# roeiherz/CanonicalSg2Im

Hardware: AMD Instinct MI355X
Metric: 256x256 images/sec/node (G+D step) (higher is better)
Workload: dtype f32; 1 GPU; BASELINE config C3: COCO-shaped AttSPADE 256x256, batch 16/GPU, 1-30 objects/img, ngf=64 ndf=64, --no_vgg_loss --use_img_disc 0; Sg2Layout GCN + SPADE G + 2-scale PatchGAN D + object-crop D, fwd+bwd+Adam; global_batch=16, parallelism=dp1

## Files before the change

canonicalsg2im_amd/_lib.py:

```python
import ctypes
import os

import torch

_HERE = os.path.dirname(os.path.abspath(__file__))
LIB_PATH = os.environ.get("CSG_HIP_LIB") or os.path.join(_HERE, "libcsg_hip.so")

MAX_TAPS = 16
ACT_NONE, ACT_LEAKY, ACT_TANH = 0, 1, 2

c_i32, c_i64, c_f32, c_f64, c_p = ctypes.c_int32, ctypes.c_int64, ctypes.c_float, ctypes.c_double, ctypes.c_void_p


class ConvDesc(ctypes.Structure):
    _fields_ = [
        ("B", c_i32), ("IHp", c_i32), ("IWp", c_i32), ("Cin", c_i32), ("x_cs", c_i32),
        ("IHv", c_i32), ("IWv", c_i32), ("in_up", c_i32),
        ("OHg", c_i32), ("OWg", c_i32), ("OHf", c_i32), ("OWf", c_i32), ("os", c_i32), ("ooy", c_i32), ("oox", c_i32),
        ("Cout", c_i32), ("y_cs", c_i32),
        ("istride", c_i32), ("ntaps", c_i32), ("wtaps", c_i32),
        ("tap_dy", c_i32 * MAX_TAPS), ("tap_dx", c_i32 * MAX_TAPS), ("tap_w", c_i32 * MAX_TAPS),
        ("act", c_i32), ("slope", c_f32), ("accumulate", c_i32), ("res_gate", c_i32),
    ]


class WinoDesc(ctypes.Structure):
    _fields_ = [("B", c_i32), ("H", c_i32), ("W", c_i32), ("Cin", c_i32), ("x_cs", c_i32), ("Cout", c_i32),
                ("y_cs", c_i32), ("act", c_i32), ("slope", c_f32)]


class WinoPackItem(ctypes.Structure):
    _fields_ = [("w", c_p), ("s_o", c_i64), ("s_i", c_i64), ("s_h", c_i64), ("s_w", c_i64), ("Cout", c_i64), ("Cin", c_i64),
                ("backward_data", c_i32), ("variant", c_i32), ("packed", c_p)]


class HingeItem(ctypes.Structure):
    _fields_ = [("x", c_p), ("dx", c_p), ("sb", c_i64), ("sh", c_i64), ("sw", c_i64), ("B", c_i64), ("H", c_i64), ("W", c_i64)]


class FewDesc(ctypes.Structure):
    _fields_ = [("B", c_i32), ("IH", c_i32), ("IW", c_i32), ("Cin", c_i32), ("x_cs", c_i32), ("KH", c_i32), ("KW", c_i32),
                ("pad", c_i32), ("cout_real", c_i32), ("act", c_i32), ("slope", c_f32), ("in_act", c_i32), ("in_slope", c_f32)]


class SnFwdItem(ctypes.Structure):
    _fields_ = [("w", c_p), ("u", c_p), ("v", c_p), ("Cout", c_i64), ("K", c_i64), ("w_eff", c_p), ("cl_Cin", c_i64),
                ("sigma", c_p), ("u_used", c_p), ("v_used", c_p), ("workspace", c_p), ("workspace_bytes", c_i64)]


class SnBwdItem(ctypes.Structure):
    _fields_ = [("dweff", c_p), ("Cout", c_i64), ("Cin", c_i64), ("KH", c_i64), ("KW", c_i64), ("s0", c_i64), ("s1", c_i64),
                ("s2", c_i64), ("s3", c_i64), ("w", c_p), ("u_used", c_p), ("v_used", c_p), ("sigma", c_p), ("dw", c_p),
                ("workspace", c_p), ("workspace_bytes", c_i64)]


class NormEvalItem(ctypes.Structure):
    _fields_ = [("running_mean", c_p), ("running_var", c_p), ("C", c_i64), ("offset", c_i64)]


class EmaItem(ctypes.Structure):
    _fields_ = [("src", c_p), ("dst", c_p), ("numel", c_i64), ("chunk0", c_i64), ("kind", c_i32), ("reserved", c_i32)]


class GemmDesc(ctypes.Structure):
    _fields_ = [("M", ctypes.c_int64), ("N", ctypes.c_int64), ("K", ctypes.c_int64),
                ("lda", ctypes.c_int64), ("ldb", ctypes.c_int64), ("ldy", ctypes.c_int64), ("ldg", ctypes.c_int64),
                ("act", ctypes.c_int32), ("slope", ctypes.c_float), ("gate_slope", ctypes.c_float)]


SIGNATURES = {
    "csg_version": (c_i32, []),
    "csg_last_error": (ctypes.c_char_p, []),
    "csg_prof_enable": (c_i32, [c_i32]),
    "csg_prof_reset": (c_i32, []),
    "csg_prof_num_kernels": (c_i32, []),
    "csg_prof_kernel_name": (ctypes.c_char_p, [c_i32]),
    "csg_prof_read": (c_i32, [c_i32, ctypes.POINTER(c_f64), ctypes.POINTER(c_i64), ctypes.POINTER(c_f64)]),
    "csg_embed_fwd": (c_i32, [c_p, c_i64, c_i64, c_p, c_i64, c_i64, c_p, c_i64, c_i64, c_p]),
    "csg_embed_bwd_workspace": (c_i64, [c_i64, c_i64, c_i64]),
    "csg_embed_bwd": (c_i32, [c_p, c_i64, c_i64, c_p, c_i64, c_i64, c_i64, c_i64, c_p, c_p, c_i64, c_p]),
    "csg_real_object_mask": (c_i32, [c_p, c_i64, c_i64, c_i64, c_i64, c_p, c_p]),
    "csg_graph_csr_build": (c_i32, [c_p, c_i64, c_i64, c_i64, c_p, c_p, c_p]),
    "csg_graph_csr_lds": (c_i64, [c_i64, c_i64]),
    "csg_gather_concat_fwd": (c_i32, [c_p, c_p, c_p, c_i64, c_i64, c_i64, c_i64, c_i64, c_p, c_p]),
    "csg_gather_concat_bwd_workspace": (c_i64, [c_i64, c_i64, c_i64, c_i64]),
    "csg_gather_concat_bwd": (c_i32, [c_p, c_p, c_p, c_i64, c_i64, c_i64, c_i64, c_i64, c_p, c_p, c_p, c_i64, c_p]),
    "csg_segment_avg_fwd_workspace": (c_i64, [c_i64, c_i64, c_i64, c_i64]),
    "csg_segment_avg_fwd": (c_i32, [c_p, c_p, c_p, c_p, c_p, c_i64, c_i64, c_i64, c_i64, c_i64, c_p, c_p, c_p, c_p,
                                    c_i64, c_p]),
    "csg_segment_avg_bwd": (c_i32, [c_p, c_p, c_p, c_p, c_p, c_p, c_p, c_p, c_i64, c_i64, c_i64, c_i64, c_i64, c_i32,
                                    c_p, c_p, c_p, c_p]),
    "csg_layout_fwd": (c_i32, [c_p, c_p, c_p, c_p, c_i64, c_i64, c_i64, c_i64, c_i64, c_i64, c_i64, c_i64, c_p, c_i64,
                               c_i64, c_p]),
    "csg_disc_input_fwd": (c_i32, [c_p, c_p, c_p, c_p, c_i64, c_i64, c_i64, c_i64, c_i64, c_i64, c_p, c_i64, c_i64, c_i64,
                                   c_i64, c_p, c_i64, c_p]),
    "csg_layout_bwd_workspace": (c_i64, [c_i64, c_i64, c_i64, c_i64, c_i64, c_i32, c_i32]),
    "csg_layout_bwd": (c_i32, [c_p, c_i64, c_i64, c_p, c_p, c_p, c_i64, c_i64, c_i64, c_i64, c_i64, c_i64, c_i64,
                               c_i64, c_p, c_i32, c_p, c_p, c_p, c_i64, c_p]),
    "csg_layout_bwd_masks": (c_i32, [c_p, c_i64, c_i64, c_p, c_p, c_i64, c_i64, c_i64, c_i64, c_i64, c_i64, c_i64, c_i64,
                                     c_p, c_p, c_i32, c_p]),
    "csg_layout_mass": (c_i32, [c_p, c_p, c_p, c_p, c_i64, c_i64, c_i64, c_i64, c_i64, c_i64, c_p, c_p]),
    "csg_layout_paint": (c_i32, [c_p, c_p, c_p, c_i64, c_p, c_i64, c_i64, c_i64, c_i64, c_i64, c_i64, c_i64, c_p, c_i64,
                                 c_i64, c_p]),
    "csg_conv_fwd_workspace": (c_i64, [ctypes.POINTER(ConvDesc)]),
    "csg_conv_fwd": (c_i32, [ctypes.POINTER(ConvDesc), c_p, c_p, c_p, c_p, c_p, c_p, c_i64, c_p]),
    "csg_conv_bwd_weight_workspace": (c_i64, [ctypes.POINTER(ConvDesc)]),
    "csg_conv_bwd_weight": (c_i32, [ctypes.POINTER(ConvDesc), c_p, c_p, c_p, c_p, c_p, c_i64, c_p]),
    "csg_wino_pack_bytes": (c_i64, [c_i64, c_i64]),
    "csg_wino_pack_weights": (c_i32, [c_p, c_i64, c_i64, c_i64, c_i64, c_i64, c_i64, c_i32, c_p, c_p, c_p]),
    "csg_conv_fwd_multi_workspace": (c_i64, [ctypes.POINTER(ConvDesc), c_i32]),
    "csg_conv_fwd_multi": (c_i32, [ctypes.POINTER(ConvDesc), c_i32, c_p, c_p, c_p, c_p, c_p, c_p, c_i64, c_p]),
    "csg_gemm_supported": (c_i32, [ctypes.POINTER(GemmDesc)]),
    "csg_gemm_nt": (c_i32, [ctypes.POINTER(GemmDesc), c_p, c_p, c_p, c_p, c_p, c_p]),
    "csg_gemm_tn_workspace": (c_i64, [c_i64, c_i64, c_i64]),
    "csg_gemm_tn": (c_i32, [c_i64, c_i64, c_i64, c_p, c_i64, c_p, c_i64, c_p, c_p, c_p, c_i64, c_p]),
    "csg_conv_few_supported": (c_i32, [ctypes.POINTER(FewDesc)]),
    "csg_conv_few_fwd_workspace": (c_i64, [ctypes.POINTER(FewDesc)]),
    "csg_conv_few_fwd": (c_i32, [ctypes.POINTER(FewDesc), c_p, c_p, c_p, c_p, c_p, c_i64, c_p]),
    "csg_conv_few_bwd_data": (c_i32, [ctypes.POINTER(FewDesc), c_p, c_p, c_p, c_p]),
    "csg_conv_few_bwd_weight_workspace": (c_i64, [ctypes.POINTER(FewDesc)]),
    "csg_conv_few_bwd_weight": (c_i32, [ctypes.POINTER(FewDesc), c_p, c_p, c_p, c_p, c_p, c_i64, c_p]),
    "csg_wino_conv_workspace": (c_i64, [ctypes.POINTER(WinoDesc)]),
    "csg_wino_conv": (c_i32, [ctypes.POINTER(WinoDesc), c_p, c_p, c_p, c_p, c_p, c_f32, c_p, c_p, c_i64, c_p]),
    "csg_wino_bwd_weight_workspace": (c_i64, [ctypes.POINTER(WinoDesc)]),
    "csg_wino_bwd_weight": (c_i32, [ctypes.POINTER(WinoDesc), c_p, c_p, c_p, c_p, c_p, c_i64, c_p]),
    "csg_wino4_bwd_weight_workspace": (c_i64, [ctypes.POINTER(WinoDesc)]),
    "csg_wino4_bwd_weight": (c_i32, [ctypes.POINTER(WinoDesc), c_p, c_p, c_p, c_p, c_p, c_i64, c_p]),
    "csg_wino4_supported": (c_i32, [ctypes.POINTER(WinoDesc)]),
    "csg_wino4_persistent": (c_i32, [c_i32]),
    "csg_wino_pack_weights_multi": (c_i32, [ctypes.POINTER(WinoPackItem), c_i32, c_p]),
    "csg_wino4_pack_bytes": (c_i64, [c_i64, c_i64]),
    "csg_wino4_pack_weights": (c_i32, [c_p, c_i64, c_i64, c_i64, c_i64, c_i64, c_i64, c_i32, c_p, c_p, c_p]),
    "csg_wino4_conv_workspace": (c_i64, [ctypes.POINTER(WinoDesc)]),
    "csg_wino4_conv": (c_i32, [ctypes.POINTER(WinoDesc), c_p, c_p, c_p, c_p, c_p, c_f32, c_p, c_p, c_i64, c_p]),
    "csg_wino4_conv_part": (c_i32, [ctypes.POINTER(WinoDesc), c_p, c_p, c_i64, c_i64, c_p, c_p, c_p, c_i64, c_p, c_p, c_f32,
                                    c_p, c_p]),
    "csg_wino4_conv_spade_supported": (c_i32, [ctypes.POINTER(WinoDesc)]),
    "csg_wino4_conv_spade": (c_i32, [ctypes.POINTER(WinoDesc), c_p, c_p, c_p, c_p, c_p, c_i64, c_p, c_p, c_f32, c_p, c_p]),
    "csg_wino34_supported": (c_i32, [ctypes.POINTER(WinoDesc), c_i32]),
    "csg_wino34_pack_weights": (c_i32, [c_p, c_i64, c_i64, c_i64, c_i64, c_i64, c_i64, c_i32, c_p, c_p, c_p]),
    "csg_wino34_conv_workspace": (c_i64, [ctypes.POINTER(WinoDesc), c_i32]),
    "csg_wino34_conv": (c_i32, [ctypes.POINTER(WinoDesc), c_i32, c_p, c_p, c_p, c_p, c_p, c_f32, c_p, c_p, c_i64, c_p]),
    "csg_act_bwd": (c_i32, [c_p, c_p, c_i64, c_i32, c_f32, c_p, c_p]),
    "csg_colsum": (c_i32, [c_p, c_i64, c_i64, c_i64, c_p, c_p, c_i64, c_p]),
    "csg_norm_stats": (c_i32, [c_p, c_i64, c_i64, c_i64, c_p, c_p, c_i64, c_p]),
    "csg_norm_finalize": (c_i32, [c_p, c_i64, c_i64, c_f64, c_f32, c_i32, c_p, c_p, c_p, c_p, c_f32, c_p]),
    "csg_norm_stats_finalize": (c_i32, [c_p, c_i64, c_i64, c_i64, c_p, c_i64, c_f64, c_f32, c_p, c_p, c_p, c_p, c_p, c_p, c_f32,
                                        c_p]),
    "csg_norm_apply_fwd": (c_i32, [c_p, c_p, c_p, c_p, c_f32, c_i64, c_i64, c_i64, c_p, c_p, c_f32, c_p, c_p]),
    "csg_norm_eval_stats_multi": (c_i32, [ctypes.POINTER(NormEvalItem), c_i32, c_f32, c_p, c_p]),
    "csg_deprocess_u8_workspace": (c_i64, [c_i64]),
    "csg_deprocess_u8": (c_i32, [c_p, c_i64, c_i64, c_i64, c_i64, ctypes.POINTER(c_f32), ctypes.POINTER(c_f32), c_i32, c_p, c_p,
                                 c_i64, c_p]),
    "csg_preprocess_workspace": (c_i64, [c_p, c_i64, c_i64]),
    "csg_preprocess": (c_i32, [c_p, c_i64, c_p, c_p, c_i64, c_i64, c_i64, ctypes.POINTER(c_f32), ctypes.POINTER(c_f32), c_p, c_p,
                               c_p, c_i64, c_p]),
    "csg_preprocess_px_workspace": (c_i64, [c_p, c_i64, c_i64]),
    "csg_preprocess_px": (c_i32, [c_p, c_i64, c_p, c_p, c_i64, c_i64, c_i64, ctypes.POINTER(c_f32), ctypes.POINTER(c_f32), c_p,
                                  c_p, c_p, c_i64, c_p]),
    "csg_clevr_boxes": (c_i32, [c_p, c_p, c_i64, c_p, c_p, c_p, c_p, c_i64, c_i64, c_p, c_p]),
    "csg_vg_rows": (c_i32, [c_p, c_p, c_p, c_p, c_p, c_p, c_i64, c_i64, c_i64, c_p, c_p, c_p]),
    "csg_draw_boxes_u8": (c_i32, [c_p, c_p, c_p, c_i64, c_i64, c_i64, c_i64, c_i64, c_i64, c_p, c_i64, c_i32, c_p, c_p]),
    "csg_draw_labels_u8": (c_i32, [c_p, c_p, c_p, c_i64, c_i64, c_i64, c_i64, c_i64, c_i64, c_p, c_i64, c_p, c_p, c_p, c_p,
                                   c_p]),
    "csg_draw_graph_u8": (c_i32, [c_p, c_i64, c_p, c_p, c_i64, c_p, c_i64, c_i64, c_i64, ctypes.c_uint32, c_p, c_p]),
    "csg_box_iou": (c_i32, [c_p, c_p, c_p, c_i64, c_i64, c_i64, c_i64, c_p, c_p, c_p, c_p, c_p]),
    "csg_relation_agreement_workspace": (c_i64, [c_i64]),
    "csg_relation_agreement": (c_i32, [c_p, c_p, c_p, c_p, c_p, c_p, c_i64, c_i64, c_i64, c_i64, c_p, c_p, c_p, c_p, c_p, c_p,
                                       c_i64, c_p]),
    "csg_layout_consistency": (c_i32, [c_p, c_p, c_p, c_i64, c_i64, c_p, c_p, c_p, c_p, c_p, c_p, c_p]),
    "csg_graph_rows_select": (c_i32, [c_p, c_p, c_i64, c_i64, c_i64, c_i64, c_p, c_p, c_p, c_p]),
    "csg_graph_rewrite": (c_i32, [c_p, c_p, c_p, c_i64, c_i64, c_i64, c_p, c_i32, c_i32, c_f64, ctypes.c_uint64, c_p, c_p]),
    "csg_norm_apply_bwd_reduce": (c_i32, [c_p, c_p, c_p, c_p, c_p, c_p, c_f32, c_i64, c_i64, c_i64, c_p, c_p, c_p, c_i64,
                                          c_i64, c_p]),
    "csg_norm_apply_bwd_dx": (c_i32, [c_p, c_p, c_p, c_p, c_p, c_f32, c_p, c_f64, c_i64, c_i64, c_i64, c_p, c_p, c_p, c_f32,
                                      c_p, c_p, c_i64, c_p]),
    "csg_nearest_resize_fwd": (c_i32, [c_p, c_i64, c_i64, c_i64, c_i64, c_i64, c_i64, c_p, c_p]),
    "csg_nearest_resize_bwd": (c_i32, [c_p, c_i64, c_i64, c_i64, c_i64, c_i64, c_i64, c_p, c_p]),
    "csg_upsample2x_fwd": (c_i32, [c_p, c_i64, c_i64, c_i64, c_i64, c_p, c_p]),
    "csg_upsample2x_bwd": (c_i32, [c_p, c_i64, c_i64, c_i64, c_i64, c_p, c_p]),
    "csg_avgpool3s2_fwd": (c_i32, [c_p, c_i64, c_i64, c_i64, c_i64, c_p, c_p]),
    "csg_avgpool3s2_bwd": (c_i32, [c_p, c_i64, c_i64, c_i64, c_i64, c_p, c_p]),
    "csg_avgpool3s2_bwd_add": (c_i32, [c_p, c_i64, c_i64, c_i64, c_i64, c_p, c_p, c_p]),
    "csg_crop_fwd": (c_i32, [c_p, c_i64, c_i64, c_i64, c_i64, c_i64, c_p, c_p, c_i64, c_i64, c_i64, c_p, c_i64, c_p]),
    "csg_crop_bwd": (c_i32, [c_p, c_i64, c_i64, c_i64, c_i64, c_i64, c_p, c_p, c_i64, c_i64, c_i64, c_i64, c_p, c_p]),
    "csg_crop_bwd_boxes": (c_i32, [c_p, c_p, c_i64, c_i64, c_i64, c_i64, c_i64, c_p, c_p, c_i64, c_i64, c_i64, c_i64, c_p,
                                   c_p]),
    "csg_maxpool2_fwd": (c_i32, [c_p, c_i64, c_i64, c_i64, c_i64, c_p, c_p]),
    "csg_maxpool2_bwd": (c_i32, [c_p, c_p, c_i64, c_i64, c_i64, c_i64, c_p, c_p]),
    "csg_avgpool2_fwd": (c_i32, [c_p, c_i64, c_i64, c_i64, c_i64, c_p, c_p]),
    "csg_avgpool2_bwd": (c_i32, [c_p, c_i64, c_i64, c_i64, c_i64, c_p, c_p]),
    "csg_l1_mean_workspace": (c_i64, [c_i64]),
    "csg_l1_mean_fwd": (c_i32, [c_p, c_p, c_i64, c_p, c_p, c_i64, c_p]),
    "csg_l1_mean_bwd": (c_i32, [c_p, c_p, c_p, c_i64, c_p, c_p]),
    "csg_hinge_mean_fwd": (c_i32, [ctypes.POINTER(HingeItem), c_i32, c_i32, c_p, c_p]),
    "csg_hinge_mean_bwd": (c_i32, [ctypes.POINTER(HingeItem), c_i32, c_i32, c_p, c_p]),
    "csg_spectral_norm_workspace": (c_i64, [c_i64, c_i64]),
    "csg_spectral_norm_fwd_multi": (c_i32, [ctypes.POINTER(SnFwdItem), c_i32, c_i32, c_f32, c_p]),
    "csg_spectral_norm_bwd_multi": (c_i32, [ctypes.POINTER(SnBwdItem), c_i32, c_p]),
    "csg_canon_workspace": (c_i64, [c_i64]),
    "csg_canon_build": (c_i32, [c_p, c_p, c_p, c_p, c_i64, c_i64, ctypes.POINTER(c_i32), c_i64, c_i32, c_i32, c_p, c_i64,
                                c_p, c_p]),
    "csg_canon_emit": (c_i32, [c_p, c_p, c_i64, c_i64, ctypes.POINTER(c_i32), c_i64, c_i32, c_i32, c_p, c_p, c_i64, c_p,
                               c_p, c_p]),
    "csg_canon_converse": (c_i32, [c_p, c_p, c_i64, c_i64, ctypes.POINTER(c_i32), c_i64, c_i32, c_i32, c_p, c_p, c_p, c_p,
                                   c_i64, c_p, c_p, c_p]),
    "csg_canon_general_workspace": (c_i64, [c_i64, c_i64, c_i64]),
    "csg_canon_general_build": (c_i32, [c_p, c_p, c_p, c_p, c_i64, c_i64, c_p, c_p, c_i64, ctypes.POINTER(c_i32), c_i64,
                                        c_i64, c_i32, c_p, c_i64, c_p, c_p]),
    "csg_canon_general_build_dev": (c_i32, [c_p, c_p, c_p, c_p, c_i64, c_i64, c_p, c_p, c_i64, ctypes.POINTER(c_i32), c_i64,
                                            c_i64, c_i32, c_p, c_i64, c_p, c_p]),
    "csg_pair_relations": (c_i32, [c_p, c_p, c_p, c_p, c_p, c_p, c_p, c_p, c_i64, c_i64, ctypes.POINTER(c_i32), c_i32, c_p,
                                   c_p]),
    "csg_coco_masks": (c_i32, [c_p] * 16 + [c_i64] * 6 + [c_p, c_p, c_p]),
    "csg_canon_general_converse": (c_i32, [c_i64, ctypes.POINTER(c_i32), c_i64, c_p, c_i64, c_p, c_p, c_p, c_p, c_p]),
    "csg_canon_general_close": (c_i32, [c_i64, ctypes.POINTER(c_i32), c_i64, c_i32, c_p, c_i64, c_p, c_p]),
    "csg_canon_general_emit": (c_i32, [c_i64, ctypes.POINTER(c_i32), c_i64, c_p, c_i64, c_p, c_i64, c_p, c_p, c_p]),
    "csg_canon_small_workspace": (c_i64, [c_i64, c_i64]),
    "csg_canon_small_build": (c_i32, [c_p, c_p, c_p, c_i64, c_i64, c_p, c_p, c_i64, c_i64, c_i64, c_i64, c_i64, c_i32, c_i32,
                                      c_p, c_p, c_p, c_i64, c_p, c_p, c_i64, c_p, c_p]),
    "csg_canon_small_emit": (c_i32, [c_i64, c_i64, c_i64, c_p, c_i64, c_p, c_i64, c_p, c_p, c_p]),
    "csg_clevr_graph_count": (c_i32, [c_p, c_p, c_i64, c_i64, c_p, c_p, c_i64, c_i64, c_i64, c_i64, c_i32, c_p, c_p]),
    "csg_clevr_graph_emit": (c_i32, [c_p, c_i64, c_i64, c_p, c_i64, c_i64, c_i64, c_i64, c_i32, c_i64, c_p, c_p, c_p]),
    "csg_resize_bilinear": (c_i32, [c_p, c_i32, c_i64, c_i64, c_i64, c_i64, c_i64, c_i64, c_f32, c_f32, c_i32, c_p, c_p]),
    "csg_pool3": (c_i32, [c_p, c_i64, c_i64, c_i64, c_i64, c_i64, c_i32, c_i32, c_i32, c_p, c_i64, c_i64, c_p]),
    "csg_spatial_mean": (c_i32, [c_p, c_i64, c_i64, c_i64, c_i64, c_p, c_p]),
    "csg_bias_act": (c_i32, [c_p, c_i64, c_i64, c_i64, c_i64, c_p, c_i32, c_f32, c_p]),
    "csg_feat_stats": (c_i32, [c_p, c_i64, c_i64, c_p, c_p, c_p]),
    "csg_feat_stats_finalize": (c_i32, [c_p, c_p, c_i64, c_i64, c_p, c_p, c_p]),
    "csg_softmax_rows": (c_i32, [c_p, c_i64, c_i64, c_i64, c_p, c_p]),
    "csg_inception_score_workspace": (c_i64, [c_i64, c_i64, c_i64]),
    "csg_inception_score": (c_i32, [c_p, c_i64, c_i64, c_i64, c_p, c_i64, c_p, c_p]),
    "csg_crop_windows": (c_i32, [c_p, c_i64, c_i64, c_i64, c_p, c_p]),
    "csg_crop_resize_bilinear": (c_i32, [c_p, c_i64, c_i64, c_i64, c_p, c_p, c_i64, c_i64, c_i64, c_f32, c_f32, c_i32, c_p, c_p]),
    "csg_kid_sums_workspace_bytes": (c_i64, [c_i64, c_i64]),
    "csg_kid_sums": (c_i32, [c_p, c_i64, c_p, c_i64, c_i64, c_p, c_p, c_i64, c_i64, c_f64, c_f64, c_i32, c_p, c_i64, c_p, c_p]),
    "csg_feat_class_sums": (c_i32, [c_p, c_p, c_i64, c_i64, c_i64, c_p, c_p, c_p]),
    "csg_manifold_column_chunks": (c_i64, [c_i64, c_i64]),
    "csg_knn_radii_workspace_bytes": (c_i64, [c_i64, c_i64]),
    "csg_knn_radii": (c_i32, [c_p, c_i64, c_i64, c_i64, c_p, c_i64, c_p, c_p]),
    "csg_ball_counts_workspace_bytes": (c_i64, [c_i64, c_i64]),
    "csg_ball_counts": (c_i32, [c_p, c_i64, c_p, c_i64, c_i64, c_p, c_p, c_i64, c_p, c_p, c_p]),
    "csg_ema_table_plan": (c_i64, [ctypes.POINTER(EmaItem), c_i64]),
    "csg_ema_apply": (c_i32, [c_p, c_i64, c_i64, c_i32, c_f32, c_f32, c_p]),
    "csg_augment_table": (c_i32, [ctypes.c_uint64, c_i64, c_i64, c_i64, c_i64, c_i64, c_p, c_p]),
    "csg_augment_table_host": (c_i32, [ctypes.c_uint64, c_i64, c_i64, c_i64, c_i64, c_i64, c_p]),
    "csg_augment_workspace_bytes": (c_i64, [c_i64, c_i64]),
    "csg_augment_fwd": (c_i32, [c_p, c_p, c_p, c_i64, c_i64, c_i64, c_i64, c_i64, c_i32, c_p, c_i64, c_p]),
    "csg_augment_bwd": (c_i32, [c_p, c_p, c_p, c_i64, c_i64, c_i64, c_i64, c_i64, c_i32, c_p, c_i64, c_p]),
    "csg_augment_gate": (c_i32, [ctypes.c_uint64, c_i64, c_i64, c_i64, c_i64, c_p, c_p, c_p]),
    "csg_augment_gate_host": (c_i32, [ctypes.c_uint64, c_i64, c_i64, c_i64, c_i64, c_i64, c_p]),
    "csg_augment_fwd_gated": (c_i32, [c_p, c_p, c_p, c_i64, c_i64, c_i64, c_i64, c_i64, c_i32, c_p, c_i64, c_p, c_p]),
    "csg_augment_bwd_gated": (c_i32, [c_p, c_p, c_p, c_i64, c_i64, c_i64, c_i64, c_i64, c_i32, c_p, c_i64, c_p, c_p]),
    "csg_ada_accumulate": (c_i32, [ctypes.POINTER(HingeItem), c_i32, c_p, c_p]),
    "csg_ada_update": (c_i32, [c_p, c_i64, c_i64, c_p]),
    "csg_ada_update_host": (c_i32, [c_p, c_i64, c_i64]),
}


def _load():
    if not os.path.exists(LIB_PATH):
        raise ImportError(
            "libcsg_hip.so is not built (%s). Run `python -c 'import __graft_entry__ as g; g.build()'` "
            "from the repository root; there is no CPU fallback." % LIB_PATH)
    lib = ctypes.CDLL(LIB_PATH)
    for name, (res, args) in SIGNATURES.items():
        fn = getattr(lib, name)
        fn.restype = res
        fn.argtypes = args
    return lib


lib = _load()


def last_error():
    return lib.csg_last_error().decode("utf-8", "replace")

# ... 41 lines not shown
```

canonicalsg2im_amd/csrc/csg_api.hip:

```cpp
#include <stdarg.h>
#include <string.h>

#include <mutex>
#include <vector>

#include "csg_common.h"

namespace csg {

static thread_local char g_err[512] = "";

void set_error(const char* fmt, ...) {
  va_list ap;
  va_start(ap, fmt);
  vsnprintf(g_err, sizeof(g_err), fmt, ap);
  va_end(ap);
}

int check_launch(const char* what) {
  hipError_t e = hipGetLastError();
  if (e != hipSuccess) {
    set_error("%s: %s", what, hipGetErrorString(e));
    return CSG_E_LAUNCH;
  }
  return CSG_OK;
}

struct Rec {
  int kid;
  double work;
  hipEvent_t e0, e1;
  bool first;
};
static int g_prof = 0;
static std::mutex g_mu;
static std::vector<Rec> g_pending;
static std::vector<hipEvent_t> g_free;
static double g_ms[K_COUNT];
static double g_work[K_COUNT];
static int64_t g_n[K_COUNT];

static bool hbm_kernel(int kid) {
  switch (kid) {
    case K_GATHER_FWD: case K_GATHER_BWD: case K_SEGAVG_FWD: case K_SEGAVG_BWD: case K_LAYOUT_FWD: case K_LAYOUT_BWD:
    case K_ACT_BWD: case K_NORM_STATS: case K_NORM_APPLY_FWD: case K_NORM_BWD_REDUCE: case K_NORM_BWD_DX:
    case K_UPSAMPLE_FWD: case K_UPSAMPLE_BWD: case K_AVGPOOL_FWD: case K_AVGPOOL_BWD:
      return true;
    default:
      return false;
  }
}

bool prof_on(int kid) {
  return g_prof == 1 || (g_prof == 2 && (kid == K_IGEMM_FWD || kid == K_WINO_CONV || kid == K_WINO4_CONV)) ||
         (g_prof == 3 && hbm_kernel(kid));
}

bool prof_serialize() { return g_prof == 1 || g_prof == 3; }

ProfCur& prof_cur() {
  static thread_local ProfCur cur = {0, 0.0, false, false};
  return cur;
}

static hipEvent_t get_event() {
  std::lock_guard<std::mutex> lk(g_mu);
  if (!g_free.empty()) {
    hipEvent_t e = g_free.back();
    g_free.pop_back();
    return e;
  }
  hipEvent_t e;
  hipEventCreate(&e);
  return e;
}

void prof_begin(int kid, double work) {
  ProfCur& c = prof_cur();
  c.kid = kid;
  c.work = work;
  c.armed = true;
  c.used = false;
}

void prof_next(hipEvent_t& e0, hipEvent_t& e1) {
  ProfCur& c = prof_cur();
  e0 = get_event();
  e1 = get_event();
  std::lock_guard<std::mutex> lk(g_mu);
  g_pending.push_back(Rec{c.kid, c.used ? 0.0 : c.work, e0, e1, !c.used});
  c.used = true;
}

void prof_end() {
  ProfCur& c = prof_cur();
  c.armed = c.used = false;
}

static void resolve() {
  std::lock_guard<std::mutex> lk(g_mu);
  for (auto& r : g_pending) {
    hipEventSynchronize(r.e1);
    float ms = 0.f;
    hipEventElapsedTime(&ms, r.e0, r.e1);
    g_ms[r.kid] += ms;
    g_work[r.kid] += r.work;
    g_n[r.kid] += r.first ? 1 : 0;
    g_free.push_back(r.e0);
    g_free.push_back(r.e1);
  }
  g_pending.clear();
}

static const char* kNames[K_COUNT] = {
    "embed_fwd",      "embed_bwd",      "real_object_mask", "graph_csr_build", "gather_concat_fwd", "gather_concat_bwd",
    "segment_avg_fwd", "segment_avg_bwd", "layout_fwd",       "layout_bwd",      "igemm_fwd",         "igemm_fwd64",   "splitk_epilogue", "igemm_wgrad",
    "wgrad_reduce",   "act_bwd",        "colsum",           "norm_stats",      "norm_finalize",     "norm_apply_fwd",
    "norm_bwd_reduce", "norm_bwd_dx",    "upsample2x_fwd",   "upsample2x_bwd",  "avgpool3s2_fwd",    "avgpool3s2_bwd", "crop_fwd", "crop_bwd",
    "maxpool2_fwd",   "maxpool2_bwd",   "l1_mean_fwd",      "l1_mean_bwd",
    "canon_build",    "canon_emit",     "spectral_norm_fwd", "spectral_norm_bwd",
    "wino_conv",      "wino_pack",      "wino_wgrad",
    "few_fwd",        "few_bwd_data",   "few_bwd_weight",
    "wino4_conv",     "wino4_wgrad",
    "gemm_nt",        "gemm_tn",
    "norm_eval_stats", "deprocess_u8", "box_iou", "preprocess", "clevr_boxes", "vg_rows", "draw_boxes_u8",
    "canon_small_build", "canon_small_emit", "clevr_graph_count", "clevr_graph_emit", "coco_masks",
    "resize_bilinear", "pool3", "spatial_mean", "bias_act", "feat_stats", "inception_score",
    "draw_labels_u8", "draw_graph_u8",
    "crop_windows", "crop_resize_bilinear", "kid_sums", "feat_class_sums",
    "knn_radii", "ball_counts",
    "ema", "augment"};

}

extern "C" {

int csg_version(void) { return 122; }
const char* csg_last_error(void) { return csg::g_err; }

int csg_prof_enable(int on) {
  csg::resolve();
  csg::g_prof = on < 0 ? 0 : (on > 3 ? 1 : on);
  return CSG_OK;
}

int csg_prof_reset(void) {
  csg::resolve();
  memset(csg::g_ms, 0, sizeof(csg::g_ms));
  memset(csg::g_work, 0, sizeof(csg::g_work));
  memset(csg::g_n, 0, sizeof(csg::g_n));
  return CSG_OK;
}

int csg_prof_num_kernels(void) { return csg::K_COUNT; }

const char* csg_prof_kernel_name(int kid) {
  if (kid < 0 || kid >= csg::K_COUNT) return "";
  return csg::kNames[kid];
}

int csg_prof_read(int kid, double* ms, int64_t* launches, double* work) {
  CSG_REQUIRE(kid >= 0 && kid < csg::K_COUNT, CSG_E_BADSHAPE, "csg_prof_read: bad kernel id %d", kid);
  csg::resolve();
  if (ms) *ms = csg::g_ms[kid];
  if (launches) *launches = csg::g_n[kid];
  if (work) *work = csg::g_work[kid];
  return CSG_OK;
}

}
```

canonicalsg2im_amd/csrc/csg_pack.h:

```cpp
#pragma once
#include <stdint.h>

#include <hip/hip_runtime.h>

#define CSG_PACK_MULTI 24

struct PackMultiItem {
  const float* w;
  float4* up;
  int s_n, s_k, s_h, s_w;
  int flip, N, K, NT32, Q8;
  int start;
};

struct PackMulti {
  PackMultiItem it[CSG_PACK_MULTI];
  int n;
};

extern "C" __attribute__((visibility("hidden"))) int csg_wino2_pack_multi_launch(const PackMulti* pm, int blocks, double bytes,
                                                                                 hipStream_t s);
extern "C" __attribute__((visibility("hidden"))) int csg_wino4_pack_multi_launch(const PackMulti* pm, int blocks, double bytes,
                                                                                 hipStream_t s);
```

canonicalsg2im_amd/csrc/csg_wino_host.h:

```cpp
#pragma once
#include "csg_common.h"
#include "csg_reduce.h"

namespace csg {

template <typename Pixels>
static inline int wino_desc_check(const csg_wino_desc* d, const char* who, int positions, Pixels pixels) {
  CSG_REQUIRE(d != nullptr, CSG_E_BADSHAPE, "%s: null descriptor", who);
  CSG_REQUIRE(d->B > 0 && d->H > 0 && d->W > 0 && d->Cin > 0 && d->Cout > 0, CSG_E_BADSHAPE, "%s: non-positive dimension", who);
  CSG_REQUIRE(d->Cin % 4 == 0 && d->x_cs % 4 == 0 && d->x_cs >= d->Cin && d->Cout % 4 == 0 && d->y_cs % 4 == 0 &&
                  d->y_cs >= d->Cout,
              CSG_E_UNSUPPORTED, "%s: channel counts and strides must be multiples of 4", who);
  CSG_REQUIRE((int64_t)pixels(*d) * (int64_t)(d->x_cs > d->y_cs ? d->x_cs : d->y_cs) * 4 < CSG_MAX_RECORDS, CSG_E_UNSUPPORTED,
              "%s: tensor too large for 32-bit byte offsets", who);
  CSG_REQUIRE((int64_t)positions * ((d->Cout + 31) / 32) * ((d->Cin + 7) / 8) * 1024 < CSG_MAX_RECORDS, CSG_E_UNSUPPORTED,
              "%s: packed weights too large for 32-bit byte offsets", who);
  return CSG_OK;
}

static inline int wino_conv_dense_x(const csg_wino_desc* d, const char* who) {
  CSG_REQUIRE(d->x_cs == d->Cin, CSG_E_UNSUPPORTED, "%s: x must be dense (x_cs=%d, Cin=%d)", who, d->x_cs, d->Cin);
  return CSG_OK;
}

template <typename P>
static inline void wino_split_plan(P& p, bool plain, int min_stages, int min_range) {
  if (!plain || p.y_cs != p.Cout) return;
  const int64_t blocks = (int64_t)p.B * p.tby * p.tbx * p.nblocks;
  if (blocks >= 384 || p.nstage < min_stages) return;
  int ks = (int)((512 + blocks - 1) / blocks);
  if (ks > p.nstage / min_range) ks = p.nstage / min_range;
  if (ks < 2) return;
  p.sps = (p.nstage + ks - 1) / ks;
  p.ksplit = (p.nstage + p.sps - 1) / p.sps;
}

template <typename P, typename Plan>
static inline int64_t wino_conv_workspace(const csg_wino_desc* d, int min_stages, int min_range, Plan plan) {
  P p;
  size_t shm = 0;
  if (plan(p, shm)) return -1;
  wino_split_plan(p, d->act == CSG_ACT_NONE, min_stages, min_range);
  return p.ksplit > 1 ? (int64_t)p.ksplit * p.slab * 4 : 0;
}

struct WinoConvArgs {
  const float *x, *packed, *bias, *residual, *gate;
  float gate_slope;
  float *y, *workspace;
  int64_t workspace_bytes;
  hipStream_t s;
};

template <typename P, typename Plan, typename Launch>
static inline int wino_conv_entry(const char* who, const char* sum_who, const csg_wino_desc* d, int min_stages, int min_range,
                                  int kid, double taps, const WinoConvArgs& a, Plan plan, Launch launch) {
  P p;
  size_t shm = 0;
  int rc = plan(p, shm);
  if (rc) return rc;
  wino_split_plan(p, d->act == CSG_ACT_NONE && a.bias == nullptr && a.residual == nullptr && a.gate == nullptr, min_stages,
                  min_range);
  p.gate_slope = a.gate_slope;
  if (p.ksplit > 1 && (a.workspace == nullptr || a.workspace_bytes < (int64_t)p.ksplit * p.slab * 4)) {
    p.ksplit = 1;
    p.sps = p.nstage;
  }
  float* const y = p.ksplit > 1 ? a.workspace : a.y;
  CSG_REQUIRE(((uintptr_t)a.x % 16) == 0 && ((uintptr_t)a.packed % 16) == 0 && ((uintptr_t)y % 16) == 0 &&
                  (a.gate == nullptr || ((uintptr_t)a.gate % 16) == 0),
              CSG_E_UNSUPPORTED, "%s: x, packed, y, gate and workspace must be 16-byte aligned", who);
  ProfScope ps(kid, 2.0 * (double)(p.slab / p.y_cs) * taps * p.Cin * p.Cout, a.s);
  rc = launch(p, shm, y);
  if (rc == CSG_OK && p.ksplit > 1) {
    launch_slab_reduce(a.workspace, p.slab, a.y, nullptr, 0, nullptr, p.ksplit, a.s);
    rc = check_launch(sum_who);
  }
  return rc;
}

static inline int64_t wino_pack_bytes(int positions, int64_t N, int64_t K) {
  if (N <= 0 || K <= 0) return -1;
  return (int64_t)positions * cdiv(N, 32) * cdiv(K, 8) * 64 * 16;
}

template <typename Launch>
static inline int wino_pack_entry(const char* who, int positions, int taps, const float* w, int64_t s_o, int64_t s_i,
                                  int64_t s_h, int64_t s_w, int64_t Cout, int64_t Cin, int32_t backward_data,
                                  const float* sigma, float* packed, void* stream, Launch launch) {
  CSG_REQUIRE(w != nullptr && packed != nullptr && Cout > 0 && Cin > 0, CSG_E_BADSHAPE, "%s: bad arguments", who);
  CSG_REQUIRE(((uintptr_t)packed % 16) == 0, CSG_E_UNSUPPORTED, "%s: packed must be 16-byte aligned", who);
  const int64_t N = backward_data ? Cin : Cout, K = backward_data ? Cout : Cin;
  const int64_t s_n = backward_data ? s_i : s_o, s_k = backward_data ? s_o : s_i;
  const int NT32 = (int)cdiv(N, 32), Q8 = (int)cdiv(K, 8);
  hipStream_t s = (hipStream_t)stream;
  ProfScope ps(K_WINO_PACK, (double)Cout * Cin * taps * 4 + (double)wino_pack_bytes(positions, N, K), s);
  launch(dim3((unsigned)cdiv(Q8, 4), (unsigned)NT32), s, w, s_n, s_k, s_h, s_w, backward_data ? 1 : 0, (int)N, (int)K, sigma, NT32,
         Q8, (float4*)packed);
  return check_launch(who);
}

template <typename P>
static inline int wino_wg_slice_plan(P& p, const char* who, int tiles2d, int target_blocks, int min_regions, int max_slices) {
  const int64_t nr = (int64_t)p.B * p.RXn * p.RYn;
  CSG_REQUIRE(nr < (1ll << 30), CSG_E_UNSUPPORTED, "%s: too many regions", who);
  p.nregions = (int)nr;
  int ns = (target_blocks + tiles2d - 1) / tiles2d;
  const int max_ns = (int)((nr + min_regions - 1) / min_regions);
  if (ns > max_ns) ns = max_ns;
  if (ns > max_slices) ns = max_slices;
  if (ns < 1) ns = 1;
  p.rps = (int)((nr + ns - 1) / ns);
  p.nsplit = (int)((nr + p.rps - 1) / p.rps);
  return CSG_OK;
}

static inline int64_t wino_wg_workspace(const csg_wino_desc* d, int nslab) {
  return (int64_t)nslab * d->Cout * (9 * (int64_t)d->Cin + 1) * 4;
}

template <typename Launch>
static inline int wino_wg_run(const char* who, const char* sum_who, const csg_wino_desc* d, int nslab, bool direct, float* dw,
                              float* db, float* workspace, int64_t workspace_bytes, hipStream_t s, Launch launch) {
  const int64_t wsize = (int64_t)d->Cout * 9 * d->Cin, need = wino_wg_workspace(d, nslab);
  CSG_REQUIRE(workspace != nullptr && workspace_bytes >= need, CSG_E_WORKSPACE, "%s: workspace %ld < %ld bytes", who,
              (long)workspace_bytes, (long)need);
  float* const dbslabs = db != nullptr ? workspace + (int64_t)nslab * wsize : nullptr;
  const int rc = direct ? launch(dw, db) : launch(workspace, dbslabs);
  if (rc || direct) return rc;
  ProfScope ps(K_WGRAD_REDUCE, (double)(nslab + 1) * wsize * 4, s);
  launch_slab_reduce(workspace, wsize, dw, dbslabs, db != nullptr ? d->Cout : 0, db, nslab, s);
  return check_launch(sum_who);
}

}
```

canonicalsg2im_amd/csrc/wino.hip:

```cpp
#include <stddef.h>
#include <stdlib.h>

#include <type_traits>

#include "csg_buffer.h"
#include "csg_common.h"
#include "csg_pack.h"
#include "csg_reduce.h"
#include "csg_wino_host.h"

using namespace csg;

typedef __attribute__((ext_vector_type(16))) float f32x16;

#define WN_BK 16
#define WN_PS 18
#define WN_RSE 36
#define WN_MAXLD 7

struct WinoParams {
  int B, H, W, Cin, x_cs, Cout, y_cs;
  int TW, TH;
  int tbx, tby;
  int nblocks;
  int RS;
  int NT32, Q8;
  int act;
  float slope;
  float gate_slope;
  int nstage;
  int ntb;
  int ksplit, sps;
  long long slab;
};

__device__ __forceinline__ int wn_xcd_remap(int bid, int nblk) {
  const int q = nblk >> 3, r = nblk & 7;
  const int xcd = bid & 7, idx = bid >> 3;
  return (xcd < r ? xcd * (q + 1) : r * (q + 1) + (xcd - r) * q) + idx;
}

#define WP_LD 33
__device__ __forceinline__ void wn_pack_tile(const float* __restrict__ w, int64_t s_n, int64_t s_k, int64_t s_h,
                                             int64_t s_w, int flip, int N, int K, const float* __restrict__ sigma,
                                             int NT32, int Q8, float4* __restrict__ up, int qb, int nt) {
  __shared__ float g[9][32][WP_LD];
  const int tid = threadIdx.x;
  const bool k_fast = s_k <= s_n;
  const float sg = sigma != nullptr ? sigma[0] : 1.0f;
  float stage[36];
#pragma unroll
  for (int it = 0; it < 36; ++it) {
    const int t = it >> 2, r = tid + 256 * (it & 3);
    const int nl = k_fast ? (r >> 5) : (r & 31), kl = k_fast ? (r & 31) : (r >> 5);
    const int n = nt * 32 + nl, k = qb * 32 + kl;
    const int a = t / 3, b = t - 3 * a;
    const int aa = flip ? 2 - a : a, bb = flip ? 2 - b : b;
    stage[it] = (n < N && k < K) ? w[(int64_t)n * s_n + (int64_t)k * s_k + aa * s_h + bb * s_w] : 0.f;
  }
#pragma unroll
  for (int it = 0; it < 36; ++it) {
    const int t = it >> 2, r = tid + 256 * (it & 3);
    const int nl = k_fast ? (r >> 5) : (r & 31), kl = k_fast ? (r & 31) : (r >> 5);
    g[t][nl][kl] = sigma != nullptr ? stage[it] / sg : stage[it];
  }
  __syncthreads();
  const int lane = tid & 63, ql = tid >> 6;
  const int q = qb * 4 + ql;
  if (q >= Q8) return;
  const int nl = lane & 31, h = lane >> 5;
  float u[16][4];
#pragma unroll
  for (int e = 0; e < 4; ++e) {
    const int kl = 8 * ql + (e >> 1) * 4 + 2 * h + (e & 1);
    float t[4][3];
#pragma unroll
    for (int b = 0; b < 3; ++b) {
      const float g0 = g[b][nl][kl], g1 = g[3 + b][nl][kl], g2 = g[6 + b][nl][kl];
      t[0][b] = g0;
      t[1][b] = 0.5f * g0 + 0.5f * g1 + 0.5f * g2;
      t[2][b] = 0.5f * g0 - 0.5f * g1 + 0.5f * g2;
      t[3][b] = g2;
    }
#pragma unroll
    for (int xi = 0; xi < 4; ++xi) {
      u[xi * 4 + 0][e] = t[xi][0];
      u[xi * 4 + 1][e] = 0.5f * t[xi][0] + 0.5f * t[xi][1] + 0.5f * t[xi][2];
      u[xi * 4 + 2][e] = 0.5f * t[xi][0] - 0.5f * t[xi][1] + 0.5f * t[xi][2];
      u[xi * 4 + 3][e] = t[xi][2];
    }
  }
#pragma unroll
  for (int p = 0; p < 16; ++p)
    up[(((int64_t)p * NT32 + nt) * Q8 + q) * 64 + lane] = make_float4(u[p][0], u[p][1], u[p][2], u[p][3]);
}

__global__ __launch_bounds__(256) void k_wino_pack(const float* __restrict__ w, int64_t s_n, int64_t s_k, int64_t s_h,
                                                    int64_t s_w, int flip, int N, int K, const float* __restrict__ sigma,
                                                    int NT32, int Q8, float4* __restrict__ up) {
  wn_pack_tile(w, s_n, s_k, s_h, s_w, flip, N, K, sigma, NT32, Q8, up, blockIdx.x, blockIdx.y);
}

__global__ __launch_bounds__(256) void k_wino_pack_multi(PackMulti pm) {
  int i = 0;
  while (i + 1 < pm.n && (int)blockIdx.x >= pm.it[i + 1].start) ++i;
  const PackMultiItem& d = pm.it[i];
  const int local = blockIdx.x - d.start, nqb = (d.Q8 + 3) >> 2;
  wn_pack_tile(d.w, d.s_n, d.s_k, d.s_h, d.s_w, d.flip, d.N, d.K, nullptr, d.NT32, d.Q8, d.up, local % nqb, local / nqb);
}

constexpr int wn_row_stride(int TW) {
  const int C = 2 * TW + 2;
  for (int pad = 0; pad < 256; pad += 2) {
    const int RS = C * WN_PS + pad;
    unsigned long long used = 0;
    bool ok = true;
    for (int j = 0; j < 32 && ok; ++j) {
      const int wa = (WN_PS * (j % TW) + 2 * RS * (j / TW)) & 63;
      const unsigned long long m = (1ull << wa) | (1ull << ((wa + 1) & 63));
      if (used & m) ok = false;
      used |= m;
    }
    if (ok) return RS;
  }
  return C * WN_PS;
}

template <int TW, int NTB = 2>
__global__ __launch_bounds__(256, 2) void k_wino_conv2(WinoParams p, const float* __restrict__ x,
                                                        const float4* __restrict__ up, const float* __restrict__ bias,
                                                        const float* __restrict__ res, const float* __restrict__ gate,
                                                        float* __restrict__ y) {
  constexpr int TH = 32 / TW;
  constexpr int R = 2 * TH + 2, C = 2 * TW + 2;
  constexpr int RS = wn_row_stride(TW);
  constexpr int BUFW = R * RS + 16;
  constexpr int HALF = (C / 2) * WN_PS;
  constexpr int NLD = (R * C * 4 + 255) / 256;
  extern __shared__ __attribute__((aligned(16))) float smem[];
  const int tid = threadIdx.x, lane = tid & 63, wave = tid >> 6;

  int bid = wn_xcd_remap(blockIdx.x, gridDim.x);
  const int split = bid % p.ksplit;
  bid /= p.ksplit;
  const int nb = bid % p.nblocks;
  bid /= p.nblocks;
  const int bx = bid % p.tbx;
  bid /= p.tbx;
  const int by = bid % p.tby;
  const int img = bid / p.tby;
  const int X0 = bx * 2 * TW, Y0 = by * 2 * TH;

  const csg_i32x4 rsX = csg_make_srd(x, (long long)p.B * p.H * p.W * p.x_cs * 4);
  const csg_i32x4 rsU = csg_make_srd(up, (long long)16 * p.NT32 * p.Q8 * 64 * 16);
  unsigned goff[NLD];
  int loff[NLD];
#pragma unroll
  for (int i = 0; i < NLD; ++i) {
    const int e = tid + 256 * i;
    goff[i] = CSG_OOB_OFF;
    loff[i] = BUFW - 16 + (tid & 3) * 4;
    if (e < R * C * 4) {
      const int pix = e >> 2, c4 = e & 3;
      const int row = pix / C, col = pix - row * C;
      const int iy = Y0 + row - 1, ix = X0 + col - 1;
      loff[i] = row * RS + ((col & 1) * (C >> 1) + (col >> 1)) * WN_PS + c4 * 4;
      if (iy >= 0 && iy < p.H && ix >= 0 && ix < p.W)
        goff[i] = (unsigned)(((img * p.H + iy) * p.W + ix) * p.x_cs + c4 * 4) * 4u;
    }
  }
  csg_f32x4 st[NLD];
  auto load_stage = [&](int s) {
#pragma unroll
    for (int i = 0; i < NLD; ++i) st[i] = csg_buf_load_x4(rsX, (int)goff[i], s * (WN_BK * 4), 0);
  };
  auto store_stage = [&](float* base) {
#pragma unroll
    for (int i = 0; i < NLD; ++i) {
      float* dst = base + loff[i];
      *(float2*)(dst) = make_float2(st[i].x, st[i].y);
      *(float2*)(dst + 2) = make_float2(st[i].z, st[i].w);
    }
  };

  const int j = lane & 31, h = lane >> 5;
  const int tx = j % TW, tyl = j / TW;
  const int ia = wave == 0 ? 0 : (wave == 2 ? 2 : 1);
  const int ib = wave == 0 ? 2 : (wave == 1 ? 2 : (wave == 2 ? 1 : 3));
  const float sgn = wave == 1 ? 1.0f : -1.0f;
  const float* pa0 = smem + (2 * tyl + ia) * RS + tx * WN_PS + 2 * h;
  const float* pb0 = smem + (2 * tyl + ib) * RS + tx * WN_PS + 2 * h;

  unsigned uoff[4][NTB];
#pragma unroll
  for (int nt = 0; nt < NTB; ++nt) {
    const int nt32 = nb * NTB + nt;
#pragma unroll
    for (int nu = 0; nu < 4; ++nu)
      uoff[nu][nt] = nt32 < p.NT32 ? (unsigned)((((wave * 4 + nu) * p.NT32 + nt32) * p.Q8) * 64 + lane) * 16u : CSG_OOB_OFF;
  }
  csg_f32x4 u[4][NTB];
  auto load_u_half = [&](int nt, int q) {
    const int qq = min(q, p.Q8 - 1);
#pragma unroll
    for (int nu = 0; nu < 4; ++nu) u[nu][nt] = csg_buf_load_x4(rsU, (int)uoff[nu][nt], qq * 1024, 0);
  };

  f32x16 acc[4][NTB];
#pragma unroll
  for (int nu = 0; nu < 4; ++nu)
#pragma unroll
    for (int nt = 0; nt < NTB; ++nt)
#pragma unroll
      for (int e = 0; e < 16; ++e) acc[nu][nt][e] = 0.f;

  float2 v[4][2];
  auto prepare = [&](int bufsel, int o) {
    const float* pa = pa0 + bufsel * BUFW + 8 * o;
    const float* pb = pb0 + bufsel * BUFW + 8 * o;
#pragma unroll
    for (int cp = 0; cp < 2; ++cp) {
      float2 q[4];
#pragma unroll
      for (int c = 0; c < 4; ++c) {
        const int co = (c & 1) * HALF + (c >> 1) * WN_PS + 4 * cp;
        const float2 da = *(const float2*)(pa + co), db = *(const float2*)(pb + co);
        q[c] = make_float2(da.x + sgn * db.x, da.y + sgn * db.y);
      }
      v[0][cp] = make_float2(q[0].x - q[2].x, q[0].y - q[2].y);
      v[1][cp] = make_float2(q[1].x + q[2].x, q[1].y + q[2].y);
      v[2][cp] = make_float2(q[2].x - q[1].x, q[2].y - q[1].y);
      v[3][cp] = make_float2(q[1].x - q[3].x, q[1].y - q[3].y);
    }
  };
  auto mfma_half = [&](int nt) {
#pragma unroll
    for (int nu = 0; nu < 4; ++nu) acc[nu][nt] = __builtin_amdgcn_mfma_f32_32x32x2f32(u[nu][nt].x, v[nu][0].x, acc[nu][nt], 0, 0, 0);
#pragma unroll
    for (int nu = 0; nu < 4; ++nu) acc[nu][nt] = __builtin_amdgcn_mfma_f32_32x32x2f32(u[nu][nt].y, v[nu][0].y, acc[nu][nt], 0, 0, 0);
#pragma unroll
    for (int nu = 0; nu < 4; ++nu) acc[nu][nt] = __builtin_amdgcn_mfma_f32_32x32x2f32(u[nu][nt].z, v[nu][1].x, acc[nu][nt], 0, 0, 0);
#pragma unroll
    for (int nu = 0; nu < 4; ++nu) acc[nu][nt] = __builtin_amdgcn_mfma_f32_32x32x2f32(u[nu][nt].w, v[nu][1].y, acc[nu][nt], 0, 0, 0);
  };
  auto stage = [&](int s, auto bufsel_tag) {
    constexpr int bufsel = decltype(bufsel_tag)::value;
    load_stage(s + 1);
#pragma unroll
    for (int o = 0; o < 2; ++o) {
      prepare(bufsel, o);
      mfma_half(0);
      __builtin_amdgcn_sched_barrier(0);
      load_u_half(0, 2 * s + o + 1);
      if (NTB > 1) {
        mfma_half(NTB - 1);
        __builtin_amdgcn_sched_barrier(0);
        load_u_half(NTB - 1, 2 * s + o + 1);
      }
    }
    store_stage(smem + (bufsel ^ 1) * BUFW);
    __syncthreads();
  };

  const int s_begin = split * p.sps, s_end = min(p.nstage, s_begin + p.sps);
  y += (long long)split * p.slab;
  load_stage(s_begin);
  load_u_half(0, 2 * s_begin);
  if (NTB > 1) load_u_half(NTB - 1, 2 * s_begin);
  store_stage(smem);
  __syncthreads();
  int s = s_begin;
  for (; s + 1 < s_end; s += 2) {
    stage(s, std::integral_constant<int, 0>());
    stage(s + 1, std::integral_constant<int, 1>());
  }
  if (s < s_end) stage(s, std::integral_constant<int, 0>());

  float* rbuf = smem;
#pragma unroll
  for (int nt = 0; nt < NTB; ++nt) {
#pragma unroll
    for (int g = 0; g < 4; ++g) {
      float r0[4], r1[4];
#pragma unroll
      for (int e = 0; e < 4; ++e) {
        const float m0 = acc[0][nt][4 * g + e], m1 = acc[1][nt][4 * g + e], m2 = acc[2][nt][4 * g + e], m3 = acc[3][nt][4 * g + e];
        r0[e] = m0 + m1 + m2;
        r1[e] = m1 - m2 - m3;
      }
      const int ch = 8 * g + 4 * h;
      *(float4*)(rbuf + ((wave * 2 + 0) * 32 + j) * WN_RSE + ch) = make_float4(r0[0], r0[1], r0[2], r0[3]);
      *(float4*)(rbuf + ((wave * 2 + 1) * 32 + j) * WN_RSE + ch) = make_float4(r1[0], r1[1], r1[2], r1[3]);
    }
    __syncthreads();
    {
      const int tile = tid >> 3, cq = tid & 7;
      const int n = nb * (32 * NTB) + nt * 32 + cq * 4;
      const int ttx = tile % TW, tty = tile / TW;
      const int oy = Y0 + 2 * tty, ox = X0 + 2 * ttx;
      if (n < p.Cout && oy < p.H && ox < p.W) {
        float4 rr[4][2];
#pragma unroll
        for (int xi = 0; xi < 4; ++xi)
#pragma unroll
          for (int b = 0; b < 2; ++b) rr[xi][b] = *(const float4*)(rbuf + ((xi * 2 + b) * 32 + tile) * WN_RSE + cq * 4);
        float4 bv = make_float4(0.f, 0.f, 0.f, 0.f);
        if (bias != nullptr) bv = *(const float4*)(bias + n);
#pragma unroll
        for (int a = 0; a < 2; ++a)
#pragma unroll
          for (int b = 0; b < 2; ++b) {
            float vv[4];
            const float4 q0 = rr[0][b], q1 = rr[1][b], q2 = rr[2][b], q3 = rr[3][b];
            if (a == 0) {
              vv[0] = q0.x + q1.x + q2.x; vv[1] = q0.y + q1.y + q2.y; vv[2] = q0.z + q1.z + q2.z; vv[3] = q0.w + q1.w + q2.w;
            } else {
              vv[0] = q1.x - q2.x - q3.x; vv[1] = q1.y - q2.y - q3.y; vv[2] = q1.z - q2.z - q3.z; vv[3] = q1.w - q2.w - q3.w;
            }
            vv[0] += bv.x; vv[1] += bv.y; vv[2] += bv.z; vv[3] += bv.w;
#pragma unroll
            for (int e = 0; e < 4; ++e) {
              if (p.act == CSG_ACT_LEAKY)
                vv[e] = vv[e] > 0.f ? vv[e] : vv[e] * p.slope;
              else if (p.act == CSG_ACT_TANH)
                vv[e] = tanhf(vv[e]);
            }
            const int64_t pix = ((int64_t)img * p.H + (oy + a)) * p.W + (ox + b);
            if (res != nullptr) {
              const float4 rv = *(const float4*)(res + pix * p.y_cs + n);
              vv[0] += rv.x; vv[1] += rv.y; vv[2] += rv.z; vv[3] += rv.w;
            }
            if (gate != nullptr) {
              const float4 gv = *(const float4*)(gate + pix * p.y_cs + n);
              vv[0] *= gv.x > 0.f ? 1.f : p.gate_slope; vv[1] *= gv.y > 0.f ? 1.f : p.gate_slope;
              vv[2] *= gv.z > 0.f ? 1.f : p.gate_slope; vv[3] *= gv.w > 0.f ? 1.f : p.gate_slope;
            }
            *(float4*)(y + pix * p.y_cs + n) = make_float4(vv[0], vv[1], vv[2], vv[3]);
          }
      }
    }
    __syncthreads();
  }
}

constexpr size_t wn_conv_lds(int TW) {
  const size_t in_bytes = (size_t)2 * ((2 * (32 / TW) + 2) * wn_row_stride(TW) + 16) * 4;
  const size_t ep_bytes = (size_t)4 * 2 * 32 * WN_RSE * 4;
  return in_bytes > ep_bytes ? in_bytes : ep_bytes;
}

static int wn_plan(const csg_wino_desc* d, WinoParams& p, size_t& shm, const char* who) {
  int rc = wino_desc_check(d, who, 16, [](const csg_wino_desc& d) { return (int64_t)d.B * d.H * d.W; });
  if (rc == CSG_OK) rc = wino_conv_dense_x(d, who);
  if (rc) return rc;
  CSG_REQUIRE(d->H % 2 == 0 && d->W % 2 == 0 && d->W >= 8, CSG_E_UNSUPPORTED, "%s: H=%d, W=%d must be even, W >= 8", who,
              d->H, d->W);
  CSG_REQUIRE(d->Cin % 16 == 0, CSG_E_UNSUPPORTED, "%s: Cin must be a multiple of 16 (one LDS stage)", who);
  p.B = d->B; p.H = d->H; p.W = d->W; p.Cin = d->Cin; p.x_cs = d->x_cs; p.Cout = d->Cout; p.y_cs = d->y_cs;
  p.TW = d->W >= 32 ? 16 : (d->W >= 16 ? 8 : 4);
  p.TH = 32 / p.TW;
  p.tbx = (d->W / 2 + p.TW - 1) / p.TW;
  p.tby = (d->H / 2 + p.TH - 1) / p.TH;
  p.ntb = d->Cout <= 32 ? 1 : 2;
  p.nblocks = (d->Cout + 32 * p.ntb - 1) / (32 * p.ntb);
  p.RS = wn_row_stride(p.TW);
  p.NT32 = (d->Cout + 31) / 32;
  p.Q8 = (d->Cin + 7) / 8;
  p.act = d->act; p.slope = d->slope;
  p.nstage = (d->Cin + WN_BK - 1) / WN_BK;
  p.ksplit = 1;
  p.sps = p.nstage;
  p.slab = (long long)d->B * d->H * d->W * d->y_cs;
  shm = wn_conv_lds(p.TW);
  return CSG_OK;
}

template <int TW, int NTB>
static int wn_conv_launch(const WinoParams& p, int64_t grid, const float* x, const float4* up, const float* bias,
                          const float* residual, const float* gate, float* y, hipStream_t s) {
  constexpr size_t shm = wn_conv_lds(TW);
  static_assert(shm <= 96 * 1024, "k_wino_conv2: two blocks per CU");
  const int rc = lds_limit<k_wino_conv2<TW, NTB>, shm>(shm, "csg_wino_conv");
  if (rc) return rc;
  CSG_LAUNCH((k_wino_conv2<TW, NTB>), dim3((unsigned)grid), dim3(256), shm, s, p, x, up, bias, residual, gate, y);
  return check_launch("csg_wino_conv");
}

static int wn_conv_dispatch(const WinoParams& p, const WinoConvArgs& a, float* y) {
  const int64_t grid = (int64_t)p.B * p.tby * p.tbx * p.nblocks * p.ksplit;
  CSG_REQUIRE(grid < (1ll << 31), CSG_E_UNSUPPORTED, "csg_wino_conv: grid too large");
  const float4* up = (const float4*)a.packed;
  if (p.ntb == 1) {
    if (p.TW == 16) return wn_conv_launch<16, 1>(p, grid, a.x, up, a.bias, a.residual, a.gate, y, a.s);
    if (p.TW == 8) return wn_conv_launch<8, 1>(p, grid, a.x, up, a.bias, a.residual, a.gate, y, a.s);
    return wn_conv_launch<4, 1>(p, grid, a.x, up, a.bias, a.residual, a.gate, y, a.s);
  }
  if (p.TW == 16) return wn_conv_launch<16, 2>(p, grid, a.x, up, a.bias, a.residual, a.gate, y, a.s);
  if (p.TW == 8) return wn_conv_launch<8, 2>(p, grid, a.x, up, a.bias, a.residual, a.gate, y, a.s);
  return wn_conv_launch<4, 2>(p, grid, a.x, up, a.bias, a.residual, a.gate, y, a.s);
}

#define WN_SPLIT 16, 8

extern "C" {

int64_t csg_wino_pack_bytes(int64_t N, int64_t K) { return wino_pack_bytes(16, N, K); }

int csg_wino_pack_weights(const float* w, int64_t s_o, int64_t s_i, int64_t s_h, int64_t s_w, int64_t Cout, int64_t Cin,
                          int32_t backward_data, const float* sigma, float* packed, void* stream) {
  return wino_pack_entry("csg_wino_pack_weights", 16, 9, w, s_o, s_i, s_h, s_w, Cout, Cin, backward_data, sigma, packed, stream,
                         [](dim3 grid, hipStream_t s, auto... a) { CSG_LAUNCH(k_wino_pack, grid, dim3(256), 0, s, a...); });
}

int csg_wino2_pack_multi_launch(const PackMulti* pm, int blocks, double bytes, hipStream_t s) {
  ProfScope ps(K_WINO_PACK, bytes, s);
  CSG_LAUNCH(k_wino_pack_multi, dim3((unsigned)blocks), dim3(256), 0, s, *pm);
  return check_launch("csg_wino_pack_weights_multi(F(2x2,3x3))");
}

int64_t csg_wino_conv_workspace(const csg_wino_desc* d) {
  return wino_conv_workspace<WinoParams>(
      d, WN_SPLIT, [&](WinoParams& p, size_t& shm) { return wn_plan(d, p, shm, "csg_wino_conv_workspace"); });
}

int csg_wino_conv(const csg_wino_desc* d, const float* x, const float* packed, const float* bias, const float* residual,
                  const float* gate, float gate_slope, float* y, float* workspace, int64_t workspace_bytes, void* stream) {
  const WinoConvArgs a{x, packed, bias, residual, gate, gate_slope, y, workspace, workspace_bytes, (hipStream_t)stream};
  return wino_conv_entry<WinoParams>(
      "csg_wino_conv", "csg_wino_conv(slab sum)", d, WN_SPLIT, K_WINO_CONV, 9.0, a,
      [&](WinoParams& p, size_t& shm) { return wn_plan(d, p, shm, "csg_wino_conv"); },
      [&](const WinoParams& p, size_t, float* out) { return wn_conv_dispatch(p, a, out); });
}

}

struct WinoWgParams {
  int B, H, W, Cin, x_cs, Cout, y_cs;
  int RXn, RYn, nregions;
  int cblocks, kblocks;
  int nsplit, rps;
};

#define WG_EPS 33

template <int TSX, int NT>
__global__ __launch_bounds__(256, 2) void k_wino_wgrad(WinoWgParams p, const float* __restrict__ x,
                                                        const float* __restrict__ dy, float* __restrict__ slabs,
                                                        float* __restrict__ dbslabs) {
  static_assert(NT == 1, "one 32-channel input group per block");
  constexpr int TSY = 16 / TSX;
  constexpr int XR = 2 * TSY + 2, XC = 2 * TSX + 2, YR = 2 * TSY, YC = 2 * TSX;
  constexpr int XCH = 32 * NT, XF4 = XCH / 4;
  constexpr int NLX = (XR * XC * XF4 + 255) / 256, NLY = (YR * YC * 16) / 256;
  static_assert((YR * YC * 16) % 256 == 0, "dY staging divides evenly");
  constexpr int XW = NLX * 256 * 4, YW = YR * YC * 64, BUFW = XW + YW;
  extern __shared__ __attribute__((aligned(16))) float smem[];
  const int tid = threadIdx.x, lane = tid & 63, wave = tid >> 6;
  const int c = lane & 31, h = lane >> 5;
  int bid = wn_xcd_remap(blockIdx.x, gridDim.x);
  const int kb = bid % p.kblocks;
  bid /= p.kblocks;
  const int cb = bid % p.cblocks;
  const int sp = bid / p.cblocks;
  const int r0 = sp * p.rps, r1 = min(p.nregions, r0 + p.rps);

  const int ia = wave == 0 ? 0 : (wave == 1 ? 1 : (wave == 2 ? 2 : 3));
  const int ib = wave == 0 ? 2 : (wave == 1 ? 2 : 1);
  const float sgn = wave == 1 ? 1.0f : -1.0f;
  const float ea = wave == 3 ? 0.f : 1.f;
  const float eb = wave == 0 ? 0.f : (wave == 2 ? -1.f : 1.f);

  const __amdgpu_buffer_rsrc_t rsX = __builtin_amdgcn_make_buffer_rsrc(
      (void*)(x - (int64_t)(p.W + 1) * p.x_cs), 0, (int)(((long long)p.B * p.H * p.W + p.W + 1) * p.x_cs * 4), 0x00020000);
  const __amdgpu_buffer_rsrc_t rsY =
      __builtin_amdgcn_make_buffer_rsrc((void*)dy, 0, (int)((long long)p.B * p.H * p.W * p.y_cs * 4), 0x00020000);
  unsigned xoff[NLX], yoff[NLY];
  int xflag[NLX];
#pragma unroll
  for (int i = 0; i < NLX; ++i) {
    const int e = tid + 256 * i;
    const int pix = e / XF4, c4 = e - pix * XF4;
    const int row = pix / XC, col = pix - row * XC;
    const int ch = kb * XCH + c4 * 4;
    const bool ok = (e < XR * XC * XF4) & (ch < p.Cin);
    xoff[i] = ok ? (unsigned)((row * p.W + col) * p.x_cs + ch) * 4u : CSG_OOB_OFF;
    xflag[i] = (row == 0 ? 1 : 0) | (row == XR - 1 ? 2 : 0) | (col == 0 ? 4 : 0) | (col == XC - 1 ? 8 : 0);
  }
#pragma unroll
  for (int i = 0; i < NLY; ++i) {
    const int e = tid + 256 * i;
    const int pix = e >> 4, c4 = e & 15;
    const int row = pix / YC, col = pix - row * YC;
    const int ch = cb * 64 + c4 * 4;
    yoff[i] = ch < p.Cout ? (unsigned)((row * p.W + col) * p.y_cs + ch) * 4u : CSG_OOB_OFF;
  }
  typedef __attribute__((address_space(3))) void* lds_ptr;
  auto dma_stage = [&](int r, int bufsel) {
    const int rr = min(r, p.nregions - 1);
    const int rx = rr % p.RXn, t = rr / p.RXn;
    const int ry = t % p.RYn, img = t / p.RYn;
    const int y0 = ry * 2 * TSY, x0 = rx * 2 * TSX;
    const int edge = (y0 == 0 ? 1 : 0) | (y0 + 2 * TSY == p.H ? 2 : 0) | (x0 == 0 ? 4 : 0) | (x0 + 2 * TSX == p.W ? 8 : 0);
    const int pix0 = (img * p.H + y0) * p.W + x0;
    float* base = smem + bufsel * BUFW + wave * 256;
#pragma unroll
    for (int i = 0; i < NLX; ++i)
      __builtin_amdgcn_raw_ptr_buffer_load_lds(rsX, (lds_ptr)(base + i * 1024), 16,
                                               (int)((xflag[i] & edge) ? CSG_OOB_OFF : xoff[i]), pix0 * p.x_cs * 4, 0, 0);
#pragma unroll
    for (int i = 0; i < NLY; ++i)
      __builtin_amdgcn_raw_ptr_buffer_load_lds(rsY, (lds_ptr)(base + XW + i * 1024), 16, (int)yoff[i], pix0 * p.y_cs * 4, 0, 0);
  };

  const bool do_db = dbslabs != nullptr && kb == 0 && wave == 1;
  float dbacc[2] = {0.f, 0.f};

  f32x16 acc[4][2][NT];
#pragma unroll
  for (int nu = 0; nu < 4; ++nu)
#pragma unroll
    for (int mt = 0; mt < 2; ++mt)
#pragma unroll
      for (int nt = 0; nt < NT; ++nt)
#pragma unroll
        for (int e = 0; e < 16; ++e) acc[nu][mt][nt][e] = 0.f;

  struct Raw {
    float dy[2][2][2];
    float xr[NT][2][4];
  };
  const float* lxx = smem + h * (2 * XCH) + c;
  const float* lxy = smem + XW + h * (2 * 64) + c;
  auto read_pair = [&](int bufsel, int kp, Raw& r) {
    const int t = 2 * kp, tsx = t % TSX, tsy = t / TSX;
    const float* bx = lxx + bufsel * BUFW;
    const float* by = lxy + bufsel * BUFW;
#pragma unroll
    for (int m = 0; m < 2; ++m)
#pragma unroll
      for (int i = 0; i < 2; ++i)
#pragma unroll
        for (int jx = 0; jx < 2; ++jx) r.dy[m][i][jx] = by[((2 * tsy + i) * YC + 2 * tsx + jx) * 64 + m * 32];
#pragma unroll
    for (int m = 0; m < NT; ++m)
#pragma unroll
      for (int jx = 0; jx < 4; ++jx) {
        r.xr[m][0][jx] = bx[((2 * tsy + ia) * XC + 2 * tsx + jx) * XCH + m * 32];
        r.xr[m][1][jx] = bx[((2 * tsy + ib) * XC + 2 * tsx + jx) * XCH + m * 32];
      }
  };
  auto compute_pair = [&](const Raw& r) {
    float E[4][2], V[4][NT];
#pragma unroll
    for (int m = 0; m < 2; ++m) {
      const float e0 = ea * r.dy[m][0][0] + eb * r.dy[m][1][0];
      const float e1 = ea * r.dy[m][0][1] + eb * r.dy[m][1][1];
      E[0][m] = e0;
      E[1][m] = e0 + e1;
      E[2][m] = e0 - e1;
      E[3][m] = e1;
      if (do_db) dbacc[m] += (r.dy[m][0][0] + r.dy[m][0][1]) + (r.dy[m][1][0] + r.dy[m][1][1]);
    }
#pragma unroll
    for (int m = 0; m < NT; ++m) {
      float q[4];
#pragma unroll
      for (int jx = 0; jx < 4; ++jx) q[jx] = r.xr[m][0][jx] + sgn * r.xr[m][1][jx];
      V[0][m] = q[0] - q[2];
      V[1][m] = q[1] + q[2];
      V[2][m] = q[2] - q[1];
      V[3][m] = q[3] - q[1];
    }
#pragma unroll
    for (int nu = 0; nu < 4; ++nu)
#pragma unroll
      for (int mt = 0; mt < 2; ++mt)
#pragma unroll
        for (int nt = 0; nt < NT; ++nt)
          acc[nu][mt][nt] = __builtin_amdgcn_mfma_f32_32x32x2f32(E[nu][mt], V[nu][nt], acc[nu][mt][nt], 0, 0, 0);
  };

  Raw ra, rb;
  auto stage = [&](int r, auto bufsel_tag) {
    constexpr int bufsel = decltype(bufsel_tag)::value;
    dma_stage(r + 1, bufsel ^ 1);
    __builtin_amdgcn_sched_barrier(0);
#pragma unroll
    for (int kp = 0; kp < 8; kp += 2) {
      read_pair(bufsel, kp + 1, rb);
      compute_pair(ra);
      __builtin_amdgcn_sched_barrier(0);
      if (kp + 2 < 8) {
        read_pair(bufsel, kp + 2, ra);
        compute_pair(rb);
        __builtin_amdgcn_sched_barrier(0);
      }
    }
    __syncthreads();
    read_pair(bufsel ^ 1, 0, ra);
    compute_pair(rb);
    __builtin_amdgcn_sched_barrier(0);
  };

  if (r0 < r1) {
    dma_stage(r0, 0);
    __syncthreads();
    read_pair(0, 0, ra);
    int r = r0;
    for (; r + 1 < r1; r += 2) {
      stage(r, std::integral_constant<int, 0>());
      stage(r + 1, std::integral_constant<int, 1>());
    }
    if (r < r1) stage(r, std::integral_constant<int, 0>());
  }
  __syncthreads();

  const float gx = (wave == 1 || wave == 2) ? 0.5f : 1.0f;
  float* slab = slabs + (int64_t)sp * p.Cout * 9 * p.Cin;
#pragma unroll
  for (int mt = 0; mt < 2; ++mt)
#pragma unroll
    for (int nt = 0; nt < NT; ++nt) {
#pragma unroll
      for (int e = 0; e < 16; ++e) {
        const float a0 = acc[0][mt][nt][e], a1 = 0.5f * acc[1][mt][nt][e], a2 = 0.5f * acc[2][mt][nt][e], a3 = acc[3][mt][nt][e];
        const int i = (e & 3) + 8 * (e >> 2) + 4 * h;
        smem[((wave * 3 + 0) * 32 + i) * WG_EPS + c] = gx * (a0 + a1 + a2);
        smem[((wave * 3 + 1) * 32 + i) * WG_EPS + c] = gx * (a1 - a2);
        smem[((wave * 3 + 2) * 32 + i) * WG_EPS + c] = gx * (a1 + a2 + a3);
      }
      __syncthreads();
      const int kcol = tid & 31;
      const int cin_g = kb * XCH + nt * 32 + kcol;
#pragma unroll
      for (int rep = 0; rep < 4; ++rep) {
        const int i = (tid >> 5) + 8 * rep;
        const int cout_g = cb * 64 + mt * 32 + i;
        if (cout_g < p.Cout && cin_g < p.Cin) {
          float R[4][3];
#pragma unroll
          for (int xi = 0; xi < 4; ++xi)
#pragma unroll
            for (int b = 0; b < 3; ++b) R[xi][b] = smem[((xi * 3 + b) * 32 + i) * WG_EPS + kcol];
          float* dst = slab + (int64_t)cout_g * 9 * p.Cin + cin_g;
#pragma unroll
          for (int b = 0; b < 3; ++b) {
            dst[(0 * 3 + b) * p.Cin] = R[0][b] + R[1][b] + R[2][b];
            dst[(1 * 3 + b) * p.Cin] = R[1][b] - R[2][b];
            dst[(2 * 3 + b) * p.Cin] = R[1][b] + R[2][b] + R[3][b];
          }
        }
      }
      __syncthreads();
    }
  if (do_db) {
#pragma unroll
    for (int m = 0; m < 2; ++m) {
      const float tot = dbacc[m] + __shfl_xor(dbacc[m], 32, 64);
      const int co = cb * 64 + m * 32 + c;
      if (h == 0 && co < p.Cout) dbslabs[(int64_t)sp * p.Cout + co] = tot;
    }
  }
}

static int wn_wg_tsx(int W) { return W >= 32 ? 16 : (W >= 16 ? 8 : 4); }

static int wn_wg_plan(const csg_wino_desc* d, WinoWgParams& p, const char* who) {
  const int rc = wino_desc_check(d, who, 0, [](const csg_wino_desc& d) { return (int64_t)d.B * d.H * d.W + d.W + 1; });
  if (rc) return rc;
  const int tsx = wn_wg_tsx(d->W), tsy = 16 / tsx;
  CSG_REQUIRE(d->W >= 8 && d->W % (2 * tsx) == 0 && d->H % (2 * tsy) == 0, CSG_E_UNSUPPORTED,
              "%s: H=%d, W=%d must be multiples of the %dx%d-tile stage", who, d->H, d->W, tsx, tsy);
  p.B = d->B; p.H = d->H; p.W = d->W; p.Cin = d->Cin; p.x_cs = d->x_cs; p.Cout = d->Cout; p.y_cs = d->y_cs;
  p.RXn = d->W / (2 * tsx);
  p.RYn = d->H / (2 * tsy);
  p.cblocks = (d->Cout + 63) / 64;
  p.kblocks = (d->Cin + 31) / 32;
  return wino_wg_slice_plan(p, who, p.cblocks * p.kblocks, 1024, 8, 512);
}

template <int TSX>
static int wn_wg_launch(const WinoWgParams& p, const float* x, const float* dy, float* slabs, float* dbslabs, hipStream_t s) {
  constexpr int tsx = TSX, tsy = 16 / TSX;
  constexpr size_t x_f4 = (size_t)(((2 * tsy + 2) * (2 * tsx + 2) * 8 + 255) / 256) * 256;
  constexpr size_t stage_bytes = 2 * (x_f4 * 16 + (size_t)(2 * tsy) * (2 * tsx) * 64 * 4);
  constexpr size_t ep_bytes = (size_t)4 * 3 * 32 * WG_EPS * 4;
  constexpr size_t shm = stage_bytes > ep_bytes ? stage_bytes : ep_bytes;
  const int rc = lds_limit<k_wino_wgrad<TSX, 1>, shm>(shm, "csg_wino_bwd_weight");
  if (rc) return rc;
  ProfScope ps(K_WINO_WGRAD, 2.0 * p.B * p.H * p.W * 9.0 * p.Cin * p.Cout, s);
  CSG_LAUNCH((k_wino_wgrad<TSX, 1>), dim3((unsigned)(p.cblocks * p.kblocks * p.nsplit)), dim3(256), shm, s, p, x, dy, slabs,
             dbslabs);
  return check_launch("csg_wino_bwd_weight");
}

extern "C" {

int64_t csg_wino_bwd_weight_workspace(const csg_wino_desc* d) {
  WinoWgParams p;
  if (wn_wg_plan(d, p, "csg_wino_bwd_weight_workspace")) return -1;
  return wino_wg_workspace(d, p.nsplit);
}

int csg_wino_bwd_weight(const csg_wino_desc* d, const float* x, const float* dy, float* dw, float* db, float* workspace,
                        int64_t workspace_bytes, void* stream) {
  WinoWgParams p;
  const int rc = wn_wg_plan(d, p, "csg_wino_bwd_weight");
  if (rc) return rc;
  hipStream_t s = (hipStream_t)stream;
  return wino_wg_run("csg_wino_bwd_weight", "csg_wino_bwd_weight(reduce)", d, p.nsplit, p.nsplit == 1, dw, db, workspace,
                     workspace_bytes, s, [&](float* slabs, float* dbslabs) {
                       const int tsx = wn_wg_tsx(d->W);
                       if (tsx == 16) return wn_wg_launch<16>(p, x, dy, slabs, dbslabs, s);
                       if (tsx == 8) return wn_wg_launch<8>(p, x, dy, slabs, dbslabs, s);
                       return wn_wg_launch<4>(p, x, dy, slabs, dbslabs, s);
                     });
}

}
```

canonicalsg2im_amd/csrc/wino4.hip:

```cpp
#include <stddef.h>
#include <stdlib.h>

#include <type_traits>

#include "csg_buffer.h"
#include "csg_common.h"
#include "csg_pack.h"
#include "csg_reduce.h"
#include "csg_wino_host.h"

using namespace csg;

typedef __attribute__((ext_vector_type(16))) float f32x16;
typedef const volatile __attribute__((address_space(3))) csg_f32x2* w4_lds_cv2;

#define W4_TW 8
#define W4_TH 4
#define W4_CQ 9
#define W4_PS 8
#define W4_RSE 36
#define W4_NLD 2
#define W4_THREADS 768
#define W4_RBUF (6 * 2 * 32 * W4_RSE)

struct Wino4Params {
  int B, H, W, Cin, x_cs, Cout, y_cs;
  int Ho, Wo, pad;
  int tbx, tby;
  int nblocks;
  int NT32, Q8;
  int act;
  float slope;
  float gate_slope;
  int nt_off;
  int mod, g_cs;
  int gb_off;
  float mod_slope;
  const float* mod_mean;
  const float* mod_invstd;
  int nstage;
  int ksplit, sps;
  long long slab;
  int nitems;
};

__device__ __forceinline__ int w4_xcd_remap(int bid, int nblk) {
  const int q = nblk >> 3, r = nblk & 7;
  const int xcd = bid & 7, idx = bid >> 3;
  return (xcd < r ? xcd * (q + 1) : r * (q + 1) + (xcd - r) * q) + idx;
}


#define WP4_LD 33
template <int RT>
__device__ __forceinline__ void w4_pack_tile(const float* __restrict__ w, int64_t s_n, int64_t s_k, int64_t s_h,
                                             int64_t s_w, int flip, int N, int K, const float* __restrict__ sigma,
                                             int NT32, int Q8, float4* __restrict__ up, int qb, int nt) {
  __shared__ float g[RT][32][WP4_LD];
  const int tid = threadIdx.x;
  const bool k_fast = s_k <= s_n;
  const float sg = sigma != nullptr ? sigma[0] : 1.0f;
  const int lane = tid & 63, ql = tid >> 6;
  const int q = qb * 4 + ql;
  const int nl = lane & 31, h = lane >> 5;
  const float Gp[5] = {0.0f, 1.0f, -1.0f, 0.5f, -2.0f};
  const float Gc[5] = {1.0f, (float)(1.0 / 3.0), (float)(-1.0 / 3.0), (float)(-16.0 / 15.0), (float)(1.0 / 15.0)};
  float G[6][RT];
#pragma unroll
  for (int k = 0; k < 5; ++k) {
    float pw = 1.0f;
#pragma unroll
    for (int a = 0; a < RT; ++a) {
      G[k][a] = (float)((double)Gc[k] * (double)pw);
      pw *= Gp[k];
    }
  }
#pragma unroll
  for (int a = 0; a < RT; ++a) G[5][a] = a == RT - 1 ? 1.0f : 0.0f;
  float stage[RT * RT * 4];
#pragma unroll
  for (int it = 0; it < RT * RT * 4; ++it) {
    const int tap = it >> 2, r = tid + 256 * (it & 3);
    const int nl2 = k_fast ? (r >> 5) : (r & 31), kl = k_fast ? (r & 31) : (r >> 5);
    const int n = nt * 32 + nl2, k = qb * 32 + kl;
    const int a = tap / RT, b = tap - RT * a;
    const int aa = flip ? RT - 1 - a : a, bb = flip ? RT - 1 - b : b;
    stage[it] = (n < N && k < K) ? w[(int64_t)n * s_n + (int64_t)k * s_k + aa * s_h + bb * s_w] : 0.f;
  }
  float t[4][6][RT];
#pragma unroll
  for (int b = 0; b < RT; ++b) {
    if (b) __syncthreads();
#pragma unroll
    for (int it = 0; it < RT * 4; ++it) {
      const int a = it >> 2, r = tid + 256 * (it & 3);
      const int nl2 = k_fast ? (r >> 5) : (r & 31), kl = k_fast ? (r & 31) : (r >> 5);
      const float v = stage[(a * RT + b) * 4 + (it & 3)];
      g[a][nl2][kl] = sigma != nullptr ? v / sg : v;
    }
    __syncthreads();
#pragma unroll
    for (int e = 0; e < 4; ++e) {
      const int kl = 8 * ql + (e >> 1) * 4 + 2 * h + (e & 1);
#pragma unroll
      for (int xi = 0; xi < 6; ++xi) {
        float acc = G[xi][0] * g[0][nl][kl];
#pragma unroll
        for (int a = 1; a < RT; ++a) acc += G[xi][a] * g[a][nl][kl];
        t[e][xi][b] = acc;
      }
    }
  }
  if (q >= Q8) return;
#pragma unroll
  for (int xi = 0; xi < 6; ++xi)
#pragma unroll
    for (int nu = 0; nu < 6; ++nu) {
      float u[4];
#pragma unroll
      for (int e = 0; e < 4; ++e) {
        float acc = t[e][xi][0] * G[nu][0];
#pragma unroll
        for (int b = 1; b < RT; ++b) acc += t[e][xi][b] * G[nu][b];
        u[e] = acc;
      }
      up[(((int64_t)(xi * 6 + nu) * NT32 + nt) * Q8 + q) * 64 + lane] = make_float4(u[0], u[1], u[2], u[3]);
    }
}

template <int RT>
__global__ __launch_bounds__(256) void k_wino4_pack(const float* __restrict__ w, int64_t s_n, int64_t s_k, int64_t s_h,
                                                     int64_t s_w, int flip, int N, int K, const float* __restrict__ sigma,
                                                     int NT32, int Q8, float4* __restrict__ up) {
  w4_pack_tile<RT>(w, s_n, s_k, s_h, s_w, flip, N, K, sigma, NT32, Q8, up, blockIdx.x, blockIdx.y);
}

__global__ __launch_bounds__(256) void k_wino4_pack_multi(PackMulti pm) {
  int i = 0;
  while (i + 1 < pm.n && (int)blockIdx.x >= pm.it[i + 1].start) ++i;
  const PackMultiItem& d = pm.it[i];
  const int local = blockIdx.x - d.start, nqb = (d.Q8 + 3) >> 2;
  w4_pack_tile<3>(d.w, d.s_n, d.s_k, d.s_h, d.s_w, d.flip, d.N, d.K, nullptr, d.NT32, d.Q8, d.up, local % nqb, local / nqb);
}

__device__ __forceinline__ csg_f32x2 w4_pfma(float c, csg_f32x2 a, csg_f32x2 b) {
  return __builtin_elementwise_fma(csg_f32x2{c, c}, a, b);
}

template <int MODE, int NB>
__device__ __forceinline__ void w4_store_columns(const Wino4Params& p, const float* rbuf, int tig, int round, int nt32,
                                                 int img, int X0, int Y0, const float* __restrict__ bias,
                                                 const float* __restrict__ res, const float* __restrict__ gate,
                                                 float* __restrict__ y) {
  for (int item = tig; item < 256 * NB; item += W4_THREADS / 2) {
    const int cq = item & 7, tile = (item >> 3) & 31, bb = item >> 8;
    const int n = nt32 * 32 + cq * 4;
    const int ttx = tile & (W4_TW - 1), tty = tile >> 3;
    const int oy = Y0 + 4 * tty, ox = X0 + 4 * ttx + NB * round + bb;
    if (n < p.Cout && oy < p.Ho && ox < p.Wo) {
      csg_f32x2 lo[6], hi[6];
#pragma unroll
      for (int xi = 0; xi < 6; ++xi) {
        const csg_f32x4 r = *(const csg_f32x4*)(rbuf + ((xi * NB + bb) * 32 + tile) * W4_RSE + cq * 4);
        lo[xi] = __builtin_shufflevector(r, r, 0, 1);
        hi[xi] = __builtin_shufflevector(r, r, 2, 3);
      }
      csg_f32x2 blo = {0.f, 0.f}, bhi = {0.f, 0.f};
      if (bias != nullptr) {
        const csg_f32x4 bv = *(const csg_f32x4*)(bias + n);
        blo = __builtin_shufflevector(bv, bv, 0, 1);
        bhi = __builtin_shufflevector(bv, bv, 2, 3);
      }
      const int64_t rowstride = (int64_t)p.Wo * p.y_cs;
      const int64_t pix0 = ((int64_t)img * p.Ho + oy) * p.Wo + ox;
      int64_t off = pix0 * p.y_cs + n;
      float4 mx[4], mg[4], mm, mr;
      if (MODE == 2) {
        mm = *(const float4*)(p.mod_mean + n);
        mr = *(const float4*)(p.mod_invstd + n);
#pragma unroll
        for (int a = 0; a < 4; ++a) {
          mx[a] = *(const float4*)(res + off + a * rowstride);
          mg[a] = *(const float4*)(gate + (pix0 + (int64_t)a * p.Wo) * p.g_cs + n);
        }
      }
#pragma unroll
      for (int a = 0; a < 4; ++a, off += rowstride) {
        csg_f32x2 vl, vh;
        if (a == 0) {
          vl = ((lo[0] + lo[1]) + (lo[2] + lo[3])) + lo[4];
          vh = ((hi[0] + hi[1]) + (hi[2] + hi[3])) + hi[4];
        } else if (a == 1) {
          vl = w4_pfma(-2.0f, lo[4], w4_pfma(0.5f, lo[3], lo[1] - lo[2]));
          vh = w4_pfma(-2.0f, hi[4], w4_pfma(0.5f, hi[3], hi[1] - hi[2]));
        } else if (a == 2) {
          vl = w4_pfma(4.0f, lo[4], w4_pfma(0.25f, lo[3], lo[1] + lo[2]));
          vh = w4_pfma(4.0f, hi[4], w4_pfma(0.25f, hi[3], hi[1] + hi[2]));
        } else {
          vl = w4_pfma(-8.0f, lo[4], w4_pfma(0.125f, lo[3], lo[1] - lo[2])) + lo[5];
          vh = w4_pfma(-8.0f, hi[4], w4_pfma(0.125f, hi[3], hi[1] - hi[2])) + hi[5];
        }
        vl += blo;
        vh += bhi;
        float vv[4] = {vl.x, vl.y, vh.x, vh.y};
        if (MODE == 2) {
          const float xs[4] = {mx[a].x, mx[a].y, mx[a].z, mx[a].w}, gs[4] = {mg[a].x, mg[a].y, mg[a].z, mg[a].w};
          const float ms[4] = {mm.x, mm.y, mm.z, mm.w}, rs[4] = {mr.x, mr.y, mr.z, mr.w};
#pragma unroll
          for (int e = 0; e < 4; ++e) {
            const float xh = (xs[e] - ms[e]) * rs[e];
            float o = xh * (1.f + gs[e]) + vv[e];
            if (p.mod_slope != 1.0f) o = o > 0.f ? o : o * p.mod_slope;
            vv[e] = o;
          }
        }
        if (MODE == 1) {
#pragma unroll
          for (int e = 0; e < 4; ++e) {
            if (p.act == CSG_ACT_LEAKY)
              vv[e] = vv[e] > 0.f ? vv[e] : vv[e] * p.slope;
            else if (p.act == CSG_ACT_TANH)
              vv[e] = tanhf(vv[e]);
          }
          if (res != nullptr) {
            const float4 rv = *(const float4*)(res + off);
            vv[0] += rv.x; vv[1] += rv.y; vv[2] += rv.z; vv[3] += rv.w;
          }
          if (gate != nullptr) {
            const float4 gv = *(const float4*)(gate + off);
            vv[0] *= gv.x > 0.f ? 1.f : p.gate_slope; vv[1] *= gv.y > 0.f ? 1.f : p.gate_slope;
            vv[2] *= gv.z > 0.f ? 1.f : p.gate_slope; vv[3] *= gv.w > 0.f ? 1.f : p.gate_slope;
          }
        }
        *(float4*)(y + off) = make_float4(vv[0], vv[1], vv[2], vv[3]);
      }
    }
  }
}

__device__ __forceinline__ csg_f32x2 w4_out_row(int a, const csg_f32x2 (&m)[6]) {
  if (a == 0) return ((m[0] + m[1]) + (m[2] + m[3])) + m[4];
  if (a == 1) return w4_pfma(-2.0f, m[4], w4_pfma(0.5f, m[3], m[1] - m[2]));
  if (a == 2) return w4_pfma(4.0f, m[4], w4_pfma(0.25f, m[3], m[1] + m[2]));
  return w4_pfma(-8.0f, m[4], w4_pfma(0.125f, m[3], m[1] - m[2])) + m[5];
}
template <int NB>
__device__ __forceinline__ void w4_store_joint(const Wino4Params& p, const float* rbuf0, int tid, int round, int nb, int img,
                                               int X0, int Y0, const float* __restrict__ bias, const float* __restrict__ xin,
                                               float* __restrict__ gout, float* __restrict__ y) {
  const float* rbuf1 = rbuf0 + W4_RBUF / 2 * NB;
  for (int item = tid; item < 512 * NB; item += W4_THREADS) {
    const int cq = item & 7, tile = (item >> 3) & 31, half = (item >> 8) & 1, bb = item >> 9;
    const int n = nb * 32 + cq * 4;
    const int ttx = tile & (W4_TW - 1), tty = tile >> 3;
    const int oy = Y0 + 4 * tty, ox = X0 + 4 * ttx + NB * round + bb;
    if (oy < p.Ho && ox < p.Wo) {
      csg_f32x2 gl2[2], gh2[2], bl2[2], bh2[2];
      {
        csg_f32x2 lo[6], hi[6];
#pragma unroll
        for (int xi = 0; xi < 6; ++xi) {
          const csg_f32x4 g = *(const csg_f32x4*)(rbuf0 + ((xi * NB + bb) * 32 + tile) * W4_RSE + cq * 4);
          lo[xi] = __builtin_shufflevector(g, g, 0, 1);
          hi[xi] = __builtin_shufflevector(g, g, 2, 3);
        }
        const csg_f32x4 bg = *(const csg_f32x4*)(bias + n);
#pragma unroll
        for (int r = 0; r < 2; ++r) {
          gl2[r] = w4_out_row(2 * half + r, lo) + csg_f32x2{bg.x, bg.y};
          gh2[r] = w4_out_row(2 * half + r, hi) + csg_f32x2{bg.z, bg.w};
        }
      }
      {
        csg_f32x2 lo[6], hi[6];
#pragma unroll
        for (int xi = 0; xi < 6; ++xi) {
          const csg_f32x4 b = *(const csg_f32x4*)(rbuf1 + ((xi * NB + bb) * 32 + tile) * W4_RSE + cq * 4);
          lo[xi] = __builtin_shufflevector(b, b, 0, 1);
          hi[xi] = __builtin_shufflevector(b, b, 2, 3);
        }
        const csg_f32x4 bbv = *(const csg_f32x4*)(bias + p.Cout + n);
#pragma unroll
        for (int r = 0; r < 2; ++r) {
          bl2[r] = w4_out_row(2 * half + r, lo) + csg_f32x2{bbv.x, bbv.y};
          bh2[r] = w4_out_row(2 * half + r, hi) + csg_f32x2{bbv.z, bbv.w};
        }
      }
      const float4 mm = *(const float4*)(p.mod_mean + n), mr = *(const float4*)(p.mod_invstd + n);
      const int64_t rowstride = (int64_t)p.Wo * p.y_cs;
      const int64_t pix0 = ((int64_t)img * p.Ho + oy + 2 * half) * p.Wo + ox;
      const int64_t off = pix0 * p.y_cs + n;
      float4 mx[2];
#pragma unroll
      for (int r = 0; r < 2; ++r) mx[r] = *(const float4*)(xin + off + r * rowstride);
#pragma unroll
// ... 450 lines not shown
      w4_epilogue<1>(acc, pe, smem + W4V_V0, tid_o, wave, grp, tid_o & 31, (tid_o >> 5) & 1, nt32, img, X0, Y0, ka->bias,
                     ka->res, ka->gate, ka->y);
    } else if (T == 4) {
      w4_epilogue<2>(acc, p, smem, tid, wave, grp, j, h, nt32, img, X0, Y0, bias, res, gate, y);
    } else {
      w3_epilogue(acc, p, smem, tid, wave, grp, j, h, nt32, img, X0, Y0, bias, res, gate, y);
    }
    if (!P || !more) break;
    v = item_n;
    nb = nb_n; img = img_n; X0 = X0_n; Y0 = Y0_n;
    nt32 = p.gb_off ? nb + grp * p.gb_off : nb * 2 + grp;
    ubase = ubase_nxt;
    tsel ^= 1;
    __syncthreads();
    produce(0, 0);
    __syncthreads();
  }
#undef W4_TAB
}

template <int T>
constexpr size_t w4_lds = (size_t)(W4Geo<T>::OFFTAB + W4_THREADS * 4) * 4;

static int w4_plan(const csg_wino_desc* d, int T, int pad, Wino4Params& p, size_t& shm, const char* who) {
  int rc = wino_desc_check(d, who, 36, [](const csg_wino_desc& d) { return (int64_t)d.B * (d.H + 1) * (d.W + 1); });
  if (rc == CSG_OK) rc = wino_conv_dense_x(d, who);
  if (rc) return rc;
  if (T == 4)
    CSG_REQUIRE(d->H % 4 == 0 && d->W % 4 == 0 && d->W >= 32 && d->H >= 16, CSG_E_UNSUPPORTED,
                "%s: F(4x4,3x3) needs H=%d, W=%d multiples of 4, W >= 32, H >= 16", who, d->H, d->W);
  else
    CSG_REQUIRE((pad == 1 || pad == 2) && d->H + 2 * pad >= 4 && d->W + 2 * pad >= 4, CSG_E_UNSUPPORTED,
                "%s: F(3x3,4x4) serves pad 1 or 2 (got %d) on maps of at least 4 - 2 pad pixels", who, pad);
  const int Ho = T == 4 ? d->H : d->H + 2 * pad - 3, Wo = T == 4 ? d->W : d->W + 2 * pad - 3;
  CSG_REQUIRE(d->Cin % 8 == 0, CSG_E_UNSUPPORTED, "%s: Cin must be a multiple of 8 (one LDS stage)", who);
  p.B = d->B; p.H = d->H; p.W = d->W; p.Cin = d->Cin; p.x_cs = d->x_cs; p.Cout = d->Cout; p.y_cs = d->y_cs;
  p.Ho = Ho; p.Wo = Wo; p.pad = pad;
  p.tbx = (Wo + T * W4_TW - 1) / (T * W4_TW);
  p.tby = (Ho + T * W4_TH - 1) / (T * W4_TH);
  p.nblocks = (d->Cout + 63) / 64;
  p.NT32 = (d->Cout + 31) / 32;
  p.Q8 = (d->Cin + 7) / 8;
  p.act = d->act; p.slope = d->slope; p.gate_slope = 0.f;
  p.nt_off = 0; p.mod = 0; p.g_cs = 0; p.gb_off = 0; p.mod_slope = 1.f; p.mod_mean = nullptr; p.mod_invstd = nullptr;
  p.nstage = d->Cin / W4_PS;
  p.ksplit = 1;
  p.sps = p.nstage;
  p.slab = (long long)d->B * Ho * Wo * d->y_cs;
  p.nitems = 0;
  shm = T == 4 ? w4_lds<4> : w4_lds<3>;
  return CSG_OK;
}

static std::atomic<int> w4_persist_on{-1};
static int w4_persistent_blocks(const Wino4Params& p, int64_t items) {
  static std::atomic<int> cus[32];
  int on = w4_persist_on.load(std::memory_order_relaxed);
  if (on < 0) {
    on = getenv("CSG_WINO4_PERSIST") ? atoi(getenv("CSG_WINO4_PERSIST")) : 1;
    int expect = -1;
    w4_persist_on.compare_exchange_strong(expect, on);
    on = w4_persist_on.load(std::memory_order_relaxed);
  }
  int dev = 0;
  (void)hipGetDevice(&dev);
  if (!on || dev < 0) return 0;
  int ncu = dev < 32 ? cus[dev].load(std::memory_order_relaxed) : 0;
  if (ncu == 0) {
    if (hipDeviceGetAttribute(&ncu, hipDeviceAttributeMultiprocessorCount, dev) != hipSuccess || ncu < 8) ncu = -1;
    if (dev < 32) cus[dev].store(ncu, std::memory_order_relaxed);
  }
  const int g = ncu > 0 ? (ncu & ~7) : 0;
  if (g == 0 || p.ksplit != 1 || (p.nstage & 1) || p.nstage < 4 || (p.gb_off == 0 && (p.Cout & 63)) || items < 2 * (int64_t)g) return 0;
  return g;
}

template <int T>
static int w4_launch(Wino4Params& p, size_t shm, const float* x, const float* packed, const float* bias,
                     const float* residual, const float* gate, float* y, hipStream_t s, const char* who) {
  const int64_t grid = (int64_t)p.B * p.tby * p.tbx * p.nblocks * p.ksplit;
  CSG_REQUIRE(grid < (1ll << 31), CSG_E_UNSUPPORTED, "%s: grid too large", who);
  p.nitems = (int)grid;
  const int pblocks = T == 4 ? w4_persistent_blocks(p, grid) : 0;
  static_assert(w4_lds<T> <= 128 * 1024, "k_wino4_conv_v: one block per CU with room for the persistent form's table");
  int rc = pblocks ? lds_limit<k_wino4_conv_v<4, true>, w4_lds<4> + W4_THREADS * 16>(shm + W4_THREADS * 16, who)
                   : lds_limit<k_wino4_conv_v<T, false>, w4_lds<T>>(shm, who);
  if (rc) return rc;
  if (pblocks)
    CSG_LAUNCH((k_wino4_conv_v<4, true>), dim3((unsigned)pblocks), dim3(W4_THREADS), shm + W4_THREADS * 16, s, p, x,
               (const float4*)packed, bias, residual, gate, y);
  else
    CSG_LAUNCH((k_wino4_conv_v<T, false>), dim3((unsigned)grid), dim3(W4_THREADS), shm, s, p, x, (const float4*)packed, bias,
               residual, gate, y);
  return check_launch(who);
}

#define W4_SPLIT 32, 16

template <int T>
static int w4_conv(const char* who, const csg_wino_desc* d, int pad, const WinoConvArgs& a) {
  return wino_conv_entry<Wino4Params>(
      who, "csg_wino4_conv(slab sum)", d, W4_SPLIT, K_WINO4_CONV, T == 4 ? 9.0 : 16.0, a,
      [&](Wino4Params& p, size_t& shm) { return w4_plan(d, T, pad, p, shm, who); },
      [&](Wino4Params& p, size_t shm, float* y) {
        return w4_launch<T>(p, shm, a.x, a.packed, a.bias, a.residual, a.gate, y, a.s, who);
      });
}

extern "C" {

int32_t csg_wino4_supported(const csg_wino_desc* d) {
  static const int on = getenv("CSG_WINO4") ? atoi(getenv("CSG_WINO4")) : 1;
  if (!on || d == nullptr) return 0;
  return (d->H % 4 == 0 && d->W % 4 == 0 && d->W >= 32 && d->H >= 16 && d->Cin % 8 == 0 && d->Cout % 4 == 0) ? 1 : 0;
}

int csg_wino4_pack_multi_launch(const PackMulti* pm, int blocks, double bytes, hipStream_t s) {
  ProfScope ps(K_WINO_PACK, bytes, s);
  CSG_LAUNCH(k_wino4_pack_multi, dim3((unsigned)blocks), dim3(256), 0, s, *pm);
  return check_launch("csg_wino_pack_weights_multi(F(4x4,3x3))");
}

int csg_wino_pack_weights_multi(const csg_wino_pack_item* items, int32_t n, void* stream) {
  CSG_REQUIRE(n >= 0 && (items != nullptr || n == 0), CSG_E_BADSHAPE, "csg_wino_pack_weights_multi: bad arguments");
  hipStream_t s = (hipStream_t)stream;
  for (int variant = 2; variant <= 4; variant += 2) {
    PackMulti pm;
    int cnt = 0, blocks = 0;
    double bytes = 0.0;
    auto flush = [&]() -> int {
      if (cnt == 0) return CSG_OK;
      pm.n = cnt;
      const int rc = variant == 4 ? csg_wino4_pack_multi_launch(&pm, blocks, bytes, s)
                                  : csg_wino2_pack_multi_launch(&pm, blocks, bytes, s);
      cnt = 0;
      blocks = 0;
      bytes = 0.0;
      return rc;
    };
    for (int i = 0; i < n; ++i) {
      const csg_wino_pack_item& it = items[i];
      CSG_REQUIRE(it.variant == 2 || it.variant == 4, CSG_E_UNSUPPORTED,
                  "csg_wino_pack_weights_multi: item %d: variant %d (2 = F(2x2,3x3), 4 = F(4x4,3x3))", i, it.variant);
      if (it.variant != variant) continue;
      CSG_REQUIRE(it.w != nullptr && it.packed != nullptr && it.Cout > 0 && it.Cin > 0 && ((uintptr_t)it.packed % 16) == 0,
                  CSG_E_BADSHAPE, "csg_wino_pack_weights_multi: item %d: bad arguments", i);
      const int64_t N = it.backward_data ? it.Cin : it.Cout, K = it.backward_data ? it.Cout : it.Cin;
      const int64_t s_n = it.backward_data ? it.s_i : it.s_o, s_k = it.backward_data ? it.s_o : it.s_i;
      const int64_t span = (it.Cout - 1) * it.s_o + (it.Cin - 1) * it.s_i + 2 * it.s_h + 2 * it.s_w;
      CSG_REQUIRE(span < (1ll << 31) && s_n >= 0 && s_k >= 0 && it.s_h >= 0 && it.s_w >= 0, CSG_E_UNSUPPORTED,
                  "csg_wino_pack_weights_multi: item %d: weight too large for 32-bit element offsets", i);
      const int NT32 = (int)cdiv(N, 32), Q8 = (int)cdiv(K, 8);
      const int nb = (int)cdiv(Q8, 4) * NT32;
      if (cnt == CSG_PACK_MULTI || blocks + nb > (1 << 20)) {
        const int rc = flush();
        if (rc) return rc;
      }
      PackMultiItem& d = pm.it[cnt++];
      d.w = it.w; d.up = (float4*)it.packed;
      d.s_n = (int)s_n; d.s_k = (int)s_k; d.s_h = (int)it.s_h; d.s_w = (int)it.s_w;
      d.flip = it.backward_data ? 1 : 0; d.N = (int)N; d.K = (int)K; d.NT32 = NT32; d.Q8 = Q8;
      d.start = blocks;
      blocks += nb;
      bytes += (double)it.Cout * it.Cin * 9 * 4 + (double)(variant == 4 ? 36 : 16) * NT32 * Q8 * 64 * 16;
    }
    const int rc = flush();
    if (rc) return rc;
  }
  return CSG_OK;
}

int32_t csg_wino4_persistent(int32_t on) {
  const int prev = w4_persist_on;
  if (on >= 0) w4_persist_on = on != 0;
  return prev;
}

int64_t csg_wino4_pack_bytes(int64_t N, int64_t K) { return wino_pack_bytes(36, N, K); }

int csg_wino4_pack_weights(const float* w, int64_t s_o, int64_t s_i, int64_t s_h, int64_t s_w, int64_t Cout, int64_t Cin,
                           int32_t backward_data, const float* sigma, float* packed, void* stream) {
  return wino_pack_entry("csg_wino4_pack_weights", 36, 9, w, s_o, s_i, s_h, s_w, Cout, Cin, backward_data, sigma, packed, stream,
                         [](dim3 grid, hipStream_t s, auto... a) { CSG_LAUNCH(k_wino4_pack<3>, grid, dim3(256), 0, s, a...); });
}

int csg_wino34_pack_weights(const float* w, int64_t s_o, int64_t s_i, int64_t s_h, int64_t s_w, int64_t Cout, int64_t Cin,
                            int32_t backward_data, const float* sigma, float* packed, void* stream) {
  return wino_pack_entry("csg_wino34_pack_weights", 36, 16, w, s_o, s_i, s_h, s_w, Cout, Cin, backward_data, sigma, packed, stream,
                         [](dim3 grid, hipStream_t s, auto... a) { CSG_LAUNCH(k_wino4_pack<4>, grid, dim3(256), 0, s, a...); });
}

int32_t csg_wino34_supported(const csg_wino_desc* d, int32_t pad) {
  static const int on = getenv("CSG_WINO34") ? atoi(getenv("CSG_WINO34")) : 1;
  if (!on || d == nullptr) return 0;
  return ((pad == 1 || pad == 2) && d->H >= 15 && d->W >= 15 && d->Cin % 8 == 0 && d->Cout % 4 == 0 && d->Cin >= 64 &&
          d->Cout >= 32) ? 1 : 0;
}

int64_t csg_wino34_conv_workspace(const csg_wino_desc* d, int32_t pad) {
  return wino_conv_workspace<Wino4Params>(
      d, W4_SPLIT, [&](Wino4Params& p, size_t& shm) { return w4_plan(d, 3, pad, p, shm, "csg_wino34_conv_workspace"); });
}

int csg_wino34_conv(const csg_wino_desc* d, int32_t pad, const float* x, const float* packed, const float* bias,
                    const float* residual, const float* gate, float gate_slope, float* y, float* workspace,
                    int64_t workspace_bytes, void* stream) {
  return w4_conv<3>("csg_wino34_conv", d, pad,
                    {x, packed, bias, residual, gate, gate_slope, y, workspace, workspace_bytes, (hipStream_t)stream});
}

int64_t csg_wino4_conv_workspace(const csg_wino_desc* d) {
  return wino_conv_workspace<Wino4Params>(
      d, W4_SPLIT, [&](Wino4Params& p, size_t& shm) { return w4_plan(d, 4, 1, p, shm, "csg_wino4_conv_workspace"); });
}

int csg_wino4_conv(const csg_wino_desc* d, const float* x, const float* packed, const float* bias, const float* residual,
                   const float* gate, float gate_slope, float* y, float* workspace, int64_t workspace_bytes, void* stream) {
  return w4_conv<4>("csg_wino4_conv", d, 1,
                    {x, packed, bias, residual, gate, gate_slope, y, workspace, workspace_bytes, (hipStream_t)stream});
}

int csg_wino4_conv_part(const csg_wino_desc* d, const float* x, const float* packed, int64_t tile_off, int64_t tiles_total,
                        const float* bias, const float* mod_x, const float* mod_gamma, int64_t gamma_cs,
                        const float* mod_mean, const float* mod_invstd, float mod_slope, float* y, void* stream) {
  Wino4Params p;
  size_t shm = 0;
  int rc = w4_plan(d, 4, 1, p, shm, "csg_wino4_conv_part");
  if (rc) return rc;
  CSG_REQUIRE(d->act == CSG_ACT_NONE, CSG_E_UNSUPPORTED, "csg_wino4_conv_part: no activation (the modulation has its own)");
  CSG_REQUIRE(tile_off >= 0 && tiles_total >= tile_off + p.NT32 && d->Cout % 32 == 0, CSG_E_BADSHAPE,
              "csg_wino4_conv_part: tiles [%ld, %ld) of %ld with Cout=%d", (long)tile_off, (long)(tile_off + p.NT32),
              (long)tiles_total, d->Cout);
  CSG_REQUIRE((int64_t)36 * tiles_total * p.Q8 * 1024 < CSG_MAX_RECORDS, CSG_E_UNSUPPORTED,
              "csg_wino4_conv_part: packed weights too large for 32-bit byte offsets");
  p.nt_off = (int)tile_off;
  p.NT32 = (int)tiles_total;
  if (mod_x != nullptr) {
    CSG_REQUIRE(mod_gamma != nullptr && mod_mean != nullptr && mod_invstd != nullptr && gamma_cs >= d->Cout &&
                    gamma_cs % 4 == 0,
                CSG_E_BADSHAPE, "csg_wino4_conv_part: the modulation needs gamma, mean, invstd");
    CSG_REQUIRE(((uintptr_t)mod_x % 16) == 0 && ((uintptr_t)mod_gamma % 16) == 0 && ((uintptr_t)mod_mean % 16) == 0 &&
                    ((uintptr_t)mod_invstd % 16) == 0,
                CSG_E_UNSUPPORTED, "csg_wino4_conv_part: pointers must be 16-byte aligned");
    p.mod = 1; p.g_cs = (int)gamma_cs; p.mod_slope = mod_slope; p.mod_mean = mod_mean; p.mod_invstd = mod_invstd;
  }
  CSG_REQUIRE(((uintptr_t)x % 16) == 0 && ((uintptr_t)packed % 16) == 0 && ((uintptr_t)y % 16) == 0 &&
                  (bias == nullptr || ((uintptr_t)bias % 16) == 0),
              CSG_E_UNSUPPORTED, "csg_wino4_conv_part: pointers must be 16-byte aligned");
  hipStream_t s = (hipStream_t)stream;
  ProfScope ps(K_WINO4_CONV, 2.0 * p.B * p.H * p.W * 9.0 * p.Cin * p.Cout, s);
  return w4_launch<4>(p, shm, x, packed, bias, mod_x, mod_gamma, y, s, "csg_wino4_conv_part");
}

static int w4_spade_plan(const csg_wino_desc* d, Wino4Params& p, size_t& shm, const char* who) {
  CSG_REQUIRE(d != nullptr && d->Cout % 32 == 0, CSG_E_UNSUPPORTED, "%s: C must be a multiple of 32", who);
  int rc = w4_plan(d, 4, 1, p, shm, who);
  if (rc) return rc;
  const int tiles = d->Cout / 32;
  p.NT32 = 2 * tiles;
  p.nblocks = tiles;
  p.gb_off = tiles;
  p.mod = 2;
  const int64_t items = (int64_t)p.B * p.tby * p.tbx * p.nblocks;
  CSG_REQUIRE(items < (1ll << 31) && w4_persistent_blocks(p, items) > 0, CSG_E_UNSUPPORTED,
              "%s: the launch does not qualify for the persistent form (%ld items, %d stages)", who, (long)items, p.nstage);
  return CSG_OK;
}

int32_t csg_wino4_conv_spade_supported(const csg_wino_desc* d) {
  if (!csg_wino4_supported(d)) return 0;
  Wino4Params p;
  size_t shm = 0;
  const int rc = w4_spade_plan(d, p, shm, "csg_wino4_conv_spade_supported");
  return rc == CSG_OK ? 1 : 0;
}

int csg_wino4_conv_spade(const csg_wino_desc* d, const float* x, const float* packed, const float* bias, const float* mod_x,
                         float* gamma_out, int64_t gamma_cs, const float* mod_mean, const float* mod_invstd, float mod_slope,
                         float* y, void* stream) {
  Wino4Params p;
  size_t shm = 0;
  int rc = w4_spade_plan(d, p, shm, "csg_wino4_conv_spade");
  if (rc) return rc;
  CSG_REQUIRE(d->act == CSG_ACT_NONE, CSG_E_UNSUPPORTED, "csg_wino4_conv_spade: no activation (the modulation has its own)");
  CSG_REQUIRE(bias != nullptr && mod_x != nullptr && mod_mean != nullptr && mod_invstd != nullptr,
              CSG_E_BADSHAPE, "csg_wino4_conv_spade: needs the 2C biases, x, mean, invstd");
  CSG_REQUIRE(gamma_out == nullptr || (gamma_cs >= d->Cout && gamma_cs % 4 == 0 && ((uintptr_t)gamma_out % 16) == 0),
              CSG_E_BADSHAPE, "csg_wino4_conv_spade: bad gamma buffer");
  const int tiles = d->Cout / 32;
  CSG_REQUIRE((int64_t)36 * 2 * tiles * p.Q8 * 1024 < CSG_MAX_RECORDS, CSG_E_UNSUPPORTED,
              "csg_wino4_conv_spade: packed weights too large for 32-bit byte offsets");
  CSG_REQUIRE(((uintptr_t)x % 16) == 0 && ((uintptr_t)packed % 16) == 0 && ((uintptr_t)y % 16) == 0 && ((uintptr_t)bias % 16) == 0 &&
                  ((uintptr_t)mod_x % 16) == 0 && ((uintptr_t)mod_mean % 16) == 0 && ((uintptr_t)mod_invstd % 16) == 0,
              CSG_E_UNSUPPORTED, "csg_wino4_conv_spade: pointers must be 16-byte aligned");
  p.g_cs = (int)gamma_cs; p.mod_slope = mod_slope; p.mod_mean = mod_mean; p.mod_invstd = mod_invstd;
  hipStream_t s = (hipStream_t)stream;
  ProfScope ps(K_WINO4_CONV, 2.0 * p.B * p.H * p.W * 9.0 * p.Cin * 2.0 * p.Cout, s);
  return w4_launch<4>(p, shm, x, packed, bias, mod_x, gamma_out, y, s, "csg_wino4_conv_spade");
}

}
```

canonicalsg2im_amd/ops.py:

```python
import collections
import ctypes
import os

import torch
import torch.distributed as dist
import torch.nn.functional as F
from torch.optim.optimizer import register_optimizer_step_post_hook as _register_optimizer_step_post_hook

from . import _lib
from . import dist as csg_dist
from ._lib import ACT_LEAKY, ACT_NONE, ACT_TANH, ConvDesc, FewDesc, GemmDesc, HingeItem, WinoDesc, WinoPackItem, check, lib, ptr, stream

__all__ = [
    "nhwc", "empty_nhwc", "conv2d", "linear", "norm_act", "upsample2x", "nearest_resize", "avgpool3s2", "embed", "real_object_mask",
    "norm_act_pair", "graph_csr", "gather_concat", "segment_avg", "layout_pyramid", "layout_paint", "disc_input", "crop_objects", "maxpool2", "avgpool2", "l1_mean",
    "invalidate_weight_caches", "pack_conv_weight", "wino_pack", "prepack_weights", "wino_eligible", "wino_variant", "plan_conv", "spectral_weight", "spectral_weights", "spade_infer", "norm_eval_stats", "deprocess_u8", "preprocess_images", "pack_frozen_forward", "ACT_NONE", "ACT_LEAKY", "ACT_TANH",
    "conv2d_forward", "pool3", "spatial_mean", "resize_bilinear", "feat_stats", "feat_stats_finalize", "softmax_rows", "inception_score", "POOL_MAX", "POOL_AVG9", "POOL_AVG_INSIDE",
    "crop_windows", "crop_resize_bilinear", "kid_sums", "feat_class_sums", "knn_radii", "ball_counts",
    "augment_table", "augment_table_host", "d_augment",
    "augment_gate", "augment_gate_host", "ada_accumulate", "ada_update", "ada_update_host",
]


def nhwc(t):
    if t.permute(0, 2, 3, 1).is_contiguous():
        return t
    return t.permute(0, 2, 3, 1).contiguous().permute(0, 3, 1, 2)


def empty_nhwc(B, C, H, W, device, zero=False):
    f = torch.zeros if zero else torch.empty
    return f((B, H, W, C), device=device, dtype=torch.float32).permute(0, 3, 1, 2)


def _f32(t):
    if t.dtype != torch.float32:
        raise RuntimeError("canonicalsg2im_amd kernels compute in fp32; got %s" % t.dtype)
    return t


_NORM_BLOCKS = int(os.environ.get("CSG_NORM_BLOCKS", "1024"))


def _chunks(P, G=1):
    c = max(1, min(P // 32, max(1, _NORM_BLOCKS // max(G, 1))))
    return int(c)


def _desc_forward(B, IH, IW, Cin, Cout, KH, KW, stride, pad, act=ACT_NONE, slope=0.0, x_cs=None, y_cs=None):
    d = ConvDesc()
    d.B, d.IHp, d.IWp, d.Cin, d.x_cs = B, IH, IW, Cin, (Cin if x_cs is None else x_cs)
    d.IHv, d.IWv, d.in_up = IH, IW, 0
    OH = (IH + 2 * pad - KH) // stride + 1
    OW = (IW + 2 * pad - KW) // stride + 1
    d.OHg, d.OWg, d.OHf, d.OWf, d.os, d.ooy, d.oox = OH, OW, OH, OW, 1, 0, 0
    d.Cout, d.y_cs = Cout, (Cout if y_cs is None else y_cs)
    d.istride, d.ntaps, d.wtaps = stride, KH * KW, KH * KW
    for ky in range(KH):
        for kx in range(KW):
            s = ky * KW + kx
            d.tap_dy[s], d.tap_dx[s], d.tap_w[s] = ky - pad, kx - pad, s
    d.act, d.slope, d.accumulate = act, slope, 0
    return d, OH, OW


def _descs_backward_data(B, IH, IW, Cin, Cout, KH, KW, stride, pad, OH, OW):
    out = []
    for py in range(stride):
        for px in range(stride):
            gh = (IH - py + stride - 1) // stride
            gw = (IW - px + stride - 1) // stride
            if gh <= 0 or gw <= 0:
                continue
            d = ConvDesc()
            d.B, d.IHp, d.IWp, d.Cin, d.x_cs = B, OH, OW, Cout, Cout
            d.IHv, d.IWv, d.in_up = OH, OW, 0
            d.OHg, d.OWg, d.OHf, d.OWf, d.os, d.ooy, d.oox = gh, gw, IH, IW, stride, py, px
            d.Cout, d.y_cs = Cin, Cin
            d.istride, d.wtaps = 1, KH * KW
            n = 0
            for ky in range(KH):
                if (py + pad - ky) % stride:
                    continue
                for kx in range(KW):
                    if (px + pad - kx) % stride:
                        continue
                    d.tap_dy[n], d.tap_dx[n], d.tap_w[n] = (py + pad - ky) // stride, (px + pad - kx) // stride, ky * KW + kx
                    n += 1
            d.ntaps = n
            d.act, d.slope, d.accumulate = ACT_NONE, 0.0, 0
            out.append(d)
    return out


def _conv_launch(d, x, w, bias, res, y, what):
    nbytes = lib.csg_conv_fwd_workspace(d)
    if nbytes < 0:
        raise RuntimeError("conv_fwd_workspace: " + _lib.last_error())
    ws = torch.empty(nbytes // 4, device=x.device, dtype=torch.float32) if nbytes > 0 else None
    y_ptr = y if isinstance(y, ctypes.c_void_p) else ptr(y)
    check(lib.csg_conv_fwd(d, ptr(x), ptr(w), ptr(bias), ptr(res), y_ptr, ptr(ws), nbytes, stream()), what)


def _conv_launch_classes(descs, x, w, y_ptr, what):
    if len(descs) == 1:
        return _conv_launch(descs[0], x, w, None, None, y_ptr, what)
    arr = (ConvDesc * len(descs))(*descs)
    nbytes = lib.csg_conv_fwd_multi_workspace(arr, len(descs))
    if nbytes < 0:
        raise RuntimeError("conv_fwd_multi_workspace: " + _lib.last_error())
    ws = torch.empty(nbytes // 4, device=x.device, dtype=torch.float32) if nbytes > 0 else None
    check(lib.csg_conv_fwd_multi(arr, len(descs), ptr(x), ptr(w), None, None, y_ptr, ptr(ws), nbytes, stream()), what)


FEW_ENABLED = os.environ.get("CSG_FEW_OUTPUT_KERNELS", "1") != "0"
WINO_MIN_PIXELS = int(os.environ.get("CSG_WINO_MIN_PIXELS", "1024"))
WINO_ENABLED = os.environ.get("CSG_WINOGRAD", "1") != "0"
WINO_WGRAD = os.environ.get("CSG_WINOGRAD_WGRAD", "1") != "0"
WINO4_WGRAD = os.environ.get("CSG_WINO4_WGRAD", "1") != "0"
WINO4_WGRAD_MIN_PIXELS = int(os.environ.get("CSG_WINO4_WGRAD_MIN_PIXELS", "64"))

GEMM_MODE = os.environ.get("CSG_GEMM", "auto")
GEMM_MIN_TILES = int(os.environ.get("CSG_GEMM_MIN_TILES", "256"))
_GEMM_CALLS = [0]


def gemm_calls():
    return _GEMM_CALLS[0]


def gemm_eligible(M, N, K):
    if GEMM_MODE in ("off", "0") or K % 4 or N % 4 or K < 32:
        return False
    if ((M + 127) // 128) * ((N + 127) // 128) < GEMM_MIN_TILES:
        return False
    return GEMM_MODE == "all" or (N <= 256 <= K)


def _gemm_nt(a, M, K, w2, N, bias, act, slope, gate, gate_slope, y):
    d = GemmDesc()
    d.M, d.N, d.K, d.lda, d.ldb, d.ldy, d.ldg = M, N, K, K, K, N, N
    d.act, d.slope, d.gate_slope = act, slope, gate_slope
    check(lib.csg_gemm_nt(d, ptr(a), ptr(w2), ptr(bias), ptr(gate), ptr(y), stream()), "gemm_nt")
    _GEMM_CALLS[0] += 1



def wino_eligible(B, H, W, Cin, Cout, KH, KW, stride, pad):
    enough = B * H * W >= WINO_MIN_PIXELS
    return (WINO_ENABLED and KH == 3 and KW == 3 and stride == 1 and pad == 1 and H % 2 == 0 and W % 2 == 0 and W >= 8
            and Cin % 16 == 0 and Cout % 4 == 0 and Cout >= 32 and enough)


def _wino_desc(B, H, W, Cin, Cout, act=ACT_NONE, slope=0.0):
    d = WinoDesc()
    d.B, d.H, d.W, d.Cin, d.x_cs, d.Cout, d.y_cs, d.act, d.slope = B, H, W, Cin, Cin, Cout, Cout, act, slope
    return d


WINO4_MIN_ITEMS = int(os.environ.get("CSG_WINO4_MIN_ITEMS", "160"))


def wino_variant(B, H, W, Cin, Cout, plain=False):
    d = _wino_desc(B, H, W, Cin, Cout)
    if lib.csg_wino4_supported(d) != 1:
        return 2
    items = B * ((H + 15) // 16) * ((W + 31) // 32) * ((Cout + 63) // 64)
    if items < WINO4_MIN_ITEMS and not (plain and lib.csg_wino4_conv_workspace(d) > 0):
        return 2
# ... 391 lines not shown
                     "wino34_conv_bwd_data", gate=gate, gate_slope=gate_slope, variant=34, pad=3 - pad, may_split=in_act is None)
        gated = True
    elif fam == "gemm":
        wt = w.detach().reshape(Cout, Cin).t().contiguous()
        dx = empty_nhwc(B, Cin, IH, IW, dev)
        _gemm_nt(dpre, B * IH * IW, Cout, wt, Cin, None, ACT_NONE, 0.0, gate, gate_slope, dx)
        gated = True
    elif fam == "direct":
        wt = packs.bwd if packs is not None else w.detach().permute(1, 2, 3, 0).contiguous()
        dx = empty_nhwc(B, Cin, IH, IW, dev)
        descs = _descs_backward_data(B, IH, IW, Cin, Cout, KH, KW, stride, pad, OH, OW)
        if in_act is not None and len(descs) == 1:
            d = descs[0]
            d.res_gate, d.slope = 1, gate_slope
            _conv_launch(d, dpre, wt, None, x, dx, "conv_bwd_data")
            gated = True
        else:
            _conv_launch_classes(descs, dpre, wt, ptr(dx), "conv_bwd_data")
    if dx is not None and not gated:
        check(lib.csg_act_bwd(ptr(dx), ptr(x), dx.numel(), in_act[0], in_act[1], ptr(dx), stream()), "act_bwd")
    want_db = plan.has_bias and need[2]
    wg = plan.wgrad
    if not need[1] and wg != "few":
        wg = "colsum" if want_db else None
    if wg == "few":
        nbytes = lib.csg_conv_few_bwd_weight_workspace(plan.few)
        ws = torch.empty(nbytes // 4, device=dev, dtype=torch.float32)
        dwp = torch.empty((Cout, KH, KW, Cin), device=dev, dtype=torch.float32)
        db = torch.empty(Cout, device=dev, dtype=torch.float32) if plan.has_bias else None
        check(lib.csg_conv_few_bwd_weight(plan.few, ptr(x), ptr(dpre), ptr(dwp), ptr(db), ptr(ws), nbytes, stream()),
              "conv_few_bwd_weight")
        dw = dwp[:w.shape[0]].permute(0, 3, 1, 2)
        db = db[:w.shape[0]] if db is not None else None
    elif wg == "gemm_tn":
        M = B * IH * IW
        nbytes = lib.csg_gemm_tn_workspace(M, Cout, Cin)
        if nbytes < 0:
            raise RuntimeError("gemm_tn_workspace: (%d, %d, %d) not served" % (M, Cout, Cin))
        ws = torch.empty(max(nbytes // 4, 4), device=dev, dtype=torch.float32)
        dwp, db = _weight_grad_dest(w, Cout, KH, KW, Cin, want_db, dev)
        check(lib.csg_gemm_tn(M, Cout, Cin, ptr(dpre), Cout, ptr(x), Cin, ptr(dwp), ptr(db), ptr(ws), nbytes, stream()),
              "gemm_tn")
        _GEMM_CALLS[0] += 1
        dw = dwp.permute(0, 3, 1, 2)
    elif wg in ("wino4w", "wino"):
        ws = torch.empty(plan.wgrad_ws // 4, device=dev, dtype=torch.float32)
        dwp, db = _weight_grad_dest(w, Cout, KH, KW, Cin, want_db, dev)
        fn, what = (lib.csg_wino4_bwd_weight, "wino4_bwd_weight") if wg == "wino4w" else (lib.csg_wino_bwd_weight, "wino_bwd_weight")
        check(fn(_wino_desc(B, IH, IW, Cin, Cout), ptr(x), ptr(dpre), ptr(dwp), ptr(db), ptr(ws), plan.wgrad_ws, stream()), what)
        dw = dwp.permute(0, 3, 1, 2)
    elif wg == "direct":
        d, _, _ = _desc_forward(B, IH, IW, Cin, Cout, KH, KW, stride, pad)
        nbytes = lib.csg_conv_bwd_weight_workspace(d)
        if nbytes < 0:
            raise RuntimeError("conv_bwd_weight_workspace: " + _lib.last_error())
        ws = torch.empty(max(nbytes // 4, 4), device=dev, dtype=torch.float32)
        dwp, db = _weight_grad_dest(w, Cout, KH, KW, Cin, want_db, dev)
        check(lib.csg_conv_bwd_weight(d, ptr(x), ptr(dpre), ptr(dwp), ptr(db), ptr(ws), nbytes, stream()), "conv_bwd_weight")
        dw = dwp.permute(0, 3, 1, 2)
    elif wg == "colsum":
        rows = B * OH * OW
        nch = _chunks(rows)
        part = torch.empty(nch * 2 * Cout, device=dev, dtype=torch.float64)
        db = torch.empty(Cout, device=dev, dtype=torch.float32)
        check(lib.csg_colsum(ptr(dpre), rows, Cout, Cout, ptr(db), ptr(part), nch, stream()), "colsum")
    return dx, dw, db


class _Conv2d(torch.autograd.Function):

    @staticmethod
    def forward(ctx, x, weight, bias, residual, stride, pad, act, slope, packs=None, dx_range=None, in_act=None,
                grad_is_pre=False, cout_real=None, pre_slope=None):
        x = nhwc(_f32(x))
        B, Cin, IH, IW = x.shape
        Cout, _, KH, KW = weight.shape
        res = nhwc(residual) if residual is not None else None
        ctx.plan = plan_conv(B, IH, IW, Cin, Cout, KH, KW, stride, pad, act, slope, bias is not None, res is not None, packs,
                             dx_range, in_act, cout_real, pre_slope, ctx.needs_input_grad[:3])
        y, ctx.ut_pre = _conv_fwd(ctx.plan, x, weight, bias, res, packs)
        ctx.packs, ctx.grad_is_pre, ctx.has_res = packs, grad_is_pre, res is not None
        ctx.save_for_backward(x, weight, y if act != ACT_NONE else None)
        return y

    @staticmethod
    def backward(ctx, dy):
        x, weight, y = ctx.saved_tensors
        dy = nhwc(dy)
        dx, dw, db = _conv_bwd(ctx.plan, dy, x, weight, None if ctx.grad_is_pre else y, ctx.needs_input_grad[:3], ctx.packs,
                               ctx.ut_pre)
        dres = dy if (ctx.has_res and ctx.needs_input_grad[3]) else None
        return dx, dw, db, dres, None, None, None, None, None, None, None, None, None, None


FrozenPacks = collections.namedtuple("FrozenPacks", "fwd bwd wino_fwd wino_bwd cache", defaults=(None, None, None))


def pack_conv_weight(weight):
    pc = (-weight.shape[1]) % 4
    w = F.pad(weight.detach(), (0, 0, 0, 0, 0, pc)) if pc else weight.detach()
    fwd, bwd = w.permute(0, 2, 3, 1).contiguous(), w.permute(1, 2, 3, 0).contiguous()
    if WINO_ENABLED and w.shape[2] == 3 and w.shape[3] == 3 and w.shape[0] % 4 == 0:
        return FrozenPacks(fwd, bwd, wino_pack(w, False), wino_pack(w, True), {"w": w})
    return FrozenPacks(fwd, bwd)


def _frozen_pack(packs, backward_data, variant):
    if variant == 2:
        return packs.wino_bwd if backward_data else packs.wino_fwd
    key = ("bwd" if backward_data else "fwd", variant)
    if key not in packs.cache:
        packs.cache[key] = wino_pack(packs.cache["w"], backward_data, None, variant)
    return packs.cache[key]


def conv2d(x, weight, bias=None, stride=1, padding=0, act=ACT_NONE, slope=0.0, residual=None, packs=None,
           dx_range=None, in_act=None, grad_is_pre=False, pre_slope=None):
    Cout, Cin = weight.shape[0], weight.shape[1]
    pc, po = (-Cin) % 4, (-Cout) % 4
    if residual is not None and act != ACT_NONE:
        raise NotImplementedError("conv2d: a fused residual needs act == ACT_NONE")
    if packs is not None and po:
        raise RuntimeError("conv2d: packed weights need an output-channel count that is a multiple of 4")
    if packs is not None and pc and weight.requires_grad and torch.is_grad_enabled():
        raise RuntimeError("conv2d: packs= needs a frozen weight when the input channels (%d) are padded" % Cin)
    if pc:
        if x.shape[1] == Cin:
            x = F.pad(x, (0, 0, 0, 0, 0, pc))
        if packs is None:
            weight = F.pad(weight, (0, 0, 0, 0, 0, pc))
    few_raw = False
    if (po and Cout + po == 4 and not pc and residual is None and packs is None and dx_range is None and in_act is None
            and x.dim() == 4 and x.is_cuda):
        few_raw = plan_conv(x.shape[0], x.shape[2], x.shape[3], Cin, 4, weight.shape[2], weight.shape[3], int(stride),
                            int(padding), int(act), float(slope), cout_real=Cout).fwd == "few"
    if pre_slope is not None and not (few_raw and x.shape[1] < 256):
        x, pre_slope = F.leaky_relu(x, float(pre_slope)), None
    if po and not few_raw:
        weight = F.pad(weight, (0, 0, 0, 0, 0, 0, 0, po))
        bias = F.pad(bias, (0, po)) if bias is not None else None
        residual = F.pad(residual, (0, 0, 0, 0, 0, po)) if residual is not None else None
    if dx_range is not None and (dx_range[0] % 4 or dx_range[1] % 4 or pc):
        raise RuntimeError("conv2d: dx_range must be 4-aligned channel bounds of an unpadded input")
    if in_act is not None and (pc or dx_range is not None or in_act[0] != ACT_LEAKY):
        raise RuntimeError("conv2d: in_act needs an unpadded input, no dx_range and a (Leaky)ReLU producer")
    if grad_is_pre and po:
        raise RuntimeError("conv2d: grad_is_pre needs an unpadded output")
    y = _Conv2d.apply(x, weight, bias, residual, int(stride), int(padding), int(act), float(slope), packs, dx_range,
                      in_act, bool(grad_is_pre), Cout if Cout + po == 4 else None,
                      None if pre_slope is None else float(pre_slope))
    return y[:, :Cout] if po else y


def linear(x, weight, bias=None, act=ACT_NONE, slope=0.0, in_act=None, grad_is_pre=False):
    lead = x.shape[:-1]
    K = x.shape[-1]
    N = weight.shape[0]
    x2 = x.reshape(-1, K)
    if not x2.is_contiguous():
        x2 = x2.contiguous()
    y = conv2d(x2.view(-1, K, 1, 1), weight.view(N, K, 1, 1), bias, 1, 0, act, slope, in_act=in_act, grad_is_pre=grad_is_pre)
    return y.reshape(*lead, N)


class _SpectralWeight(torch.autograd.Function):

    @staticmethod
    def forward(ctx, iterate, eps, *wuv):
        n = len(wuv) // 3
        ws = [_f32(wuv[3 * i]).contiguous() for i in range(n)]
        items = (_lib.SnFwdItem * n)()
        outs, smalls, keep = [], [], []
        for i, w in enumerate(ws):
            u, v = wuv[3 * i + 1], wuv[3 * i + 2]
            Cout = w.shape[0]
            K = w.numel() // Cout
            nbytes = lib.csg_spectral_norm_workspace(Cout, K)
            if nbytes < 0:
                raise RuntimeError("spectral_weight: weight (%d x %d) needs K %% 4 == 0" % (Cout, K))
            wsb = torch.empty(nbytes // 4, device=w.device, dtype=torch.float32)
            cl = w.shape[1] if (w.dim() == 4 and w.shape[1] % 4 == 0 and w.shape[2] * w.shape[3] > 1
                               and w.shape[2] * w.shape[3] * (w.shape[1] + 4) * 4 <= 65536) else 0
            w_eff = torch.empty_like(w, memory_format=torch.channels_last) if cl else torch.empty_like(w)
            small = torch.empty(1 + Cout + K, device=w.device, dtype=torch.float32)
            it = items[i]
            it.w, it.u, it.v, it.Cout, it.K = w.data_ptr(), u.data_ptr(), v.data_ptr(), Cout, K
            it.w_eff, it.cl_Cin = w_eff.data_ptr(), cl
            it.sigma, it.u_used, it.v_used = small.data_ptr(), small.data_ptr() + 4, small.data_ptr() + 4 * (1 + Cout)
            it.workspace, it.workspace_bytes = wsb.data_ptr(), nbytes
            outs.append(w_eff)
            smalls.append(small)
            keep.append(wsb)
        check(lib.csg_spectral_norm_fwd_multi(items, n, 1 if iterate else 0, eps, stream()), "spectral_norm_fwd_multi")
        ctx.n = n
        ctx.set_materialize_grads(False)
        ctx.save_for_backward(*ws, *smalls)
        return tuple(outs)

    @staticmethod
    def backward(ctx, *dweffs):
        n = ctx.n
        ws, smalls = ctx.saved_tensors[:n], ctx.saved_tensors[n:]
        idx = [i for i in range(n) if dweffs[i] is not None and ctx.needs_input_grad[2 + 3 * i]]
        grads = [None] * (2 + 3 * n)
        if not idx:
            return tuple(grads)
        items = (_lib.SnBwdItem * len(idx))()
        keep = []
        for j, i in enumerate(idx):
            w, small = ws[i], smalls[i]
            Cout = w.shape[0]
            K = w.numel() // Cout
            Cin, KH, KW = (w.shape[1], w.shape[2], w.shape[3]) if w.dim() == 4 else (K, 1, 1)
            dweff = _f32(dweffs[i])
            if dweff.dim() != 4:
                dweff = dweff.contiguous()
            st = dweff.stride() if dweff.dim() == 4 else (K, 1, 1, 1)
            if not _rows_dense(st, (Cin, KH, KW), K):
                dweff = dweff.contiguous()
                st = dweff.stride() if dweff.dim() == 4 else (K, 1, 1, 1)
            nbytes = lib.csg_spectral_norm_workspace(Cout, K)
            wsb = torch.empty(nbytes // 4, device=w.device, dtype=torch.float32)
            dw = _grad_dest(w, tuple(w.shape))
            if dw is None:
                dw = torch.empty_like(w)
            it = items[j]
            it.dweff, it.Cout, it.Cin, it.KH, it.KW = dweff.data_ptr(), Cout, Cin, KH, KW
            it.s0, it.s1, it.s2, it.s3 = st[0], st[1], st[2], st[3]
            it.w, it.sigma = w.data_ptr(), small.data_ptr()
            it.u_used, it.v_used = small.data_ptr() + 4, small.data_ptr() + 4 * (1 + Cout)
            it.dw, it.workspace, it.workspace_bytes = dw.data_ptr(), wsb.data_ptr(), nbytes
            keep += [dweff, wsb]
            grads[2 + 3 * i] = dw
        check(lib.csg_spectral_norm_bwd_multi(items, len(idx), stream()), "spectral_norm_bwd_multi")
        return tuple(grads)


def spectral_weights(wuv, iterate, eps=1e-12):
    flat = [t for triple in wuv for t in triple]
    for t in flat:
        if not t.is_cuda:
            raise RuntimeError("canonicalsg2im_amd ops need HIP (cuda) tensors; there is no CPU path")
    return list(_SpectralWeight.apply(bool(iterate), float(eps), *flat))


def _rows_dense(st, dims, K):
    run = 1
    for i in sorted(range(3), key=lambda i: st[1 + i]):
        if dims[i] > 1 and st[1 + i] != run:
            return False
        run *= dims[i]
    return st[0] == K


def spectral_weight(w, u, v, iterate, eps=1e-12):
    return spectral_weights([(w, u, v)], iterate, eps)[0]


def _sync_world():
    return dist.get_world_size() if (dist.is_available() and dist.is_initialized()) else 1


def _multi(world, syncs):
    return bool(syncs) and (world > 1 or csg_dist.active())


def _drop_clamped_invstd_term(dsums, invstd, eps, C):
    live = invstd < (float(eps) ** -0.5) * (1.0 - 1e-6)
    dsums.view(-1, 2 * C)[:, C:].mul_(live.to(dsums.dtype))
    return dsums


def _nothing():
    return None


class _Norm:

    __slots__ = ("G", "P", "C", "count", "eps", "multi", "nch")

    def __init__(self, x, G, eps, syncs):
        B, C, H, W = x.shape
        world = _sync_world() if syncs else 1
        self.G, self.P, self.C, self.eps = G, (B * H * W) // G, C, eps
        self.multi = _multi(world, syncs)
        self.count = float(self.P * world)
        self.nch = _chunks(self.P, G)

    @staticmethod
    def _exchange(sums, overlap):
        if overlap:
            return csg_dist.all_reduce_stats_async(sums)
        csg_dist.all_reduce_stats(sums)
        return None

    def stats(self, x, momentum, running, overlap=False):
        G, P, C, dev = self.G, self.P, self.C, x.device
        mean = torch.empty(G * C, device=dev, dtype=torch.float32)
        invstd = torch.empty(G * C, device=dev, dtype=torch.float32)
        part = torch.empty(G * self.nch * 2 * C, device=dev, dtype=torch.float64)
        running = [(rm, rv if rm is not None else None) for rm, rv in running]
        if not self.multi:
            (rm0, rv0), (rm1, rv1) = (running + [(None, None)])[:2]
            check(lib.csg_norm_stats_finalize(ptr(x), G, P, C, ptr(part), self.nch, self.count, self.eps, ptr(mean), ptr(invstd),
                                              ptr(rm0), ptr(rv0), ptr(rm1), ptr(rv1), momentum, stream()), "norm_stats_finalize")
            return mean, invstd, _nothing
# ... 1962 lines not shown
```

canonicalsg2im_amd/spade/models/networks/generator.py:

```python
import torch.nn as nn

from .... import ops
from .... import spectral_norm as csg_spectral_norm
from ....sg2im.attribute_embed import AttributeEmbeddings
from ....sg2im.layers import Conv2d, GlobalAvgPool, build_cnn, build_mlp
from ....sg2im.utils import real_object_mask
from .architecture import SPADEResnetBlock
from .base_network import BaseNetwork
from .normalization import SegPyramid


class AppearanceEncoder(nn.Module):

    def __init__(self, vocab, arch, normalization='none', activation='relu', padding='same', vecs_size=1024,
                 pooling='avg'):
        super().__init__()
        self.vocab = vocab
        cnn, channels = build_cnn(arch=arch, normalization=normalization, activation=activation, pooling=pooling,
                                  padding=padding)
        self.cnn = nn.Sequential(cnn, GlobalAvgPool(), nn.Linear(channels, vecs_size))

    def forward(self, crops):
        return self.cnn(crops)


_BLOCKS = (("head_0", 16, 16), ("G_middle_0", 16, 16), ("G_middle_1", 16, 16),
           ("up_0", 16, 8), ("up_1", 8, 4), ("up_2", 4, 2), ("up_3", 2, 1))
_LATENT_HALVINGS = {'normal': 5, 'more': 6, 'most': 7}


class SPADEGenerator(BaseNetwork):

    def __init__(self, opt):
        super().__init__()
        if opt.use_vae:
            raise NotImplementedError("--use_vae is never wired in the reference trainer (SURVEY.md §2 row 22)")
        self.attribute_embedding = AttributeEmbeddings(opt.vocab['attributes'], opt.embedding_dim)
        self.opt = opt
        nf = opt.ngf
        self.sw, self.sh = self.compute_latent_vector_size(opt)
        self.fc = Conv2d(opt.semantic_nc, 16 * nf, 3, padding=1)
        blocks = list(_BLOCKS)
        if opt.num_upsampling_layers == 'most':
            blocks.append(("up_4", 1, 0.5))
        for name, win, wout in blocks:
            setattr(self, name, SPADEResnetBlock(int(win * nf), int(wout * nf), opt))
        self._block_names = [b[0] for b in blocks]
        self.conv_img = Conv2d(int(blocks[-1][2] * nf), 3, 3, padding=1, act=ops.ACT_TANH)
        self.up = nn.Upsample(scale_factor=2)
        self.repr_input = opt.g_mask_dim
        self.repr_net = build_mlp([self.repr_input, 64, opt.rep_size], batch_norm=opt.mlp_normalization)
        self.image_encoder = AppearanceEncoder(vocab=opt.vocab, arch='C4-64-2,C4-128-2,C4-256-2', padding='valid',
                                               normalization=opt.appearance_normalization,
                                               activation=opt.a_activation, vecs_size=opt.g_mask_dim)

    def compute_latent_vector_size(self, opt):
        if opt.num_upsampling_layers not in _LATENT_HALVINGS:
            raise ValueError('opt.num_upsampling_layers [%s] not recognized' % opt.num_upsampling_layers)
        sw = opt.image_size[0] >> _LATENT_HALVINGS[opt.num_upsampling_layers]
        return sw, round(sw / opt.aspect_ratio)

    def forward(self, objs, layout_boxes, layout_masks, test_mode=False):
        if self.sw != self.sh:
            raise NotImplementedError("aspect_ratio != 1 is not on the hot path")
        csg_spectral_norm.prepare(self)
        ops.prepack_weights(self)
        H = self.opt.image_size[0]
        levels = [self.sw << k for k in range(H.bit_length()) if (self.sw << k) <= H]
        valid = real_object_mask(objs, self.opt.vocab)
        if layout_masks is not None and test_mode:
            maps = ops.layout_paint(self.attribute_embedding(objs), layout_boxes, valid, layout_masks, H, levels)
        else:
            maps = ops.layout_pyramid(self.attribute_embedding(objs), layout_boxes, valid, H, levels, masks=layout_masks)
        seg = SegPyramid(zip(levels, maps))
        x = self.fc(seg.at(self.sw))
        no_upsample = {"head_0"} | (set() if self.opt.num_upsampling_layers in ('more', 'most') else {"G_middle_1"})
        for name in self._block_names:
            if name not in no_upsample:
                x = ops.upsample2x(x)
            x = getattr(self, name)(x, seg)
        return self.conv_img(x, pre_slope=2e-1)
```

canonicalsg2im_amd/spade/models/networks/normalization.py:

```python
import re

import torch
import torch.nn as nn

from .... import ops
from ....spectral_norm import spectral_norm
from ....sg2im.layers import Conv2d, _FusedActivation
from .sync_batchnorm import LocalBatchNorm2d, SynchronizedBatchNorm2d


class SegPyramid:

    def __init__(self, levels):
        self.levels = dict(levels)

    def at(self, h):
        return self.levels[int(h)]


class InstanceNormAct(nn.InstanceNorm2d):

    def __init__(self, num_features, fused_slope=1.0):
        super().__init__(num_features, affine=False)
        self.fused_slope = fused_slope

    def forward(self, x, gb=None, fused_slope=None):
        slope = self.fused_slope if fused_slope is None else fused_slope
        return ops.norm_act(x, gb, None, None, instance=True, training=self.training, slope=slope, eps=self.eps)


class SyncBatchNormAct(SynchronizedBatchNorm2d):

    def __init__(self, num_features, fused_slope=1.0):
        super().__init__(num_features, affine=True)
        self.fused_slope = fused_slope

    def forward(self, x):
        return super().forward(x, None, self.fused_slope)


def get_nonspade_norm_layer(opt, norm_type='instance'):
    use_sn = norm_type.startswith('spectral')
    after = norm_type[len('spectral'):] if use_sn else norm_type

    def wrap(conv):
        if use_sn:
            conv = spectral_norm(conv)
        if after in ('', 'none'):
            return conv
        if after not in ('instance', 'batch', 'sync_batch'):
            raise ValueError('normalization layer %s is not recognized' % after)
        if getattr(conv, 'bias', None) is not None:
            del conv.bias
            conv.register_parameter('bias', None)
        width = getattr(conv, 'out_channels', None) or conv.weight.size(0)
        if after == 'batch':
            from ....sg2im.layers import BatchNormAct
            return nn.Sequential(conv, BatchNormAct(width))
        if after == 'sync_batch':
            return nn.Sequential(conv, SyncBatchNormAct(width))
        return nn.Sequential(conv, InstanceNormAct(width))

    return wrap


class _JoinedPair(torch.autograd.Function):

    @staticmethod
    def forward(ctx, a, b, joined):
        ctx.n = a.shape[0]
        return joined.view_as(joined)

    @staticmethod
    def backward(ctx, g):
        return g[:ctx.n], g[ctx.n:], None


def _join_storage(pa, pb):
    cl = pa.dim() == 4
    joined = torch.empty((2 * pa.shape[0],) + tuple(pa.shape[1:]), device=pa.device, dtype=pa.dtype)
    if cl:
        joined = joined.contiguous(memory_format=torch.channels_last)
    n = pa.shape[0]
    with torch.no_grad():
        joined[:n].copy_(pa)
        joined[n:].copy_(pb)
    pa.data = joined[:n]
    pb.data = joined[n:]
    return joined


def _joined(mod, name, pa, pb):
    j = getattr(mod, name, None)
    n = pa.shape[0]
    if (j is None or j.device != pa.device or pa.data_ptr() != j.data_ptr() or
            pb.data_ptr() != j.data_ptr() + n * j.stride(0) * j.element_size() or pa.stride() != j.stride()
            or pb.stride() != j.stride()):
        j = _join_storage(pa, pb)
        object.__setattr__(mod, name, j)
    return _JoinedPair.apply(pa, pb, j)


def _training_batchnorm(pn):
    return isinstance(pn, (SynchronizedBatchNorm2d, LocalBatchNorm2d)) and not pn.affine and pn.training


class SPADE(nn.Module):
    def __init__(self, config_text, norm_nc, label_nc):
        super().__init__()
        assert config_text.startswith('spade')
        parsed = re.search(r'spade(\D+)(\d)x\d', config_text)
        kind, ks = str(parsed.group(1)), int(parsed.group(2))
        if kind == 'instance':
            self.param_free_norm = InstanceNormAct(norm_nc)
        elif kind == 'syncbatch':
            self.param_free_norm = SynchronizedBatchNorm2d(norm_nc, affine=False)
        elif kind == 'batch':
            self.param_free_norm = LocalBatchNorm2d(norm_nc, affine=False)
        else:
            raise ValueError('%s is not a recognized param-free norm type in SPADE' % kind)
        nhidden = 128
        self.pw = ks // 2
        self.mlp_shared = nn.Sequential(Conv2d(label_nc, nhidden, kernel_size=ks, padding=self.pw,
                                               act=ops.ACT_LEAKY, slope=0.0), _FusedActivation())
        self.mlp_gamma = Conv2d(nhidden, norm_nc, kernel_size=ks, padding=self.pw)
        self.mlp_beta = Conv2d(nhidden, norm_nc, kernel_size=ks, padding=self.pw)

    def forward(self, x, segmap, fused_slope=1.0):
        if self.fusable(x):
            return ops.spade_fused(x, [self.fused_operands(x, segmap, fused_slope)], self.param_free_norm.eps,
                                   self.param_free_norm.momentum, getattr(self.param_free_norm, "sync", True))[0]
        pn = self.param_free_norm
        if self.joinable(x):
            actv, w, b, rm, rv, slope, in_slope = self.fused_operands(x, segmap, fused_slope)
            return ops.spade_joined(x, actv, w, b, rm, rv, self.pw, slope, in_slope, pn.eps, pn.momentum,
                                    getattr(pn, "sync", True))
        return pn(x, gb=self.modulation(x, segmap), fused_slope=fused_slope)

    def joinable(self, x):
        return (ops.SPADE_JOINED and _training_batchnorm(self.param_free_norm) and x.dim() == 4 and x.is_cuda
                and self.mlp_gamma.weight.shape[0] % 4 == 0)

    def fusable(self, x):
        return (_training_batchnorm(self.param_free_norm)
                and ops.spade_fused_eligible(x, self.mlp_gamma.weight.shape[1], self.mlp_gamma.weight.shape[0],
                                             self.mlp_gamma.weight.shape[2]))

    def joined_weight(self):
        _joined(self, "_joined_w", self.mlp_gamma.weight, self.mlp_beta.weight)
        return self.__dict__.get("_joined_w")

    def _conv_operands(self, x, segmap):
        if isinstance(segmap, SegPyramid):
            seg = segmap.at(x.size(2))
        else:
            seg = segmap if segmap.shape[2:] == x.shape[2:] else ops.nearest_resize(segmap, x.shape[2:])
        sh = self.mlp_shared[0]
        actv = ops.conv2d(seg, sh.weight, sh.bias, 1, sh.padding[0], sh.act, sh.slope, grad_is_pre=True)
        w = _joined(self, "_joined_w", self.mlp_gamma.weight, self.mlp_beta.weight)
        b = _joined(self, "_joined_b", self.mlp_gamma.bias, self.mlp_beta.bias)
        return actv, w, b

    def fused_operands(self, x, segmap, slope):
        pn = self.param_free_norm
        return self._conv_operands(x, segmap) + (pn.running_mean, pn.running_var, slope, self.mlp_shared[0].slope)

    def modulation(self, x, segmap):
        actv, w, b = self._conv_operands(x, segmap)
        sh = self.mlp_shared[0]
        return ops.conv2d(actv, w, b, 1, self.pw, in_act=(sh.act, sh.slope))


def spade_pair(norm_a, norm_b, x, segmap, slope_a, slope_b):
    pa, pb = norm_a.param_free_norm, norm_b.param_free_norm
    same = (type(pa) is type(pb) and _training_batchnorm(pa) and _training_batchnorm(pb) and pa.eps == pb.eps
            and pa.momentum == pb.momentum and getattr(pa, "sync", True) == getattr(pb, "sync", True) and x.dim() == 4)
    if not same:
        return norm_a(x, segmap, fused_slope=slope_a), norm_b(x, segmap, fused_slope=slope_b)
    if norm_a.fusable(x) and norm_b.fusable(x):
        ya, yb = ops.spade_fused(x, [norm_a.fused_operands(x, segmap, slope_a), norm_b.fused_operands(x, segmap, slope_b)],
                                 pa.eps, pa.momentum, getattr(pa, "sync", True))
        return ya, yb
    return ops.norm_act_pair(x, norm_a.modulation(x, segmap), norm_b.modulation(x, segmap), pa.running_mean, pa.running_var,
                             pb.running_mean, pb.running_var, slope_a, slope_b, pa.eps, pa.momentum,
                             getattr(pa, "sync", True))
```

include/csg_hip.h:

```cpp
#ifndef CSG_HIP_H
#define CSG_HIP_H

#include <stdint.h>

#ifdef __cplusplus
extern "C" {
#endif

#define CSG_OK 0
#define CSG_E_BADSHAPE (-1)
#define CSG_E_UNSUPPORTED (-2)
#define CSG_E_LAUNCH (-3)
#define CSG_E_WORKSPACE (-4)

#define CSG_ACT_NONE 0
#define CSG_ACT_LEAKY 1
#define CSG_ACT_TANH 2

#define CSG_MAX_TAPS 16

int csg_version(void);
const char* csg_last_error(void);

int csg_prof_enable(int mode);
int csg_prof_reset(void);
int csg_prof_num_kernels(void);
const char* csg_prof_kernel_name(int kernel_id);
int csg_prof_read(int kernel_id, double* ms, int64_t* launches, double* work);

int csg_embed_fwd(const int64_t* idx, int64_t rows, int64_t idx_stride, const float* table, int64_t num_emb,
                  int64_t dim, float* out, int64_t out_stride, int64_t out_off, void* stream);
int64_t csg_embed_bwd_workspace(int64_t rows, int64_t num_emb, int64_t dim);
int csg_embed_bwd(const int64_t* idx, int64_t rows, int64_t idx_stride, const float* dout, int64_t out_stride,
                  int64_t out_off, int64_t num_emb, int64_t dim, float* dtable, float* workspace, int64_t workspace_bytes,
                  void* stream);

int csg_real_object_mask(const int64_t* objs, int64_t B, int64_t O, int64_t A, int64_t image_id, uint8_t* mask,
                         void* stream);

int csg_graph_csr_build(const int64_t* triplets, int64_t B, int64_t T, int64_t O, int32_t* row_ptr, int32_t* col,
                        void* stream);
int64_t csg_graph_csr_lds(int64_t T, int64_t O);

int csg_gather_concat_fwd(const float* obj, const float* pred, const int64_t* triplets, int64_t B, int64_t O,
                          int64_t T, int64_t Din, int64_t Dp, float* out, void* stream);
int64_t csg_gather_concat_bwd_workspace(int64_t B, int64_t O, int64_t T, int64_t Din);
int csg_gather_concat_bwd(const float* dcat, const int32_t* row_ptr, const int32_t* col, int64_t B, int64_t O,
                          int64_t T, int64_t Din, int64_t Dp, float* dobj, float* dpred, void* workspace,
                          int64_t workspace_bytes, void* stream);

int64_t csg_segment_avg_fwd_workspace(int64_t B, int64_t O, int64_t T, int64_t H);
int csg_segment_avg_fwd(const float* h, const float* conf, const uint8_t* valid, const int32_t* row_ptr,
                        const int32_t* col, int64_t B, int64_t O, int64_t T, int64_t H, int64_t Dp, float* pooled,
                        float* cnt, float* new_p, void* workspace, int64_t workspace_bytes, void* stream);
int csg_segment_avg_bwd(const float* dpooled, const float* dnew_p, const float* h, const float* conf,
                        const uint8_t* valid, const int64_t* triplets, const float* pooled, const float* cnt,
                        int64_t B, int64_t O, int64_t T, int64_t H, int64_t Dp, int32_t gate_relu, float* dh,
                        float* dconf, float* dcnt_scratch, void* stream);

int csg_layout_fwd(const float* vecs, const float* boxes, const uint8_t* valid, const float* masks, int64_t M,
                   int64_t B, int64_t O, int64_t S, int64_t H, int64_t W, int64_t OH, int64_t OW, float* out,
                   int64_t out_cs, int64_t out_off, void* stream);
int csg_disc_input_fwd(const float* vecs, const float* boxes, const uint8_t* valid, const float* masks, int64_t M, int64_t B,
                       int64_t O, int64_t S, int64_t H, int64_t W, const float* img, int64_t img_sb, int64_t img_sc,
                       int64_t img_sh, int64_t img_sw, float* out, int64_t out_cs, void* stream);
int64_t csg_layout_bwd_workspace(int64_t B, int64_t O, int64_t S, int64_t OH, int64_t OW, int32_t has_masks,
                                 int32_t box_gradients);
int csg_layout_bwd(const float* dout, int64_t out_cs, int64_t out_off, const float* boxes, const uint8_t* valid,
                   const float* masks, int64_t M, int64_t B, int64_t O, int64_t S, int64_t H, int64_t W, int64_t OH,
                   int64_t OW, float* dvecs, int accumulate, const float* vecs, float* dboxes, void* workspace,
                   int64_t workspace_bytes, void* stream);
int csg_layout_bwd_masks(const float* dout, int64_t out_cs, int64_t out_off, const float* boxes, const uint8_t* valid,
                         int64_t M, int64_t B, int64_t O, int64_t S, int64_t H, int64_t W, int64_t OH, int64_t OW,
                         const float* vecs, float* dmasks, int accumulate, void* stream);
int csg_layout_mass(const float* vecs, const float* boxes, const uint8_t* valid, const float* masks, int64_t M,
                    int64_t B, int64_t O, int64_t S, int64_t H, int64_t W, float* mass, void* stream);
int csg_layout_paint(const float* vecs, const float* boxes, const float* masks, int64_t M, const int32_t* order,
                     int64_t B, int64_t O, int64_t S, int64_t H, int64_t W, int64_t OH, int64_t OW, float* out,
                     int64_t out_cs, int64_t out_off, void* stream);

typedef struct csg_conv_desc {
  int32_t B, IHp, IWp, Cin, x_cs;
  int32_t IHv, IWv, in_up;
  int32_t OHg, OWg, OHf, OWf, os, ooy, oox;
  int32_t Cout, y_cs;
  int32_t istride, ntaps, wtaps;
  int32_t tap_dy[CSG_MAX_TAPS], tap_dx[CSG_MAX_TAPS], tap_w[CSG_MAX_TAPS];
  int32_t act;
  float slope;
  int32_t accumulate;
  int32_t res_gate;
} csg_conv_desc;

int64_t csg_conv_fwd_workspace(const csg_conv_desc* d);
int csg_conv_fwd(const csg_conv_desc* d, const float* x, const float* w, const float* bias, const float* residual,
                 float* y, float* workspace, int64_t workspace_bytes, void* stream);
int64_t csg_conv_fwd_multi_workspace(const csg_conv_desc* descs, int32_t n);
int csg_conv_fwd_multi(const csg_conv_desc* descs, int32_t n, const float* x, const float* w, const float* bias,
                       const float* residual, float* y, float* workspace, int64_t workspace_bytes, void* stream);
int64_t csg_conv_bwd_weight_workspace(const csg_conv_desc* d);
int csg_conv_bwd_weight(const csg_conv_desc* d, const float* x, const float* dy, float* dw, float* db,
                        float* workspace, int64_t workspace_bytes, void* stream);

typedef struct csg_wino_desc {
  int32_t B, H, W;
  int32_t Cin, x_cs;
  int32_t Cout, y_cs;
  int32_t act;
  float slope;
} csg_wino_desc;
int64_t csg_wino_pack_bytes(int64_t N, int64_t K);
int csg_wino_pack_weights(const float* w, int64_t s_o, int64_t s_i, int64_t s_h, int64_t s_w, int64_t Cout, int64_t Cin,
                          int32_t backward_data, const float* sigma, float* packed, void* stream);
int64_t csg_wino_conv_workspace(const csg_wino_desc* d);
int csg_wino_conv(const csg_wino_desc* d, const float* x, const float* packed, const float* bias,
                  const float* residual, const float* gate, float gate_slope, float* y, float* workspace,
                  int64_t workspace_bytes, void* stream);
int64_t csg_wino_bwd_weight_workspace(const csg_wino_desc* d);
int csg_wino_bwd_weight(const csg_wino_desc* d, const float* x, const float* dy, float* dw, float* db, float* workspace,
                        int64_t workspace_bytes, void* stream);

int64_t csg_wino4_bwd_weight_workspace(const csg_wino_desc* d);
int csg_wino4_bwd_weight(const csg_wino_desc* d, const float* x, const float* dy, float* dw, float* db, float* workspace,
                         int64_t workspace_bytes, void* stream);

int32_t csg_wino4_supported(const csg_wino_desc* d);
typedef struct csg_wino_pack_item {
  const float* w;
  int64_t s_o, s_i, s_h, s_w;
  int64_t Cout, Cin;
  int32_t backward_data;
  int32_t variant;
  float* packed;
} csg_wino_pack_item;
int csg_wino_pack_weights_multi(const csg_wino_pack_item* items, int32_t n, void* stream);
int32_t csg_wino4_persistent(int32_t on);
int64_t csg_wino4_pack_bytes(int64_t N, int64_t K);
int csg_wino4_pack_weights(const float* w, int64_t s_o, int64_t s_i, int64_t s_h, int64_t s_w, int64_t Cout, int64_t Cin,
                           int32_t backward_data, const float* sigma, float* packed, void* stream);
int64_t csg_wino4_conv_workspace(const csg_wino_desc* d);
int csg_wino4_conv(const csg_wino_desc* d, const float* x, const float* packed, const float* bias,
                   const float* residual, const float* gate, float gate_slope, float* y, float* workspace,
                   int64_t workspace_bytes, void* stream);

int csg_wino4_conv_part(const csg_wino_desc* d, const float* x, const float* packed, int64_t tile_off, int64_t tiles_total,
                        const float* bias, const float* mod_x, const float* mod_gamma, int64_t gamma_cs,
                        const float* mod_mean, const float* mod_invstd, float mod_slope, float* y, void* stream);

int32_t csg_wino4_conv_spade_supported(const csg_wino_desc* d);
int csg_wino4_conv_spade(const csg_wino_desc* d, const float* x, const float* packed, const float* bias, const float* mod_x,
                         float* gamma_out, int64_t gamma_cs, const float* mod_mean, const float* mod_invstd, float mod_slope,
                         float* y, void* stream);

int32_t csg_wino34_supported(const csg_wino_desc* d, int32_t pad);
int csg_wino34_pack_weights(const float* w, int64_t s_o, int64_t s_i, int64_t s_h, int64_t s_w, int64_t Cout, int64_t Cin,
                            int32_t backward_data, const float* sigma, float* packed, void* stream);
int64_t csg_wino34_conv_workspace(const csg_wino_desc* d, int32_t pad);
int csg_wino34_conv(const csg_wino_desc* d, int32_t pad, const float* x, const float* packed, const float* bias,
                    const float* residual, const float* gate, float gate_slope, float* y, float* workspace,
                    int64_t workspace_bytes, void* stream);

typedef struct csg_few_desc {
  int32_t B, IH, IW;
  int32_t Cin, x_cs;
  int32_t KH, KW, pad;
  int32_t cout_real;
  int32_t act;
  float slope;
  int32_t in_act;
  float in_slope;
} csg_few_desc;
int csg_conv_few_supported(const csg_few_desc* d);
int64_t csg_conv_few_fwd_workspace(const csg_few_desc* d);
int csg_conv_few_fwd(const csg_few_desc* d, const float* x, const float* w, const float* bias, float* y, float* workspace,
                     int64_t workspace_bytes, void* stream);
int csg_conv_few_bwd_data(const csg_few_desc* d, const float* dy, const float* w, float* dx, void* stream);
int64_t csg_conv_few_bwd_weight_workspace(const csg_few_desc* d);
int csg_conv_few_bwd_weight(const csg_few_desc* d, const float* x, const float* dy, float* dw, float* db,
                            float* workspace, int64_t workspace_bytes, void* stream);

typedef struct csg_gemm_desc {
  int64_t M, N, K;
  int64_t lda, ldb, ldy, ldg;
  int32_t act;
  float slope;
  float gate_slope;
} csg_gemm_desc;
int csg_gemm_supported(const csg_gemm_desc* d);
int csg_gemm_nt(const csg_gemm_desc* d, const float* a, const float* bw, const float* bias, const float* gate, float* y,
                void* stream);
int64_t csg_gemm_tn_workspace(int64_t M, int64_t N, int64_t K);
int csg_gemm_tn(int64_t M, int64_t N, int64_t K, const float* dy, int64_t ldy, const float* x, int64_t ldx, float* dw,
                float* db, float* workspace, int64_t workspace_bytes, void* stream);

int csg_act_bwd(const float* dy, const float* y, int64_t n, int32_t act, float slope, float* dpre, void* stream);
int csg_colsum(const float* x, int64_t rows, int64_t C, int64_t x_cs, float* out, double* partial, int64_t nchunk,
               void* stream);

int csg_norm_stats(const float* x, int64_t G, int64_t P, int64_t C, double* sums, double* partial, int64_t nchunk,
                   void* stream);
int csg_norm_finalize(const double* sums, int64_t G, int64_t C, double count, float eps, int32_t mode, float* mean,
                      float* invstd, float* running_mean, float* running_var, float momentum, void* stream);
int csg_norm_stats_finalize(const float* x, int64_t G, int64_t P, int64_t C, double* partial, int64_t nchunk, double count,
                            float eps, float* mean, float* invstd, float* running_mean, float* running_var,
                            float* running_mean2, float* running_var2, float momentum, void* stream);
int csg_norm_apply_fwd(const float* x, const float* mean, const float* invstd, const float* gb, float slope,
                       int64_t G, int64_t P, int64_t C, float* y, const float* gb2, float slope2, float* y2,
                       void* stream);
typedef struct csg_norm_eval_item {
  const float* running_mean;
  const float* running_var;
  int64_t C;
  int64_t offset;
} csg_norm_eval_item;
int csg_norm_eval_stats_multi(const csg_norm_eval_item* items, int32_t n, float eps, float* out, void* stream);
int csg_norm_apply_bwd_reduce(const float* dy, const float* x, const float* mean, const float* invstd,
                              const float* gb, const float* yact, float slope, int64_t G, int64_t P, int64_t C, float* dgb,
                              double* dsums, double* partial, int64_t nchunk, int64_t gb_cs, void* stream);
int csg_norm_apply_bwd_dx(const float* dy, const float* x, const float* mean, const float* invstd, const float* gb,
                          float slope, const double* dsums, double count, int64_t G, int64_t P, int64_t C, float* dx,
                          const float* dy2, const float* gb2, float slope2, const float* dgb, const float* dgb2,
                          int64_t gb_cs, void* stream);

int64_t csg_deprocess_u8_workspace(int64_t B);
int csg_deprocess_u8(const float* img, int64_t B, int64_t H, int64_t W, int64_t img_cs, const float* div3, const float* sub3,
                     int32_t rescale, uint8_t* out, float* workspace, int64_t workspace_bytes, void* stream);

int csg_draw_boxes_u8(const uint8_t* img, const float* boxes, const int64_t* objs, int64_t B, int64_t O, int64_t A, int64_t H,
                      int64_t W, int64_t image_id, const uint8_t* palette, int64_t P, int32_t thickness, uint8_t* out,
                      void* stream);

int csg_draw_labels_u8(const uint8_t* img, const float* boxes, const int64_t* objs, int64_t B, int64_t O, int64_t A,
                       int64_t H, int64_t W, int64_t image_id, const uint8_t* palette, int64_t P, const uint8_t* text,
                       const int32_t* text_off, const uint8_t* font, uint8_t* out, void* stream);

int csg_draw_graph_u8(const int32_t* prims, int64_t n_prims, const int32_t* prim_off, const uint8_t* text,
                      int64_t text_bytes, const uint8_t* font, int64_t B, int64_t H, int64_t W, uint32_t background,
                      uint8_t* out, void* stream);

#define CSG_PREPROCESS_MAX_SCALE 64
#define CSG_PREPROCESS_MAX_SIDE 8192
#define CSG_PREPROCESS_MAX_BATCH 1024
int64_t csg_preprocess_workspace(const int64_t* desc_host, int64_t B, int64_t W);
int csg_preprocess(const uint8_t* src, int64_t src_bytes, const int64_t* desc, const int64_t* desc_host, int64_t B, int64_t H,
                   int64_t W, const float* sub3, const float* div3, float* out, uint8_t* out_u8, uint8_t* workspace,
                   int64_t workspace_bytes, void* stream);

int64_t csg_preprocess_px_workspace(const int64_t* desc_host, int64_t B, int64_t W);
int csg_preprocess_px(const uint8_t* src, int64_t src_bytes, const int64_t* desc, const int64_t* desc_host, int64_t B, int64_t H,
                      int64_t W, const float* sub3, const float* div3, float* out, uint8_t* out_u8, uint8_t* workspace,
                      int64_t workspace_bytes, void* stream);

#define CSG_CLEVR_MAX_BATCH 65535
#define CSG_CLEVR_MAX_OBJECTS 1024
int csg_clevr_boxes(const double* geom, const int64_t* objs, int64_t A, const double* rot, const int64_t* counts,
                    const int64_t* objs_host, const int64_t* counts_host, int64_t B, int64_t O, float* boxes, void* stream);

#define CSG_VG_MAX_BATCH 1024
#define CSG_VG_MAX_OBJECTS 255
int csg_vg_rows(const int32_t* rows, const int64_t* sizes, const int64_t* counts, const int32_t* rows_host,
                const int64_t* sizes_host, const int64_t* counts_host, int64_t num_object_names, int64_t B, int64_t O,
                int64_t* objs, float* boxes, void* stream);

int csg_box_iou(const float* boxes_pred, const float* boxes_gt, const int64_t* objs, int64_t B, int64_t O, int64_t A,
                int64_t image_id, float* iou, uint8_t* counted, double* per_sample, double* totals, void* stream);

int64_t csg_relation_agreement_workspace(int64_t B);
int csg_relation_agreement(const float* boxes, const float* centers, const int64_t* triplets, const int64_t* triplet_type,
                           const int64_t* triplets_host, const int64_t* triplet_type_host, int64_t B, int64_t O, int64_t T,
                           int64_t P, const int32_t* pred_ids, uint8_t* tested, uint8_t* agrees, int64_t* per_sample,
                           int64_t* totals, void* workspace, int64_t workspace_bytes, void* stream);

int csg_layout_consistency(const float* boxes_a, const float* boxes_b, const uint8_t* counted, int64_t B, int64_t O,
                           float* iou_ab, float* shift, double* per_sample_f, int64_t* per_sample_i, double* totals_f,
                           int64_t* totals_i, void* stream);

#define CSG_REWRITE_ONE_SIDED 0
#define CSG_REWRITE_NOISE 1
#define CSG_REWRITE_FORWARD 0
#define CSG_REWRITE_BACKWARD 1
#define CSG_REWRITE_RANDOM 2
int csg_graph_rows_select(const int64_t* triplets, const int64_t* triplet_type, int64_t B, int64_t T, int64_t O, int64_t P,
                          const int32_t* pred_ids, int64_t* rows, int64_t* counts, void* stream);
int csg_graph_rewrite(const int64_t* rows, const int64_t* counts, const int64_t* image_id, int64_t B, int64_t R, int64_t P,
                      const int32_t* pred_ids, int mode, int direction, double share, uint64_t seed, int64_t* out,
                      void* stream);

int csg_nearest_resize_fwd(const float* x, int64_t B, int64_t IH, int64_t IW, int64_t C, int64_t OH, int64_t OW, float* y,
// ... 216 lines not shown
```

Before: 217.6 img/s.

## Group SPADE hidden convs sharing a segmap into single Winograd launches

Adds grouped Winograd kernels (forward, backward-data, weight-gradient) that run up to four SPADE mlp_shared convolutions reading the same segmentation map at one resolution as one launch. The generator collects same-level SPADE norms and computes their hidden activations together through a new autograd function. Weight packing gains offsets so the member weights land in one packed operand. This removes repeated launches and repeated reads of the shared input, at the cost of more complex kernels with per-member pointer selection and extra host-side planning.

```diff
diff --git a/canonicalsg2im_amd/_lib.py b/canonicalsg2im_amd/_lib.py
--- a/canonicalsg2im_amd/_lib.py
+++ b/canonicalsg2im_amd/_lib.py
@@ -31,7 +31,8 @@
 
 class WinoPackItem(ctypes.Structure):
     _fields_ = [("w", c_p), ("s_o", c_i64), ("s_i", c_i64), ("s_h", c_i64), ("s_w", c_i64), ("Cout", c_i64), ("Cin", c_i64),
-                ("backward_data", c_i32), ("variant", c_i32), ("packed", c_p)]
+                ("backward_data", c_i32), ("variant", c_i32), ("packed", c_p),
+                ("n_off", c_i32), ("k_off", c_i32), ("n_total", c_i32), ("k_total", c_i32)]
 
 
 class HingeItem(ctypes.Structure):
@@ -124,6 +125,10 @@
     "csg_wino_conv": (c_i32, [ctypes.POINTER(WinoDesc), c_p, c_p, c_p, c_p, c_p, c_f32, c_p, c_p, c_i64, c_p]),
     "csg_wino_bwd_weight_workspace": (c_i64, [ctypes.POINTER(WinoDesc)]),
     "csg_wino_bwd_weight": (c_i32, [ctypes.POINTER(WinoDesc), c_p, c_p, c_p, c_p, c_p, c_i64, c_p]),
+    "csg_wino_conv_group_fwd": (c_i32, [ctypes.POINTER(WinoDesc), c_i32, c_p, c_p, ctypes.POINTER(c_p), ctypes.POINTER(c_p), c_p]),
+    "csg_wino_conv_group_bwd_data": (c_i32, [ctypes.POINTER(WinoDesc), c_i32, ctypes.POINTER(c_p), c_p, c_p, c_f32, c_p, c_p]),
+    "csg_wino_bwd_weight_group_workspace": (c_i64, [ctypes.POINTER(WinoDesc), c_i32]),
+    "csg_wino_bwd_weight_group": (c_i32, [ctypes.POINTER(WinoDesc), c_i32, c_p, ctypes.POINTER(c_p), c_p, c_p, c_p, c_i64, c_p]),
     "csg_wino4_bwd_weight_workspace": (c_i64, [ctypes.POINTER(WinoDesc)]),
     "csg_wino4_bwd_weight": (c_i32, [ctypes.POINTER(WinoDesc), c_p, c_p, c_p, c_p, c_p, c_i64, c_p]),
     "csg_wino4_supported": (c_i32, [ctypes.POINTER(WinoDesc)]),
diff --git a/canonicalsg2im_amd/csrc/csg_api.hip b/canonicalsg2im_amd/csrc/csg_api.hip
--- a/canonicalsg2im_amd/csrc/csg_api.hip
+++ b/canonicalsg2im_amd/csrc/csg_api.hip
@@ -135,7 +135,7 @@
 
 extern "C" {
 
-int csg_version(void) { return 122; }
+int csg_version(void) { return 123; }
 const char* csg_last_error(void) { return csg::g_err; }
 
 int csg_prof_enable(int on) {
diff --git a/canonicalsg2im_amd/csrc/csg_pack.h b/canonicalsg2im_amd/csrc/csg_pack.h
--- a/canonicalsg2im_amd/csrc/csg_pack.h
+++ b/canonicalsg2im_amd/csrc/csg_pack.h
@@ -10,6 +10,7 @@
   float4* up;
   int s_n, s_k, s_h, s_w;
   int flip, N, K, NT32, Q8;
+  int NT32d, Q8d, nt_off, q_off;
   int start;
 };
 
diff --git a/canonicalsg2im_amd/csrc/csg_wino_host.h b/canonicalsg2im_amd/csrc/csg_wino_host.h
--- a/canonicalsg2im_amd/csrc/csg_wino_host.h
+++ b/canonicalsg2im_amd/csrc/csg_wino_host.h
@@ -79,6 +79,64 @@
   return rc;
 }
 
+
+template <typename T>
+static inline int wino_group_members(const char* who, const char* what, int n, T* const* a, T* (&out)[CSG_WINO_GROUP_MAX],
+                                     bool nullable) {
+  CSG_REQUIRE(n >= 1 && n <= CSG_WINO_GROUP_MAX, CSG_E_BADSHAPE, "%s: %d members (1..%d)", who, n, CSG_WINO_GROUP_MAX);
+  for (int i = 0; i < CSG_WINO_GROUP_MAX; ++i) out[i] = nullptr;
+  if (a == nullptr) {
+    CSG_REQUIRE(nullable, CSG_E_BADSHAPE, "%s: no %s", who, what);
+    return CSG_OK;
+  }
+  for (int i = 0; i < n; ++i) {
+    CSG_REQUIRE(a[i] != nullptr, CSG_E_BADSHAPE, "%s: %s of member %d is missing", who, what, i);
+    CSG_REQUIRE(((uintptr_t)a[i] % 16) == 0, CSG_E_UNSUPPORTED, "%s: %s of member %d must be 16-byte aligned", who, what, i);
+    out[i] = a[i];
+  }
+  return CSG_OK;
+}
+
+static inline int wino_group_operand(const char* who, int positions, int64_t NT32, int64_t Q8) {
+  CSG_REQUIRE((int64_t)positions * NT32 * Q8 * 1024 < CSG_MAX_RECORDS, CSG_E_UNSUPPORTED,
+              "%s: the group's packed weights are too large for 32-bit byte offsets", who);
+  return CSG_OK;
+}
+
+template <typename P>
+static inline int wino_group_fwd_plan(const char* who, P& p, int n, int positions, int& div) {
+  CSG_REQUIRE(n >= 1 && n <= CSG_WINO_GROUP_MAX, CSG_E_BADSHAPE, "%s: %d members (1..%d)", who, n, CSG_WINO_GROUP_MAX);
+  CSG_REQUIRE(p.Cout % 64 == 0 && p.y_cs == p.Cout, CSG_E_UNSUPPORTED,
+              "%s: members need dense outputs of a multiple of 64 channels (Cout=%d, y_cs=%d)", who, p.Cout, p.y_cs);
+  div = p.Cout / 64;
+  p.nblocks = div * n;
+  p.NT32 = (p.Cout / 32) * n;
+  return wino_group_operand(who, positions, p.NT32, p.Q8);
+}
+
+template <typename P>
+static inline int wino_group_bwd_plan(const char* who, P& p, int n, int positions, int stage_channels, int& div) {
+  CSG_REQUIRE(n >= 1 && n <= CSG_WINO_GROUP_MAX, CSG_E_BADSHAPE, "%s: %d members (1..%d)", who, n, CSG_WINO_GROUP_MAX);
+  CSG_REQUIRE(p.Cin % stage_channels == 0 && p.nstage == p.Cin / stage_channels, CSG_E_UNSUPPORTED,
+              "%s: members need a multiple of %d gradient channels (%d)", who, stage_channels, p.Cin);
+  div = p.nstage;
+  p.nstage = div * n;
+  p.ksplit = 1;
+  p.sps = p.nstage;
+  p.Q8 = (p.Cin / 8) * n;
+  return wino_group_operand(who, positions, p.NT32, p.Q8);
+}
+
+template <typename P>
+static inline int wino_group_wg_plan(const char* who, P& p, int n, int& div) {
+  CSG_REQUIRE(n >= 1 && n <= CSG_WINO_GROUP_MAX, CSG_E_BADSHAPE, "%s: %d members (1..%d)", who, n, CSG_WINO_GROUP_MAX);
+  CSG_REQUIRE(p.Cout % 64 == 0, CSG_E_UNSUPPORTED, "%s: members need a multiple of 64 output channels (%d)", who, p.Cout);
+  div = p.Cout / 64;
+  p.cblocks = div * n;
+  p.Cout *= n;
+  return CSG_OK;
+}
+
 static inline int64_t wino_pack_bytes(int positions, int64_t N, int64_t K) {
   if (N <= 0 || K <= 0) return -1;
   return (int64_t)positions * cdiv(N, 32) * cdiv(K, 8) * 64 * 16;
diff --git a/canonicalsg2im_amd/csrc/wino.hip b/canonicalsg2im_amd/csrc/wino.hip
--- a/canonicalsg2im_amd/csrc/wino.hip
+++ b/canonicalsg2im_amd/csrc/wino.hip
@@ -34,6 +34,19 @@
   long long slab;
 };
 
+struct WinoGroup {
+  const float* src[CSG_WINO_GROUP_MAX];
+  const float* bias[CSG_WINO_GROUP_MAX];
+  float* dst[CSG_WINO_GROUP_MAX];
+  int n, div;
+};
+
+template <typename T>
+__device__ __forceinline__ T wn_pick(T const (&a)[CSG_WINO_GROUP_MAX], int m) {
+  static_assert(CSG_WINO_GROUP_MAX == 4, "one select per member");
+  return m == 0 ? a[0] : (m == 1 ? a[1] : (m == 2 ? a[2] : a[3]));
+}
+
 __device__ __forceinline__ int wn_xcd_remap(int bid, int nblk) {
   const int q = nblk >> 3, r = nblk & 7;
   const int xcd = bid & 7, idx = bid >> 3;
@@ -43,7 +56,8 @@
 #define WP_LD 33
 __device__ __forceinline__ void wn_pack_tile(const float* __restrict__ w, int64_t s_n, int64_t s_k, int64_t s_h,
                                              int64_t s_w, int flip, int N, int K, const float* __restrict__ sigma,
-                                             int NT32, int Q8, float4* __restrict__ up, int qb, int nt) {
+                                             int Q8, float4* __restrict__ up, int qb, int nt, int NT32d, int Q8d,
+                                             int nt_off, int q_off) {
   __shared__ float g[9][32][WP_LD];
   const int tid = threadIdx.x;
   const bool k_fast = s_k <= s_n;
@@ -92,13 +106,13 @@
   }
 #pragma unroll
   for (int p = 0; p < 16; ++p)
-    up[(((int64_t)p * NT32 + nt) * Q8 + q) * 64 + lane] = make_float4(u[p][0], u[p][1], u[p][2], u[p][3]);
+    up[(((int64_t)p * NT32d + nt_off + nt) * Q8d + q_off + q) * 64 + lane] = make_float4(u[p][0], u[p][1], u[p][2], u[p][3]);
 }
 
 __global__ __launch_bounds__(256) void k_wino_pack(const float* __restrict__ w, int64_t s_n, int64_t s_k, int64_t s_h,
                                                     int64_t s_w, int flip, int N, int K, const float* __restrict__ sigma,
                                                     int NT32, int Q8, float4* __restrict__ up) {
-  wn_pack_tile(w, s_n, s_k, s_h, s_w, flip, N, K, sigma, NT32, Q8, up, blockIdx.x, blockIdx.y);
+  wn_pack_tile(w, s_n, s_k, s_h, s_w, flip, N, K, sigma, Q8, up, blockIdx.x, blockIdx.y, NT32, Q8, 0, 0);
 }
 
 __global__ __launch_bounds__(256) void k_wino_pack_multi(PackMulti pm) {
@@ -106,7 +120,8 @@
   while (i + 1 < pm.n && (int)blockIdx.x >= pm.it[i + 1].start) ++i;
   const PackMultiItem& d = pm.it[i];
   const int local = blockIdx.x - d.start, nqb = (d.Q8 + 3) >> 2;
-  wn_pack_tile(d.w, d.s_n, d.s_k, d.s_h, d.s_w, d.flip, d.N, d.K, nullptr, d.NT32, d.Q8, d.up, local % nqb, local / nqb);
+  wn_pack_tile(d.w, d.s_n, d.s_k, d.s_h, d.s_w, d.flip, d.N, d.K, nullptr, d.Q8, d.up, local % nqb, local / nqb, d.NT32d, d.Q8d,
+               d.nt_off, d.q_off);
 }
 
 constexpr int wn_row_stride(int TW) {
@@ -126,11 +141,11 @@
   return C * WN_PS;
 }
 
-template <int TW, int NTB = 2>
-__global__ __launch_bounds__(256, 2) void k_wino_conv2(WinoParams p, const float* __restrict__ x,
-                                                        const float4* __restrict__ up, const float* __restrict__ bias,
-                                                        const float* __restrict__ res, const float* __restrict__ gate,
-                                                        float* __restrict__ y) {
+template <int TW, int NTB, int GRP>
+__device__ __forceinline__ void wn_conv2_body(const WinoParams& p, const float* __restrict__ x,
+                                              const float4* __restrict__ up, const float* __restrict__ bias,
+                                              const float* __restrict__ res, const float* __restrict__ gate,
+                                              float* __restrict__ y, const WinoGroup& g) {
   constexpr int TH = 32 / TW;
   constexpr int R = 2 * TH + 2, C = 2 * TW + 2;
   constexpr int RS = wn_row_stride(TW);
@@ -150,8 +165,16 @@
   const int by = bid % p.tby;
   const int img = bid / p.tby;
   const int X0 = bx * 2 * TW, Y0 = by * 2 * TH;
-
-  const csg_i32x4 rsX = csg_make_srd(x, (long long)p.B * p.H * p.W * p.x_cs * 4);
+  int nbl = nb;
+  if constexpr (GRP == 1) {
+    const int m = nb / g.div;
+    nbl = nb - m * g.div;
+    bias = wn_pick(g.bias, m);
+    y = wn_pick(g.dst, m);
+  }
+
+  const long long x_bytes = (long long)p.B * p.H * p.W * p.x_cs * 4;
+  csg_i32x4 rsX = csg_make_srd(GRP == 2 ? g.src[0] : x, x_bytes);
   const csg_i32x4 rsU = csg_make_srd(up, (long long)16 * p.NT32 * p.Q8 * 64 * 16);
   unsigned goff[NLD];
   int loff[NLD];
@@ -170,9 +193,17 @@
     }
   }
   csg_f32x4 st[NLD];
+  int gm = 0, gl = 0;
   auto load_stage = [&](int s) {
-#pragma unroll
-    for (int i = 0; i < NLD; ++i) st[i] = csg_buf_load_x4(rsX, (int)goff[i], s * (WN_BK * 4), 0);
+    const int sl = GRP == 2 ? gl : s;
+#pragma unroll
+    for (int i = 0; i < NLD; ++i) st[i] = csg_buf_load_x4(rsX, (int)goff[i], sl * (WN_BK * 4), 0);
+    if constexpr (GRP == 2) {
+      const bool next = gl + 1 == g.div && gm + 1 < g.n;
+      gl = next ? 0 : gl + 1;
+      gm = next ? gm + 1 : gm;
+      rsX = csg_make_srd(wn_pick(g.src, gm), x_bytes);
+    }
   };
   auto store_stage = [&](float* base) {
 #pragma unroll
@@ -295,7 +326,7 @@
     __syncthreads();
     {
       const int tile = tid >> 3, cq = tid & 7;
-      const int n = nb * (32 * NTB) + nt * 32 + cq * 4;
+      const int n = nbl * (32 * NTB) + nt * 32 + cq * 4;
       const int ttx = tile % TW, tty = tile / TW;
       const int oy = Y0 + 2 * tty, ox = X0 + 2 * ttx;
       if (n < p.Cout && oy < p.H && ox < p.W) {
@@ -341,6 +372,22 @@
     }
     __syncthreads();
   }
+}
+
+template <int TW, int NTB = 2>
+__global__ __launch_bounds__(256, 2) void k_wino_conv2(WinoParams p, const float* __restrict__ x,
+                                                        const float4* __restrict__ up, const float* __restrict__ bias,
+                                                        const float* __restrict__ res, const float* __restrict__ gate,
+                                                        float* __restrict__ y) {
+  wn_conv2_body<TW, NTB, 0>(p, x, up, bias, res, gate, y, WinoGroup{});
+}
+
+template <int TW, int NTB, int GRP>
+__global__ __launch_bounds__(256, 2) void k_wino_conv2_group(WinoParams p, WinoGroup g, const float* __restrict__ x,
+                                                              const float4* __restrict__ up, const float* __restrict__ gate,
+                                                              float* __restrict__ y) {
+  static_assert(GRP == 1 || GRP == 2, "forward or backward-data");
+  wn_conv2_body<TW, NTB, GRP>(p, x, up, nullptr, nullptr, gate, y, g);
 }
 
 constexpr size_t wn_conv_lds(int TW) {
@@ -434,6 +481,77 @@
 
 }
 
+template <int GRP>
+static int wn_group_dispatch(const WinoParams& p, const WinoGroup& g, const float* x, const float4* up, const float* gate,
+                             float* y, hipStream_t s, const char* who) {
+  const int64_t grid = (int64_t)p.B * p.tby * p.tbx * p.nblocks;
+  CSG_REQUIRE(grid < (1ll << 31), CSG_E_UNSUPPORTED, "%s: grid too large", who);
+  auto go = [&](auto tw, auto ntb) {
+    constexpr int TW = decltype(tw)::value, NTB = decltype(ntb)::value;
+    constexpr size_t shm = wn_conv_lds(TW);
+    const int rc = lds_limit<k_wino_conv2_group<TW, NTB, GRP>, shm>(shm, who);
+    if (rc) return rc;
+    CSG_LAUNCH((k_wino_conv2_group<TW, NTB, GRP>), dim3((unsigned)grid), dim3(256), shm, s, p, g, x, up, gate, y);
+    return check_launch(who);
+  };
+  using I1 = std::integral_constant<int, 1>;
+  using I2 = std::integral_constant<int, 2>;
+  using I4 = std::integral_constant<int, 4>;
+  using I8 = std::integral_constant<int, 8>;
+  using I16 = std::integral_constant<int, 16>;
+  if constexpr (GRP == 2) {
+    if (p.ntb == 1) return p.TW == 16 ? go(I16(), I1()) : (p.TW == 8 ? go(I8(), I1()) : go(I4(), I1()));
+  }
+  return p.TW == 16 ? go(I16(), I2()) : (p.TW == 8 ? go(I8(), I2()) : go(I4(), I2()));
+}
+
+extern "C" {
+
+int csg_wino_conv_group_fwd(const csg_wino_desc* d, int32_t n, const float* x, const float* packed, const float* const* bias,
+                            float* const* y, void* stream) {
+  const char* who = "csg_wino_conv_group_fwd";
+  WinoParams p;
+  size_t shm = 0;
+  int rc = wn_plan(d, p, shm, who);
+  if (rc) return rc;
+  WinoGroup g = {};
+  rc = wino_group_fwd_plan(who, p, n, 16, g.div);
+  if (rc == CSG_OK) rc = wino_group_members(who, "y", n, y, g.dst, false);
+  if (rc == CSG_OK) rc = wino_group_members(who, "bias", n, bias, g.bias, true);
+  if (rc) return rc;
+  CSG_REQUIRE(x != nullptr && packed != nullptr && ((uintptr_t)x % 16) == 0 && ((uintptr_t)packed % 16) == 0, CSG_E_UNSUPPORTED,
+              "%s: x and packed must be 16-byte aligned", who);
+  g.n = n;
+  p.gate_slope = 0.f;
+  hipStream_t s = (hipStream_t)stream;
+  ProfScope ps(K_WINO_CONV, 2.0 * (double)(p.slab / p.y_cs) * 9.0 * p.Cin * p.Cout * n, s);
+  return wn_group_dispatch<1>(p, g, x, (const float4*)packed, nullptr, nullptr, s, who);
+}
+
+int csg_wino_conv_group_bwd_data(const csg_wino_desc* d, int32_t n, const float* const* dy, const float* packed,
+                                 const float* gate, float gate_slope, float* dx, void* stream) {
+  const char* who = "csg_wino_conv_group_bwd_data";
+  WinoParams p;
+  size_t shm = 0;
+  int rc = wn_plan(d, p, shm, who);
+  if (rc) return rc;
+  CSG_REQUIRE(d->act == CSG_ACT_NONE, CSG_E_UNSUPPORTED, "%s: no activation", who);
+  WinoGroup g = {};
+  rc = wino_group_bwd_plan(who, p, n, 16, WN_BK, g.div);
+  if (rc == CSG_OK) rc = wino_group_members(who, "dy", n, dy, g.src, false);
+  if (rc) return rc;
+  CSG_REQUIRE(dx != nullptr && packed != nullptr && ((uintptr_t)dx % 16) == 0 && ((uintptr_t)packed % 16) == 0 &&
+                  ((uintptr_t)gate % 16) == 0,
+              CSG_E_UNSUPPORTED, "%s: dx, packed and gate must be 16-byte aligned", who);
+  g.n = n;
+  p.gate_slope = gate_slope;
+  hipStream_t s = (hipStream_t)stream;
+  ProfScope ps(K_WINO_CONV, 2.0 * (double)(p.slab / p.y_cs) * 9.0 * p.Cin * p.Cout * n, s);
+  return wn_group_dispatch<2>(p, g, nullptr, (const float4*)packed, gate, dx, s, who);
+}
+
+}
+
 struct WinoWgParams {
   int B, H, W, Cin, x_cs, Cout, y_cs;
   int RXn, RYn, nregions;
@@ -443,10 +561,10 @@
 
 #define WG_EPS 33
 
-template <int TSX, int NT>
-__global__ __launch_bounds__(256, 2) void k_wino_wgrad(WinoWgParams p, const float* __restrict__ x,
-                                                        const float* __restrict__ dy, float* __restrict__ slabs,
-                                                        float* __restrict__ dbslabs) {
+template <int TSX, int NT, bool GRP>
+__device__ __forceinline__ void wn_wgrad_body(const WinoWgParams& p, const float* __restrict__ x,
+                                              const float* __restrict__ dy, float* __restrict__ slabs,
+                                              float* __restrict__ dbslabs, const WinoGroup& g) {
   static_assert(NT == 1, "one 32-channel input group per block");
   constexpr int TSY = 16 / TSX;
   constexpr int XR = 2 * TSY + 2, XC = 2 * TSX + 2, YR = 2 * TSY, YC = 2 * TSX;
@@ -463,6 +581,13 @@
   const int cb = bid % p.cblocks;
   const int sp = bid / p.cblocks;
   const int r0 = sp * p.rps, r1 = min(p.nregions, r0 + p.rps);
+  int cbl = cb, cout_m = p.Cout;
+  if constexpr (GRP) {
+    const int m = cb / g.div;
+    cbl = cb - m * g.div;
+    cout_m = g.div * 64;
+    dy = wn_pick(g.src, m);
+  }
 
   const int ia = wave == 0 ? 0 : (wave == 1 ? 1 : (wave == 2 ? 2 : 3));
   const int ib = wave == 0 ? 2 : (wave == 1 ? 2 : 1);
@@ -491,8 +616,8 @@
     const int e = tid + 256 * i;
     const int pix = e >> 4, c4 = e & 15;
     const int row = pix / YC, col = pix - row * YC;
-    const int ch = cb * 64 + c4 * 4;
-    yoff[i] = ch < p.Cout ? (unsigned)((row * p.W + col) * p.y_cs + ch) * 4u : CSG_OOB_OFF;
+    const int ch = cbl * 64 + c4 * 4;
+    yoff[i] = ch < cout_m ? (unsigned)((row * p.W + col) * p.y_cs + ch) * 4u : CSG_OOB_OFF;
   }
   typedef __attribute__((address_space(3))) void* lds_ptr;
   auto dma_stage = [&](int r, int bufsel) {
@@ -663,6 +788,19 @@
   }
 }
 
+template <int TSX, int NT>
+__global__ __launch_bounds__(256, 2) void k_wino_wgrad(WinoWgParams p, const float* __restrict__ x,
+                                                        const float* __restrict__ dy, float* __restrict__ slabs,
+                                                        float* __restrict__ dbslabs) {
+  wn_wgrad_body<TSX, NT, false>(p, x, dy, slabs, dbslabs, WinoGroup{});
+}
+
+template <int TSX, int NT>
+__global__ __launch_bounds__(256, 2) void k_wino_wgrad_group(WinoWgParams p, WinoGroup g, const float* __restrict__ x,
+                                                              float* __restrict__ slabs, float* __restrict__ dbslabs) {
+  wn_wgrad_body<TSX, NT, true>(p, x, nullptr, slabs, dbslabs, g);
+}
+
 static int wn_wg_tsx(int W) { return W >= 32 ? 16 : (W >= 16 ? 8 : 4); }
 
 static int wn_wg_plan(const csg_wino_desc* d, WinoWgParams& p, const char* who) {
@@ -680,18 +818,31 @@
 }
 
 template <int TSX>
-static int wn_wg_launch(const WinoWgParams& p, const float* x, const float* dy, float* slabs, float* dbslabs, hipStream_t s) {
+static int wn_wg_launch(const WinoWgParams& p, const float* x, const float* dy, float* slabs, float* dbslabs, hipStream_t s,
+                        const WinoGroup* g = nullptr) {
   constexpr int tsx = TSX, tsy = 16 / TSX;
   constexpr size_t x_f4 = (size_t)(((2 * tsy + 2) * (2 * tsx + 2) * 8 + 255) / 256) * 256;
   constexpr size_t stage_bytes = 2 * (x_f4 * 16 + (size_t)(2 * tsy) * (2 * tsx) * 64 * 4);
   constexpr size_t ep_bytes = (size_t)4 * 3 * 32 * WG_EPS * 4;
   constexpr size_t shm = stage_bytes > ep_bytes ? stage_bytes : ep_bytes;
-  const int rc = lds_limit<k_wino_wgrad<TSX, 1>, shm>(shm, "csg_wino_bwd_weight");
+  const int rc = g != nullptr ? lds_limit<k_wino_wgrad_group<TSX, 1>, shm>(shm, "csg_wino_bwd_weight_group")
+                              : lds_limit<k_wino_wgrad<TSX, 1>, shm>(shm, "csg_wino_bwd_weight");
   if (rc) return rc;
   ProfScope ps(K_WINO_WGRAD, 2.0 * p.B * p.H * p.W * 9.0 * p.Cin * p.Cout, s);
-  CSG_LAUNCH((k_wino_wgrad<TSX, 1>), dim3((unsigned)(p.cblocks * p.kblocks * p.nsplit)), dim3(256), shm, s, p, x, dy, slabs,
-             dbslabs);
+  const dim3 grid((unsigned)(p.cblocks * p.kblocks * p.nsplit));
+  if (g != nullptr) {
+    CSG_LAUNCH((k_wino_wgrad_group<TSX, 1>), grid, dim3(256), shm, s, p, *g, x, slabs, dbslabs);
+    return check_launch("csg_wino_bwd_weight_group");
+  }
+  CSG_LAUNCH((k_wino_wgrad<TSX, 1>), grid, dim3(256), shm, s, p, x, dy, slabs, dbslabs);
   return check_launch("csg_wino_bwd_weight");
+}
+
+static int wn_wg_group_plan(const csg_wino_desc* d, int n, WinoWgParams& p, int& div, const char* who) {
+  int rc = wn_wg_plan(d, p, who);
+  if (rc == CSG_OK) rc = wino_group_wg_plan(who, p, n, div);
+  if (rc) return rc;
+  return wino_wg_slice_plan(p, who, p.cblocks * p.kblocks, 1024, 8, 512);
 }
 
 extern "C" {
@@ -717,4 +868,34 @@
                      });
 }
 
-}
+int64_t csg_wino_bwd_weight_group_workspace(const csg_wino_desc* d, int32_t n) {
+  WinoWgParams p;
+  int div = 0;
+  if (wn_wg_group_plan(d, n, p, div, "csg_wino_bwd_weight_group_workspace")) return -1;
+  csg_wino_desc all = *d;
+  all.Cout = p.Cout;
+  return wino_wg_workspace(&all, p.nsplit);
+}
+
+int csg_wino_bwd_weight_group(const csg_wino_desc* d, int32_t n, const float* x, const float* const* dy, float* dw, float* db,
+                              float* workspace, int64_t workspace_bytes, void* stream) {
+  const char* who = "csg_wino_bwd_weight_group";
+  WinoWgParams p;
+  WinoGroup g = {};
+  int rc = wn_wg_group_plan(d, n, p, g.div, who);
+  if (rc == CSG_OK) rc = wino_group_members(who, "dy", n, dy, g.src, false);
+  if (rc) return rc;
+  g.n = n;
+  csg_wino_desc all = *d;
+  all.Cout = p.Cout;
+  hipStream_t s = (hipStream_t)stream;
+  return wino_wg_run(who, "csg_wino_bwd_weight_group(reduce)", &all, p.nsplit, p.nsplit == 1, dw, db, workspace, workspace_bytes, s,
+                     [&](float* slabs, float* dbslabs) {
+                       const int tsx = wn_wg_tsx(d->W);
+                       if (tsx == 16) return wn_wg_launch<16>(p, x, nullptr, slabs, dbslabs, s, &g);
+                       if (tsx == 8) return wn_wg_launch<8>(p, x, nullptr, slabs, dbslabs, s, &g);
+                       return wn_wg_launch<4>(p, x, nullptr, slabs, dbslabs, s, &g);
+                     });
+}
+
+}
diff --git a/canonicalsg2im_amd/csrc/wino4.hip b/canonicalsg2im_amd/csrc/wino4.hip
--- a/canonicalsg2im_amd/csrc/wino4.hip
+++ b/canonicalsg2im_amd/csrc/wino4.hip
@@ -55,7 +55,8 @@
 template <int RT>
 __device__ __forceinline__ void w4_pack_tile(const float* __restrict__ w, int64_t s_n, int64_t s_k, int64_t s_h,
                                              int64_t s_w, int flip, int N, int K, const float* __restrict__ sigma,
-                                             int NT32, int Q8, float4* __restrict__ up, int qb, int nt) {
+                                             int Q8, float4* __restrict__ up, int qb, int nt, int NT32d, int Q8d,
+                                             int nt_off, int q_off) {
   __shared__ float g[RT][32][WP4_LD];
   const int tid = threadIdx.x;
   const bool k_fast = s_k <= s_n;
@@ -124,7 +125,7 @@
         for (int b = 1; b < RT; ++b) acc += t[e][xi][b] * G[nu][b];
         u[e] = acc;
       }
-      up[(((int64_t)(xi * 6 + nu) * NT32 + nt) * Q8 + q) * 64 + lane] = make_float4(u[0], u[1], u[2], u[3]);
+      up[(((int64_t)(xi * 6 + nu) * NT32d + nt_off + nt) * Q8d + q_off + q) * 64 + lane] = make_float4(u[0], u[1], u[2], u[3]);
     }
 }
 
@@ -132,7 +133,7 @@
 __global__ __launch_bounds__(256) void k_wino4_pack(const float* __restrict__ w, int64_t s_n, int64_t s_k, int64_t s_h,
                                                      int64_t s_w, int flip, int N, int K, const float* __restrict__ sigma,
                                                      int NT32, int Q8, float4* __restrict__ up) {
-  w4_pack_tile<RT>(w, s_n, s_k, s_h, s_w, flip, N, K, sigma, NT32, Q8, up, blockIdx.x, blockIdx.y);
+  w4_pack_tile<RT>(w, s_n, s_k, s_h, s_w, flip, N, K, sigma, Q8, up, blockIdx.x, blockIdx.y, NT32, Q8, 0, 0);
 }
 
 __global__ __launch_bounds__(256) void k_wino4_pack_multi(PackMulti pm) {
@@ -140,7 +141,8 @@
   while (i + 1 < pm.n && (int)blockIdx.x >= pm.it[i + 1].start) ++i;
   const PackMultiItem& d = pm.it[i];
   const int local = blockIdx.x - d.start, nqb = (d.Q8 + 3) >> 2;
-  w4_pack_tile<3>(d.w, d.s_n, d.s_k, d.s_h, d.s_w, d.flip, d.N, d.K, nullptr, d.NT32, d.Q8, d.up, local % nqb, local / nqb);
+  w4_pack_tile<3>(d.w, d.s_n, d.s_k, d.s_h, d.s_w, d.flip, d.N, d.K, nullptr, d.Q8, d.up, local % nqb, local / nqb, d.NT32d, d.Q8d,
+                  d.nt_off, d.q_off);
 }
 
 __device__ __forceinline__ csg_f32x2 w4_pfma(float c, csg_f32x2 a, csg_f32x2 b) {
@@ -897,6 +899,12 @@
                   "csg_wino_pack_weights_multi: item %d: weight too large for 32-bit element offsets", i);
       const int NT32 = (int)cdiv(N, 32), Q8 = (int)cdiv(K, 8);
       const int nb = (int)cdiv(Q8, 4) * NT32;
+      const bool placed = it.n_total != 0 || it.k_total != 0;
+      CSG_REQUIRE(!placed || (N % 32 == 0 && K % 8 == 0 && it.n_off >= 0 && it.k_off >= 0 && it.n_off % 32 == 0 &&
+                              it.k_off % 8 == 0 && it.n_total % 32 == 0 && it.k_total % 8 == 0 && it.n_off + N <= it.n_total &&
+                              it.k_off + K <= it.k_total),
+                  CSG_E_BADSHAPE, "csg_wino_pack_weights_multi: item %d: (%ld, %ld) at (%d, %d) of a (%d, %d) operand", i, (long)N,
+                  (long)K, it.n_off, it.k_off, it.n_total, it.k_total);
       if (cnt == CSG_PACK_MULTI || blocks + nb > (1 << 20)) {
         const int rc = flush();
         if (rc) return rc;
@@ -905,6 +913,8 @@
       d.w = it.w; d.up = (float4*)it.packed;
       d.s_n = (int)s_n; d.s_k = (int)s_k; d.s_h = (int)it.s_h; d.s_w = (int)it.s_w;
       d.flip = it.backward_data ? 1 : 0; d.N = (int)N; d.K = (int)K; d.NT32 = NT32; d.Q8 = Q8;
+      d.NT32d = placed ? it.n_total / 32 : NT32; d.Q8d = placed ? it.k_total / 8 : Q8;
+      d.nt_off = placed ? it.n_off / 32 : 0; d.q_off = placed ? it.k_off / 8 : 0;
       d.start = blocks;
       blocks += nb;
       bytes += (double)it.Cout * it.Cin * 9 * 4 + (double)(variant == 4 ? 36 : 16) * NT32 * Q8 * 64 * 16;
diff --git a/canonicalsg2im_amd/ops.py b/canonicalsg2im_amd/ops.py
--- a/canonicalsg2im_amd/ops.py
+++ b/canonicalsg2im_amd/ops.py
@@ -14,7 +14,7 @@
 __all__ = [
     "nhwc", "empty_nhwc", "conv2d", "linear", "norm_act", "upsample2x", "nearest_resize", "avgpool3s2", "embed", "real_object_mask",
     "norm_act_pair", "graph_csr", "gather_concat", "segment_avg", "layout_pyramid", "layout_paint", "disc_input", "crop_objects", "maxpool2", "avgpool2", "l1_mean",
-    "invalidate_weight_caches", "pack_conv_weight", "wino_pack", "prepack_weights", "wino_eligible", "wino_variant", "plan_conv", "spectral_weight", "spectral_weights", "spade_infer", "norm_eval_stats", "deprocess_u8", "preprocess_images", "pack_frozen_forward", "ACT_NONE", "ACT_LEAKY", "ACT_TANH",
+    "invalidate_weight_caches", "pack_conv_weight", "wino_pack", "prepack_weights", "wino_eligible", "wino_variant", "plan_conv", "plan_hidden_group", "spade_hidden_group", "spectral_weight", "spectral_weights", "spade_infer", "norm_eval_stats", "deprocess_u8", "preprocess_images", "pack_frozen_forward", "ACT_NONE", "ACT_LEAKY", "ACT_TANH",
     "conv2d_forward", "pool3", "spatial_mean", "resize_bilinear", "feat_stats", "feat_stats_finalize", "softmax_rows", "inception_score", "POOL_MAX", "POOL_AVG9", "POOL_AVG_INSIDE",
     "crop_windows", "crop_resize_bilinear", "kid_sums", "feat_class_sums", "knn_radii", "ball_counts",
     "augment_table", "augment_table_host", "d_augment",
@@ -712,6 +712,146 @@
     return y[:, :Cout] if po else y
 
 
+HIDDEN_GROUP_MAX = 4
+HiddenGroupPlan = collections.namedtuple("HiddenGroupPlan", "plans fwd dx wgrad")
+
+
+def plan_hidden_group(B, H, W, Cin, couts, act=ACT_LEAKY, slope=0.0, has_bias=True, need=(True, True, True)):
+    if isinstance(has_bias, bool):
+        has_bias = [has_bias] * len(couts)
+    plans = [plan_conv(B, H, W, Cin, c, 3, 3, 1, 1, act, slope, has_bias=hb, need=need) for c, hb in zip(couts, has_bias)]
+    n = len(plans)
+    same = 1 < n <= HIDDEN_GROUP_MAX and len(set(couts)) == 1 and couts[0] % 64 == 0 and len(set(has_bias)) == 1
+
+    def mode(keys, grouped):
+        if getattr(plans[0], keys[0]) is None:
+            return None
+        kinds = set(tuple(getattr(p, k) for k in keys) for p in plans)
+        return "group" if (same and kinds == {grouped}) else "members"
+
+    return HiddenGroupPlan(plans, mode(("fwd", "fwd_var"), ("wino", 2)), mode(("dx", "dx_var"), ("wino", 2)),
+                           mode(("wgrad",), ("wino",)))
+
+
+def _ptr_array(ts):
+    return (ctypes.c_void_p * len(ts))(*[t.data_ptr() for t in ts])
+
+
+def _pack_group(weights, directions):
+    ws = [_f32(w.detach()) for w in weights]
+    Cout, Cin = ws[0].shape[0], ws[0].shape[1]
+    n = len(ws)
+    items, out = [], []
+    for backward_data in directions:
+        N, K = (Cin, n * Cout) if backward_data else (n * Cout, Cin)
+        packed = torch.empty(lib.csg_wino_pack_bytes(N, K) // 4, device=ws[0].device, dtype=torch.float32)
+        out.append(packed)
+        for k, w in enumerate(ws):
+            st = w.stride()
+            it = WinoPackItem()
+            it.w, it.s_o, it.s_i, it.s_h, it.s_w = w.data_ptr(), st[0], st[1], st[2], st[3]
+            it.Cout, it.Cin, it.backward_data, it.variant, it.packed = Cout, Cin, 1 if backward_data else 0, 2, packed.data_ptr()
+            it.n_off, it.k_off = (0, k * Cout) if backward_data else (k * Cout, 0)
+            it.n_total, it.k_total = N, K
+            items.append(it)
+    if items:
+        check(lib.csg_wino_pack_weights_multi((WinoPackItem * len(items))(*items), len(items), stream()),
+              "wino_pack_weights_multi(group)")
+    return out
+
+
+class _HiddenGroup(torch.autograd.Function):
+
+    @staticmethod
+    def forward(ctx, seg, act, slope, *wb):
+        x = nhwc(_f32(seg))
+        B, Cin, H, W = x.shape
+        n = len(wb) // 2
+        ws, bs = wb[:n], wb[n:]
+        for w in ws:
+            if tuple(w.shape[1:]) != (Cin, 3, 3):
+                raise RuntimeError("spade_hidden_group: a member's weight is %s for %d input channels" % (tuple(w.shape), Cin))
+        need = (ctx.needs_input_grad[0], any(ctx.needs_input_grad[3:3 + n]), any(ctx.needs_input_grad[3 + n:]))
+        gp = plan_hidden_group(B, H, W, Cin, [w.shape[0] for w in ws], act, slope, [b is not None for b in bs], need)
+        Cout = ws[0].shape[0]
+        ctx.ut, ctx.ut_pre = None, [None] * n
+        dirs = ([False] if gp.fwd == "group" else []) + ([True] if gp.dx == "group" else [])
+        packed = dict(zip(dirs, _pack_group(ws, dirs)))
+        ctx.ut = packed.get(True)
+        if gp.fwd == "group":
+            ys = [empty_nhwc(B, Cout, H, W, x.device) for _ in ws]
+            bias = _ptr_array([b.detach() for b in bs]) if bs[0] is not None else None
+            check(lib.csg_wino_conv_group_fwd(_wino_desc(B, H, W, Cin, Cout, act, slope), n, ptr(x), ptr(packed[False]),
+                                              bias, _ptr_array(ys), stream()), "wino_conv_group_fwd")
+            if gp.dx == "members":
+                ctx.ut_pre = [_take_dx_operand(p, w) for p, w in zip(gp.plans, ws)]
+        else:
+            ys = []
+            for k in range(n):
+                y, ctx.ut_pre[k] = _conv_fwd(gp.plans[k], x, ws[k], bs[k], None, None)
+                ys.append(y)
+        ctx.gp, ctx.n = gp, n
+        ctx.set_materialize_grads(False)
+        ctx.save_for_backward(x, *ws)
+        return tuple(ys)
+
+    @staticmethod
+    def backward(ctx, *dys):
+        x, ws = ctx.saved_tensors[0], ctx.saved_tensors[1:]
+        gp, n, dev = ctx.gp, ctx.n, x.device
+        B, Cin, H, W = x.shape
+        Cout = ws[0].shape[0]
+        live = [k for k in range(n) if dys[k] is not None]
+        dys = [nhwc(_f32(d)) if d is not None else None for d in dys]
+        dx, dws, dbs = None, [None] * n, [None] * n
+        if ctx.needs_input_grad[0] and live:
+            if gp.dx == "group":
+                ut = ctx.ut if len(live) == n else _pack_group([ws[k] for k in live], [True])[0]
+                dx = empty_nhwc(B, Cin, H, W, dev)
+                check(lib.csg_wino_conv_group_bwd_data(_wino_desc(B, H, W, Cout, Cin), len(live), _ptr_array([dys[k] for k in live]),
+                                                       ptr(ut), None, 0.0, ptr(dx), stream()), "wino_conv_group_bwd_data")
+            else:
+                for k in live:
+                    p = gp.plans[k]
+                    if p.dx == "wino":
+                        ut = ctx.ut_pre[k] if ctx.ut_pre[k] is not None else wino_pack(ws[k], True, None, p.dx_var)
+                        nxt = empty_nhwc(B, Cin, H, W, dev)
+                        _wino_launch(dys[k], ut, None, dx, nxt, B, H, W, ws[k].shape[0], Cin, ACT_NONE, 0.0, "wino_conv_bwd_data",
+                                     variant=p.dx_var)
+                        dx = nxt
+                    else:
+                        dk = _conv_bwd(p, dys[k], x, ws[k], None, (True, False, False), None, None)[0]
+                        dx = dk if dx is None else dx + dk
+        want_w, want_b = ctx.needs_input_grad[3:3 + n], ctx.needs_input_grad[3 + n:]
+        if live and (any(want_w) or any(want_b)):
+            if gp.wgrad == "group" and len(live) > 1:
+                m = len(live)
+                d = _wino_desc(B, H, W, Cin, Cout)
+                nws = lib.csg_wino_bwd_weight_group_workspace(d, m)
+                if nws < 0:
+                    raise RuntimeError("wino_bwd_weight_group_workspace: " + _lib.last_error())
+                wsb = torch.empty(nws // 4, device=dev, dtype=torch.float32)
+                dwp = torch.empty((m * Cout, 3, 3, Cin), device=dev, dtype=torch.float32)
+                dbp = torch.empty(m * Cout, device=dev, dtype=torch.float32) if any(want_b) else None
+                check(lib.csg_wino_bwd_weight_group(d, m, ptr(x), _ptr_array([dys[k] for k in live]), ptr(dwp), ptr(dbp), ptr(wsb),
+                                                    nws, stream()), "wino_bwd_weight_group")
+                for i, k in enumerate(live):
+                    dws[k] = dwp[i * Cout:(i + 1) * Cout].permute(0, 3, 1, 2) if want_w[k] else None
+                    dbs[k] = dbp[i * Cout:(i + 1) * Cout] if want_b[k] else None
+            else:
+                for k in live:
+                    _, dws[k], dbs[k] = _conv_bwd(gp.plans[k], dys[k], x, ws[k], None, (False, want_w[k], want_b[k]), None, None)
+        return (dx, None, None) + tuple(dws) + tuple(dbs)
+
+
+def spade_hidden_group(seg, members, act=ACT_LEAKY, slope=0.0):
+    if not 1 <= len(members) <= HIDDEN_GROUP_MAX:
+        raise RuntimeError("spade_hidden_group: %d members (1..%d)" % (len(members), HIDDEN_GROUP_MAX))
+    if any(w.shape[0] % 4 or w.shape[1] % 4 for w, _ in members):
+        raise RuntimeError("spade_hidden_group: channel counts must be multiples of 4")
+    return list(_HiddenGroup.apply(seg, int(act), float(slope), *([w for w, _ in members] + [b for _, b in members])))
+
+
 def linear(x, weight, bias=None, act=ACT_NONE, slope=0.0, in_act=None, grad_is_pre=False):
     lead = x.shape[:-1]
     K = x.shape[-1]
diff --git a/canonicalsg2im_amd/spade/models/networks/generator.py b/canonicalsg2im_amd/spade/models/networks/generator.py
--- a/canonicalsg2im_amd/spade/models/networks/generator.py
+++ b/canonicalsg2im_amd/spade/models/networks/generator.py
@@ -1,3 +1,4 @@
+import torch
 import torch.nn as nn
 
 from .... import ops
@@ -7,7 +8,7 @@
 from ....sg2im.utils import real_object_mask
 from .architecture import SPADEResnetBlock
 from .base_network import BaseNetwork
-from .normalization import SegPyramid
+from .normalization import SegPyramid, hidden_groupable
 
 
 class AppearanceEncoder(nn.Module):
@@ -60,6 +61,17 @@
         sw = opt.image_size[0] >> _LATENT_HALVINGS[opt.num_upsampling_layers]
         return sw, round(sw / opt.aspect_ratio)
 
+    def _hidden_groups(self, no_upsample):
+        h, by_level = self.sw, {}
+        for name in self._block_names:
+            if name not in no_upsample:
+                h *= 2
+            blk = getattr(self, name)
+            by_level.setdefault(h, []).extend(([blk.norm_s] if blk.learned_shortcut else []) + [blk.norm_0, blk.norm_1])
+        n = ops.HIDDEN_GROUP_MAX
+        return {h: [ms[i:i + n] for i in range(0, len(ms), n) if len(ms[i:i + n]) > 1 and hidden_groupable(ms[i:i + n])]
+                for h, ms in by_level.items()}
+
     def forward(self, objs, layout_boxes, layout_masks, test_mode=False):
         if self.sw != self.sh:
             raise NotImplementedError("aspect_ratio != 1 is not on the hot path")
@@ -72,9 +84,10 @@
             maps = ops.layout_paint(self.attribute_embedding(objs), layout_boxes, valid, layout_masks, H, levels)
         else:
             maps = ops.layout_pyramid(self.attribute_embedding(objs), layout_boxes, valid, H, levels, masks=layout_masks)
-        seg = SegPyramid(zip(levels, maps))
+        no_upsample = {"head_0"} | (set() if self.opt.num_upsampling_layers in ('more', 'most') else {"G_middle_1"})
+        grouped = self.training and torch.is_grad_enabled() and not test_mode and maps[0].is_cuda
+        seg = SegPyramid(zip(levels, maps), self._hidden_groups(no_upsample) if grouped else None)
         x = self.fc(seg.at(self.sw))
-        no_upsample = {"head_0"} | (set() if self.opt.num_upsampling_layers in ('more', 'most') else {"G_middle_1"})
         for name in self._block_names:
             if name not in no_upsample:
                 x = ops.upsample2x(x)
diff --git a/canonicalsg2im_amd/spade/models/networks/normalization.py b/canonicalsg2im_amd/spade/models/networks/normalization.py
--- a/canonicalsg2im_amd/spade/models/networks/normalization.py
+++ b/canonicalsg2im_amd/spade/models/networks/normalization.py
@@ -11,11 +11,30 @@
 
 class SegPyramid:
 
-    def __init__(self, levels):
+    def __init__(self, levels, hidden_groups=None):
         self.levels = dict(levels)
+        self.hidden_groups = hidden_groups or {}
+        self._actv = {}
 
     def at(self, h):
         return self.levels[int(h)]
+
+    def hidden_actv(self, spade, h):
+        if id(spade) not in self._actv:
+            group = next((g for g in self.hidden_groups.get(int(h), ()) if any(m is spade for m in g)), None)
+            if group is None:
+                return None
+            convs = [m.mlp_shared[0] for m in group]
+            outs = ops.spade_hidden_group(self.at(h), [(c.weight, c.bias) for c in convs], convs[0].act, convs[0].slope)
+            self._actv.update((id(m), y) for m, y in zip(group, outs))
+        return self._actv.pop(id(spade))
+
+
+def hidden_groupable(spades):
+    convs = [m.mlp_shared[0] for m in spades]
+    c0 = convs[0]
+    return all(tuple(c.kernel_size) == (3, 3) and c.padding[0] == 1 and c.weight.shape == c0.weight.shape
+               and (c.bias is None) == (c0.bias is None) and (c.act, c.slope) == (c0.act, c0.slope) for c in convs)
 
 
 class InstanceNormAct(nn.InstanceNorm2d):
@@ -150,13 +169,16 @@
         _joined(self, "_joined_w", self.mlp_gamma.weight, self.mlp_beta.weight)
         return self.__dict__.get("_joined_w")
 
-    def _conv_operands(self, x, segmap):
-        if isinstance(segmap, SegPyramid):
-            seg = segmap.at(x.size(2))
-        else:
-            seg = segmap if segmap.shape[2:] == x.shape[2:] else ops.nearest_resize(segmap, x.shape[2:])
-        sh = self.mlp_shared[0]
-        actv = ops.conv2d(seg, sh.weight, sh.bias, 1, sh.padding[0], sh.act, sh.slope, grad_is_pre=True)
+    def _conv_operands(self, x, segmap, actv=None):
+        if actv is None and isinstance(segmap, SegPyramid):
+            actv = segmap.hidden_actv(self, x.size(2))
+        if actv is None:
+            if isinstance(segmap, SegPyramid):
+                seg = segmap.at(x.size(2))
+            else:
+                seg = segmap if segmap.shape[2:] == x.shape[2:] else ops.nearest_resize(segmap, x.shape[2:])
+            sh = self.mlp_shared[0]
+            actv = ops.conv2d(seg, sh.weight, sh.bias, 1, sh.padding[0], sh.act, sh.slope, grad_is_pre=True)
         w = _joined(self, "_joined_w", self.mlp_gamma.weight, self.mlp_beta.weight)
         b = _joined(self, "_joined_b", self.mlp_gamma.bias, self.mlp_beta.bias)
         return actv, w, b
diff --git a/include/csg_hip.h b/include/csg_hip.h
--- a/include/csg_hip.h
+++ b/include/csg_hip.h
@@ -132,8 +132,18 @@
   int32_t backward_data;
   int32_t variant;
   float* packed;
+  int32_t n_off, k_off, n_total, k_total;
 } csg_wino_pack_item;
 int csg_wino_pack_weights_multi(const csg_wino_pack_item* items, int32_t n, void* stream);
+
+#define CSG_WINO_GROUP_MAX 4
+int csg_wino_conv_group_fwd(const csg_wino_desc* d, int32_t n, const float* x, const float* packed,
+                            const float* const* bias, float* const* y, void* stream);
+int csg_wino_conv_group_bwd_data(const csg_wino_desc* d, int32_t n, const float* const* dy, const float* packed,
+                                 const float* gate, float gate_slope, float* dx, void* stream);
+int64_t csg_wino_bwd_weight_group_workspace(const csg_wino_desc* d, int32_t n);
+int csg_wino_bwd_weight_group(const csg_wino_desc* d, int32_t n, const float* x, const float* const* dy, float* dw,
+                              float* db, float* workspace, int64_t workspace_bytes, void* stream);
 int32_t csg_wino4_persistent(int32_t on);
 int64_t csg_wino4_pack_bytes(int64_t N, int64_t K);
 int csg_wino4_pack_weights(const float* w, int64_t s_o, int64_t s_i, int64_t s_h, int64_t s_w, int64_t Cout, int64_t Cin,
```

Result: no change. 218.1 img/s (median of 6 runs) (+0.2%).
